# lh3/ropebwt2

Measured on AMD Instinct MI355X. Metric: Gsymbols/s inserted (wall-clock), bit-identical .fmd, higher is better.
Workload: dtype u8; 1 GPU; configs[1]: 100000000 x 101 bp synthetic reads (splitmix64 seed 42), -bsR -m4g, 1 x MI355X; step = one -m batch (40844297/40844297/18311406 reads); 20 steps = 7 job(s) of 3 batches, each job on an empty index (the last job stops after batch 2); reads_per_job=100000000, symbols=69532236588, symbols_per_gpu=69532236588, parallelism=1 GPU, driver=single engine, counts_ok=True

## Files before the change

include/rb2_hip.h:

```cpp
#ifndef RB2_HIP_H_
#define RB2_HIP_H_

#include <stdint.h>

#ifdef __cplusplus
extern "C" {
#endif

typedef struct rb2_hip_s rb2_hip_t;

#define RB2_SO_IO   0
#define RB2_SO_RLO  1
#define RB2_SO_RCLO 2

typedef void (*rb2_hip_fatal_cb)(void *user, const char *message);
void rb2_hip_set_fatal_handler(rb2_hip_fatal_cb cb, void *user);

int rb2_hip_device_count(void);

rb2_hip_t *rb2_hip_create(int device, int sorting_order);
void rb2_hip_destroy(rb2_hip_t *h);
int  rb2_hip_sorting_order(const rb2_hip_t *h);
void rb2_hip_reset(rb2_hip_t *h);

void rb2_hip_insert_multi(rb2_hip_t *h, int64_t len, const uint8_t *s);

void rb2_hip_set_lazy(rb2_hip_t *h, int on);
void rb2_hip_wait(rb2_hip_t *h);
int  rb2_hip_last_batch_counts(rb2_hip_t *h, int64_t d[36]);

void rb2_hip_prefetch(rb2_hip_t *h, const uint8_t *s, int64_t n_final, int64_t capacity);
int rb2_hip_host_register(void *p, int64_t nbytes);
int rb2_hip_host_unregister(void *p);

void rb2_hip_mem_info(int device, int64_t *free_bytes, int64_t *total_bytes);

void rb2_hip_insert_multi_dev(rb2_hip_t *h, int64_t len, const uint8_t *s_dev);

void rb2_hip_get_counts(rb2_hip_t *h, int64_t c[36]);

int64_t rb2_hip_rope_bytes(rb2_hip_t *h, int b);
int64_t rb2_hip_download_rope(rb2_hip_t *h, int b, uint8_t *dst);
typedef void (*rb2_hip_run_cb)(void *user, const uint8_t *runs, int64_t n_bytes);
int64_t rb2_hip_stream_rope(rb2_hip_t *h, int b, rb2_hip_run_cb cb, void *user);

void rb2_hip_load_ropes(rb2_hip_t *h, const uint8_t *const rle[6], const int64_t n_bytes[6]);

int64_t rb2_hip_load_fmd(rb2_hip_t *h, const void *fmd, int64_t n_bytes);
int64_t rb2_hip_load_fmd_file(rb2_hip_t *h, const char *path);

int64_t rb2_hip_save_fmd(rb2_hip_t *h, void *dst, int64_t cap);
int64_t rb2_hip_save_fmd_file(rb2_hip_t *h, const char *path);

int64_t rb2_hip_delete_strings(rb2_hip_t *h, int64_t n, const int64_t *ids);
void rb2_hip_delete_stats(rb2_hip_t *h, int64_t out[5]);

void rb2_hip_reserve(rb2_hip_t *h, int64_t batch_bytes, int64_t batch_strings, int64_t total_symbols);

void rb2_hip_rank1a(rb2_hip_t *h, int b, int64_t x, int64_t cx[6]);
void rb2_hip_rank_batch(rb2_hip_t *h, int b, int64_t n, const int64_t *x, int64_t *out);

void rb2_hip_backward_search(rb2_hip_t *h, int64_t n, const uint8_t *pat, const int64_t *off, int64_t *out);
void rb2_hip_backward_search_dev(rb2_hip_t *h, int64_t n, const uint8_t *pat, const int64_t *off, int64_t *out);
void rb2_hip_extend(rb2_hip_t *h, int64_t n, const int64_t *ik, int is_back, int64_t *ok);
int64_t rb2_hip_extract(rb2_hip_t *h, int64_t n, const int64_t *rows, int64_t max_len, uint8_t *out, int64_t *len);
int64_t rb2_hip_smem(rb2_hip_t *h, int64_t n, const uint8_t *qry, const int64_t *off, int64_t min_len, int64_t min_occ, int64_t max_mems,
                     int64_t *mem, int64_t *cnt);
void rb2_hip_smem_dev(rb2_hip_t *h, int64_t n, const uint8_t *qry, const int64_t *off, int64_t min_len, int64_t min_occ, int64_t max_mems,
                      int64_t *mem, int64_t *cnt);

int64_t rb2_hip_ssa_build(rb2_hip_t *h, int log2_step);
void    rb2_hip_ssa_drop(rb2_hip_t *h);
void    rb2_hip_ssa_info(rb2_hip_t *h, int64_t out[4]);
int64_t rb2_hip_locate(rb2_hip_t *h, int64_t n, const int64_t *iv, int64_t max_hits, int64_t *hit, int64_t *cnt);
void    rb2_hip_locate_dev(rb2_hip_t *h, int64_t n, const int64_t *iv, int64_t max_hits, int64_t *hit, int64_t *cnt);

int64_t rb2_hip_overlap(rb2_hip_t *h, int64_t n, const uint8_t *qry, const int64_t *off, int64_t min_ovlp, int64_t max_recs, int64_t *rec, int64_t *cnt);
void    rb2_hip_overlap_dev(rb2_hip_t *h, int64_t n, const uint8_t *qry, const int64_t *off, int64_t min_ovlp, int64_t max_recs, int64_t *rec, int64_t *cnt);
int64_t rb2_hip_string_ids(rb2_hip_t *h, int64_t n, const int64_t *zv, int64_t max_hits, int64_t *ids, int64_t *cnt);
void    rb2_hip_string_ids_dev(rb2_hip_t *h, int64_t n, const int64_t *zv, int64_t max_hits, int64_t *ids, int64_t *cnt);

int64_t rb2_hip_kmers(rb2_hip_t *h, int k, int64_t min_occ, int canonical, int64_t max_recs, int64_t *rec, int64_t hist_len, int64_t *hist, int64_t info[4]);

int64_t rb2_hip_approx(rb2_hip_t *h, int64_t n, const uint8_t *qry, const int64_t *off, int max_mm, int64_t min_occ, int64_t max_steps, int64_t max_recs, int64_t *rec, int64_t *cnt);
void    rb2_hip_approx_dev(rb2_hip_t *h, int64_t n, const uint8_t *qry, const int64_t *off, int max_mm, int64_t min_occ, int64_t max_steps, int64_t max_recs, int64_t *rec, int64_t *cnt);

int64_t rb2_hip_contained(rb2_hip_t *h, int64_t n, const int64_t *ids, int64_t *rec);
void    rb2_hip_contained_dev(rb2_hip_t *h, int64_t n, const int64_t *ids, int64_t *rec);

int64_t rb2_hip_irreducible(rb2_hip_t *h, int64_t n, const uint8_t *qry, const int64_t *off, int64_t min_ovlp, int64_t max_ext, int64_t max_steps, int64_t max_recs,
                            int64_t *rec, int64_t *cnt);
void    rb2_hip_irreducible_dev(rb2_hip_t *h, int64_t n, const uint8_t *qry, const int64_t *off, int64_t max_len, int64_t min_ovlp, int64_t max_ext, int64_t max_steps,
                                int64_t max_recs, int64_t *rec, int64_t *cnt);

int64_t rb2_hip_unitig_chains(rb2_hip_t *h, int64_t n_str, int64_t m, const int64_t *edges, int64_t *vtx, int64_t info[4]);
void    rb2_hip_unitig_chains_dev(rb2_hip_t *h, int64_t n_str, int64_t m, const int64_t *edges, int64_t *vtx, int64_t *info);
int64_t rb2_hip_unitig_text(rb2_hip_t *h, int64_t n_str, const int64_t *vtx, int canonical, int64_t min_reads, int64_t cap_u, int64_t cap_txt, int64_t *urec, uint8_t *txt,
                            int64_t info[4]);
int64_t rb2_hip_unitig_text_dev(rb2_hip_t *h, int64_t n_str, const int64_t *vtx, int canonical, int64_t min_reads, int64_t cap_u, int64_t cap_txt, int64_t *urec, uint8_t *txt,
                                int64_t info[4]);

uint64_t rb2_hip_rope_hash(rb2_hip_t *h, int b);

int64_t rb2_hip_unpack(rb2_hip_t *h, int64_t first, int64_t n, int reversed, int64_t cap, uint8_t *txt, int64_t *off);
int64_t rb2_hip_unpack_dev(rb2_hip_t *h, int64_t first, int64_t n, int reversed, int64_t cap, uint8_t *txt, int64_t *off);
int64_t rb2_hip_merge(rb2_hip_t *dst, rb2_hip_t *src, int64_t batch_bytes, int64_t info[4]);

int64_t rb2_hip_string_graph(rb2_hip_t *h, int64_t first, int64_t n, int64_t min_ovlp, int64_t max_ext, int64_t max_steps, int64_t max_recs, int64_t max_hits, int pairs,
                             int64_t cap, int64_t *edges, int64_t info[8]);
int64_t rb2_hip_string_graph_dev(rb2_hip_t *h, int64_t first, int64_t n, int64_t min_ovlp, int64_t max_ext, int64_t max_steps, int64_t max_recs, int64_t max_hits, int pairs,
                                 int64_t cap, int64_t *edges, int64_t info[8]);

int     rb2_hip_num_subropes(void);
void    rb2_hip_memcpy(rb2_hip_t *h, void *dst, const void *src, int64_t bytes, int kind);
void    rb2_hip_use_stream(rb2_hip_t *h, void *hip_stream);


typedef struct rb2_hip_multi_s rb2_hip_multi_t;
#define RB2_TRANSPORT_PEER 0
#define RB2_TRANSPORT_RCCL 1
#define RB2_MULTI_MAX_RANKS 64
rb2_hip_multi_t *rb2_hip_multi_create(int n, const int *devices, int sorting_order, int transport, const int *owner );
int rb2_hip_multi_transport(const rb2_hip_multi_t *m);
void rb2_hip_multi_unique_id(void *id128);
rb2_hip_multi_t *rb2_hip_multi_create_rank(int device, int rank, int nranks, const void *nccl_id, int sorting_order, const int *owner);
void rb2_hip_multi_destroy(rb2_hip_multi_t *m);
void rb2_hip_default_owners(int nranks, int owner[] );
int  rb2_hip_multi_nranks(const rb2_hip_multi_t *m);
int  rb2_hip_multi_nlocal(const rb2_hip_multi_t *m);
rb2_hip_t *rb2_hip_multi_engine(rb2_hip_multi_t *m, int local_rank);
void rb2_hip_multi_insert_multi(rb2_hip_multi_t *m, int64_t len, const uint8_t *s);
void rb2_hip_multi_insert_multi_dev(rb2_hip_multi_t *m, int64_t len, const uint8_t *const *s_dev);
void rb2_hip_multi_get_counts(rb2_hip_multi_t *m, int64_t c[36]);
int64_t rb2_hip_multi_rope_bytes(rb2_hip_multi_t *m, int b);
int64_t rb2_hip_multi_download_rope(rb2_hip_multi_t *m, int b, uint8_t *dst);
int64_t rb2_hip_multi_stream_rope(rb2_hip_multi_t *m, int b, rb2_hip_run_cb cb, void *user);
void rb2_hip_multi_load_ropes(rb2_hip_multi_t *m, const uint8_t *const rle[6], const int64_t n_bytes[6]);
int64_t rb2_hip_multi_load_fmd(rb2_hip_multi_t *m, const void *fmd, int64_t n_bytes);
void rb2_hip_multi_reserve(rb2_hip_multi_t *m, int64_t batch_bytes, int64_t batch_strings, int64_t total_symbols);
void rb2_hip_multi_reset(rb2_hip_multi_t *m);
void rb2_hip_multi_sync(rb2_hip_multi_t *m);
void rb2_hip_multi_rank1a(rb2_hip_multi_t *m, int b, int64_t x, int64_t cx[6]);
void rb2_hip_multi_stats(rb2_hip_multi_t *m, int64_t out[6]);
int64_t rb2_hip_multi_text_bytes(const rb2_hip_multi_t *m, int k);
uint64_t rb2_hip_multi_rope_hash(rb2_hip_multi_t *m, int b);
int rb2_hip_multi_plan_host(const int *owner , int nranks, const int64_t *g , int me, int64_t *sdest , int64_t (*pieces)[5] , int64_t *total);


void *rb2_hip_dev_alloc(rb2_hip_t *h, int64_t bytes);
void  rb2_hip_dev_free(rb2_hip_t *h, void *p);

void rb2_hip_synth_reads(rb2_hip_t *h, uint8_t *dst_dev, int64_t first_read, int64_t n_reads,
                         int read_len, uint64_t seed, int strand);
void rb2_hip_synth_reads_cov(rb2_hip_t *h, uint8_t *dst_dev, int64_t first_read, int64_t n_reads,
                             int read_len, uint64_t seed, int strand, int64_t genome_len);
void rb2_hip_synth_reads_skew(rb2_hip_t *h, uint8_t *dst_dev, int64_t first_read, int64_t n_reads,
                              int read_len, uint64_t seed, int strand, int64_t genome_len, int skew);

void rb2_hip_sync(rb2_hip_t *h);

void rb2_hip_sparse_stats(rb2_hip_t *h, int64_t out[4]);
void rb2_hip_layout_stats(rb2_hip_t *h, int64_t out[8]);
void rb2_hip_rewind_stats(rb2_hip_t *h, int64_t out[4]);
void rb2_hip_steady_stats(rb2_hip_t *h, int64_t out[4]);
void rb2_hip_lean_stats(rb2_hip_t *h, int64_t out[2]);
void rb2_hip_window_stats(rb2_hip_t *h, int64_t out[6]);

#define RB2_K_SYM      0
#define RB2_K_TSCAN    1
#define RB2_K_PREP     2
#define RB2_K_PART     3
#define RB2_K_MERGE    4
#define RB2_K_META     5
#define RB2_K_ADVANCE  6
#define RB2_K_INIT     7
#define RB2_K_RELAYOUT 8
#define RB2_K_SPLIT    9
#define RB2_K_COUNT    10
void rb2_hip_profile(rb2_hip_t *h, int enable);
void rb2_hip_profile_get(rb2_hip_t *h, int64_t launches[RB2_K_COUNT], double ms[RB2_K_COUNT],
                         int64_t units[RB2_K_COUNT], int reset);
const char *rb2_hip_kernel_name(int k);

void rb2_hip_layout(int *leaf_syms, int *tile_leaves, int *string_tile);

#ifdef __cplusplus
}
#endif
#endif
```

ropebwt2_amd/build.py:

```python
import os
import subprocess
import sys

PKG = os.path.dirname(os.path.abspath(__file__))
ROOT = os.path.dirname(PKG)
CSRC = os.path.join(PKG, "csrc")
LIBDIR = os.path.join(PKG, "lib")
BINDIR = os.path.join(PKG, "bin")
INC = os.path.join(ROOT, "include")


def lib_path(name):
    return os.path.join(LIBDIR, name)


def _newer(target, sources):
    if not os.path.exists(target):
        return False
    t = os.path.getmtime(target)
    return all(os.path.getmtime(s) <= t for s in sources)


def _run(cmd):
    r = subprocess.run(cmd, stdout=subprocess.PIPE, stderr=subprocess.STDOUT, text=True)
    if r.returncode != 0:
        sys.stderr.write(r.stdout)
        raise RuntimeError("build failed: " + " ".join(cmd))
    return r.stdout


def build_hip(force=False):
    os.makedirs(LIBDIR, exist_ok=True)
    out = lib_path("librb2hip.so")
    srcs = [os.path.join(CSRC, f) for f in ("rb2_engine.hip", "rb2_kernels.h", "rb2_merge.h", "rb2_device.h", "rb2_multi.h", "rb2_query.h", "rb2_unitig.h", "rb2_query_host.h", "rb2_query_plan.h", "rb2_kmer_plan.h", "rb2_fmd_load.h", "rb2_delete.h", "rb2_delete_plan.h", "rb2_fmd_save.h", "rb2_fmd_plan.h", "rb2_unpack.h", "rb2_merge_plan.h", "rb2_graph.h", "rb2_graph_plan.h")] + [os.path.join(INC, "rb2_hip.h")]
    if not force and _newer(out, srcs):
        return out
    hipcc = os.environ.get("HIPCC", "/opt/rocm/bin/hipcc")
    _run([hipcc, "--offload-arch=gfx950", "-O3", "-std=c++17", "-fPIC", "-shared", "-I" + INC, "-I" + CSRC,
          "-Wno-unused-value", "-o", out, srcs[0], "-ldl", "-lpthread"])
    return out


def build_host(force=False):
    host = os.path.join(CSRC, "host")
    if not os.path.isdir(host):
        return None
    os.makedirs(LIBDIR, exist_ok=True)
    os.makedirs(BINDIR, exist_ok=True)
    csrcs = sorted(os.path.join(host, f) for f in os.listdir(host) if f.endswith(".c") and f != "main.c")
    hdrs = [os.path.join(INC, f) for f in os.listdir(INC)] + [os.path.join(host, f) for f in os.listdir(host) if f.endswith(".h")]
    out = lib_path("libropebwt2.so")
    if force or not _newer(out, csrcs + hdrs + [lib_path("librb2hip.so")]):
        _run(["gcc", "-O2", "-g", "-std=gnu99", "-Wall", "-Werror=implicit-function-declaration", "-fPIC", "-shared", "-I" + INC, "-I" + host, "-o", out] + csrcs +
             ["-L" + LIBDIR, "-lrb2hip", "-Wl,-rpath,$ORIGIN", "-lpthread"])
    main_c = os.path.join(host, "main.c")
    exe = os.path.join(BINDIR, "ropebwt2")
    if os.path.exists(main_c) and (force or not _newer(exe, [main_c, out] + hdrs)):
        _run(["gcc", "-O2", "-g", "-std=gnu99", "-Wall", "-Werror=implicit-function-declaration", "-I" + INC, "-I" + host, "-o", exe, main_c,
              "-L" + LIBDIR, "-lropebwt2", "-lrb2hip", "-Wl,-rpath,$ORIGIN/../lib", "-lz", "-lpthread"])
    gen_c = os.path.join(ROOT, "tools", "synth_reads.c")
    gen = os.path.join(BINDIR, "synth_reads")
    if os.path.exists(gen_c) and (force or not _newer(gen, [gen_c])):
        _run(["gcc", "-O2", "-std=c99", "-Wall", "-o", gen, gen_c])
    return out


def build_all(force=False):
    build_hip(force)
    build_host(force)


if __name__ == "__main__":
    build_all(force="--force" in sys.argv)
    print("built:", sorted(os.listdir(LIBDIR)))
```

ropebwt2_amd/csrc/rb2_engine.hip:

```cpp
#include <hip/hip_runtime.h>
#include <cstdio>
#include <cstdlib>
#include <cstring>
#include <climits>
#include <vector>
#include <algorithm>
#include <chrono>
#include <mutex>
#include <thread>
#include <condition_variable>
#include "rb2_hip.h"
#include "rb2_kernels.h"
#include "rb2_query.h"
#include "rb2_unitig.h"
#include "rb2_unpack.h"
#include "rb2_graph.h"
#include "rb2_merge_plan.h"
#include "rb2_fmd_load.h"
#include "rb2_delete.h"
#include "rb2_fmd_save.h"
#include <cerrno>
#include <fcntl.h>
#include <unistd.h>

// ... 22 lines not shown
	if (g_fatal_cb) g_fatal_cb(g_fatal_user, msg);
	abort();
}
#define HIPCHK(expr) do { hipError_t e_ = (expr); if (e_ != hipSuccess) { \
	rb2_fatal("[rb2_hip] %s failed at %s:%d: %s\n", #expr, __FILE__, __LINE__, hipGetErrorString(e_)); } } while (0)

namespace {

static int g_vmm_ok = -1;
static size_t g_vmm_va = 0;
static bool vmm_enabled()
{
	if (g_vmm_ok < 0) {
		size_t fr = 0, tot = 0;
		g_vmm_ok = getenv("RB2_NO_VMM") ? 0 : 1;
		if (g_vmm_ok && hipMemGetInfo(&fr, &tot) == hipSuccess && tot > 0) g_vmm_va = (tot + (1ull << 30)) & ~((1ull << 30) - 1);
		else g_vmm_ok = 0;
	}
	return g_vmm_ok == 1;
}

static thread_local int64_t *t_grow_in_rounds = nullptr;
template <typename T> struct DevBuf {
	T *p = nullptr; size_t cap = 0;
	bool vm = false;
	size_t vm_div = 1;
	size_t vm_bytes = 0;
	bool vm_res = false;
	size_t vm_res_bytes = 0;
	size_t vm_piece = 0;
	std::vector<hipMemGenericAllocationHandle_t> vm_h; std::vector<size_t> vm_sz;
	size_t vm_range() const { return (g_vmm_va / vm_div + (4ull << 30)) & ~((2ull << 30) - 1); }
	bool vm_grow(size_t n)
	{
		const size_t CH = 64ull << 20;
		if (!vmm_enabled() || (p && !vm_res)) return false;
		int dev = 0;
		if (hipGetDevice(&dev) != hipSuccess) return false;
		hipMemAllocationProp prop = {};
		prop.type = hipMemAllocationTypePinned; prop.location.type = hipMemLocationTypeDevice; prop.location.id = dev;
		if (!p) {
			void *base = nullptr;
			const hipError_t er = hipMemAddressReserve(&base, vm_range(), CH, nullptr, 0);
			if (er != hipSuccess) {
				if (getenv("RB2_HIP_TRACE")) fprintf(stderr, "[rb2_hip] hipMemAddressReserve(%.1f GB) failed (%s): pools grow by hipMalloc + copy\n", vm_range() / 1e9, hipGetErrorString(er));
				(void)hipGetLastError(); g_vmm_ok = 0; return false;
			}
			p = (T*)base; vm_res = true; vm_res_bytes = vm_range();
		}
		if (!vm_piece) { vm_piece = CH; while (vm_piece < (2ull << 30) && vm_piece * 8 < n * sizeof(T)) vm_piece <<= 1; }
		const size_t want = (n * sizeof(T) + vm_piece - 1) / vm_piece * vm_piece;
		if (want > vm_res_bytes) {
			if (vm_bytes == 0) vm_release();
			return false;
		}
		hipMemAccessDesc acc = {};
		acc.location = prop.location; acc.flags = hipMemAccessFlagsProtReadWrite;
		while (vm_bytes < want) {
			const size_t add = vm_piece;
			hipMemGenericAllocationHandle_t h;
			bool ok = hipMemCreate(&h, add, &prop, 0) == hipSuccess;
			if (ok && (hipMemMap((char*)p + vm_bytes, add, 0, h, 0) != hipSuccess || hipMemSetAccess((char*)p + vm_bytes, add, &acc, 1) != hipSuccess)) {
				(void)hipMemUnmap((char*)p + vm_bytes, add); (void)hipMemRelease(h); ok = false;
			}
			if (!ok) {
				if (getenv("RB2_HIP_TRACE")) fprintf(stderr, "[rb2_hip] mapping %.2f GB behind %.2f GB failed (%s)\n", add / 1e9, vm_bytes / 1e9, hipGetErrorString(hipGetLastError()));
				(void)hipGetLastError();
				if (vm_bytes == 0) vm_release();
				return false;
			}
			vm_h.push_back(h); vm_sz.push_back(add);
			vm_bytes += add; cap = vm_bytes / sizeof(T);
		}
		return true;
	}
	void vm_release()
	{
		size_t off = 0;
		for (size_t i = 0; i < vm_h.size(); ++i) { (void)hipMemUnmap((char*)p + off, vm_sz[i]); (void)hipMemRelease(vm_h[i]); off += vm_sz[i]; }
		if (vm_res) (void)hipMemAddressFree(p, vm_res_bytes);
		vm_h.clear(); vm_sz.clear(); vm_bytes = 0; vm_res = false; vm_res_bytes = 0; p = nullptr; cap = 0;
	}
	void ensure(size_t n, bool keep = false, hipStream_t st = 0) {
		if (n <= cap) return;
		if (t_grow_in_rounds) ++*t_grow_in_rounds;
		if (vm && vm_grow(n)) return;
		size_t ncap = std::max(n, cap + cap / 2);
		T *q = nullptr;
		hipError_t e_ = hipMalloc((void**)&q, ncap * sizeof(T));
		if (e_ != hipSuccess && ncap > n) { ncap = n; (void)hipGetLastError(); e_ = hipMalloc((void**)&q, ncap * sizeof(T)); }
		if (e_ != hipSuccess) {
			size_t fr = 0, tot = 0;
			(void)hipMemGetInfo(&fr, &tot);
			rb2_fatal("[rb2_hip] out of device memory: a buffer of %.2f GB was needed (it held %.2f GB before), %.2f of %.2f GB are free; "
					"use smaller batches (-m) or shard the index over more GPUs\n", ncap * sizeof(T) / 1e9, cap * sizeof(T) / 1e9, fr / 1e9, tot / 1e9);
		}
		if (keep && p && cap) { HIPCHK(hipMemcpyAsync(q, p, cap * sizeof(T), hipMemcpyDeviceToDevice, st)); HIPCHK(hipStreamSynchronize(st)); }
		if (p) { if (vm_res) vm_release(); else HIPCHK(hipFree(p)); }
		p = q; cap = ncap;
	}
	void release() { if (p) { if (vm_res) vm_release(); else HIPCHK(hipFree(p)); } p = nullptr; cap = 0; }
};

struct Pool {
	DevBuf<uint8_t> data, xh; DevBuf<LeafMeta> meta, own; DevBuf<SbRec> sbrec; DevBuf<SbBase> sbbase;
	uint64_t cap_leaves = 0;
	void ensure(uint64_t leaves, bool keep, hipStream_t st) {
		if (leaves <= cap_leaves) return;
		data.vm = meta.vm = own.vm = sbrec.vm = true;
		meta.vm_div = own.vm_div = 16; sbrec.vm_div = 256;
		uint64_t nl = std::max<uint64_t>(leaves, cap_leaves + cap_leaves / 4);
		nl = (nl + SB - 1) / SB * SB;
		data.ensure(nl * LEAFB, keep, st); meta.ensure(nl, keep, st); own.ensure(nl, keep, st);
		sbrec.ensure(nl / SB + 1, keep, st); sbbase.ensure(nl / SB / SCHUNK + 2, keep, st); xh.ensure(nl / WPL + 1024, keep, st);
		cap_leaves = nl;
	}
	PoolView view() const { return PoolView{data.p, meta.p, sbrec.p, own.p, sbbase.p, xh.p}; }
	void release() { data.release(); meta.release(); own.release(); sbrec.release(); sbbase.release(); xh.release(); cap_leaves = 0; }
};

struct ProfRec { int k; hipEvent_t a, b; int64_t units; int round; };
constexpr uint64_t POS32_LIMIT = (1ull << 32) - (1ull << 24);

}

struct rb2_hip_s {
	int dev = 0, so = 0;
	hipStream_t st = 0;
	Pool pool[2];
	int side = 0;
	int pside = 0;
	bool sparse = false;
	double sp_lambda = 0.6;
	int sp_backoff = 0, sp_penalty = 0;
	int sp_head = 8;
	int sp_maxpen = 6;
	int leaf_pipe = 8192;
	Mailbox *mb_h = nullptr;
	Mailbox *mb_d = nullptr;
	uint64_t layout_epoch = 0;
	hipEvent_t ev_flag = nullptr;
	int dir_ride = 1;
	int ts_blocks = TSB;
	int lazy_verdict = 1;
	uint64_t spec_rounds = 0;
	int run_ahead = 3;
	int verdict_poll = 1;
	int steady_on = 1;
	int steady_ahead = 3;
	bool steady_launched = false;
	int64_t n_prep_skipped = 0, steady_seen = -1, steady_used = -1;
	int lean = 1;
	int64_t n_lean_rounds = 0;
	int64_t n_rewind = 0, n_rewound = 0, rewind_max = 0, n_rewind_even = 0;
	unsigned long long *pair_d = nullptr, *pair_h = nullptr;
	bool pair_valid = false;
	bool pending_end = false;
	double tl_base = 0, tl_last = 0;
	int64_t n_grow_in_rounds = 0;
	int timeline = 0;
	int lazy_insert = 1;
	int64_t n_relayout = 0, n_void = 0, n_sparse_rounds = 0;
	Ctl *ctl = nullptr;
	RopeDesc h_rope[NR];
	DevBuf<uint64_t> L[2], U[2], W[2], START, SIZE, INS_E, zblk;
	bool pos32 = false, want_pos32 = false;
	int pos_mode = getenv("RB2_POS") ? atoi(getenv("RB2_POS")) : 0;
	uint64_t pos_m0 = 0;
	DevBuf<uint16_t> RKREL;
	DevBuf<uint64_t> RKOLD;
	DevBuf<uint32_t> SPL;
	uint32_t split_epoch = 0;
	bool want_respread = false;
	int64_t n_respread = 0;
	DevBuf<uint64_t> qbuf;
	DevBuf<QTab> qtab;
	DevBuf<uint8_t> qbytes; DevBuf<int64_t> qin, qout;
	DevBuf<uint8_t> qscr;
	DevBuf<uint64_t> ssa_smp, ssa_len, ssa_head;
	bool ssa_valid = false; int ssa_s = 0; int64_t ssa_n = 0; uint64_t ssa_nstr = 0;
	uint64_t sp_nsb = 0;
	DevBuf<LeafDesc> LD;
	DevBuf<uint8_t> A[2], INS_A, sbuf;
	DevBuf<uint8_t> sbuf2; hipStream_t st_copy = nullptr; const uint8_t *pf_host = nullptr; size_t pf_done = 0; std::mutex pf_mu;
	bool pf_busy = false; std::condition_variable pf_cv;
	static constexpr int UP_T = 6, UP_NB = 2; static constexpr size_t UP_CH = 8u << 20;
	uint8_t *up_pin[UP_T][UP_NB] = {}; hipStream_t up_st[UP_T] = {}; hipEvent_t up_ev[UP_T][UP_NB] = {}; bool up_init = false;
	DevBuf<TileRec> trec; DevBuf<TileScan> tsc; DevBuf<TileFix> tfix; DevBuf<ChunkPart> cpart;
	DevBuf<SbTot> sbtot;
	uint64_t *d_tmp = nullptr;
	int prof = 0;
	std::vector<ProfRec> recs;
	std::vector<hipEvent_t> evpool;
	int64_t p_launch[RB2_K_COUNT]; double p_ms[RB2_K_COUNT]; int64_t p_units[RB2_K_COUNT];
	int debug = 0;
	int cur_round = -1;
	uint64_t *gcnt = nullptr;
	bool own_stream = true;
	int rank = 0, nranks = 1; int owner[NR] = {0};
	PushTab *push[2] = {nullptr, nullptr};
	int nactive = 1;
	DevBuf<uint8_t> xstage, xpack; DevBuf<uint16_t> xnb; DevBuf<uint64_t> xoff;
	uint8_t *xhost[2] = {nullptr, nullptr}; uint64_t *xtot[2] = {nullptr, nullptr}; hipEvent_t xev[2] = {nullptr, nullptr};
	int64_t fmds_size = -1;
	int compact_ok = 1;
	int compact_stats = 0;
	int64_t n_compact_rounds = 0;
	int64_t n_plain_handover = 0;
	bool pool_compact = false;
	bool plain_next = false;
	int ts_fold = SCHUNK;
	int ts_max = TS_MAX;
	int trace = 0;
	int64_t del_stats[5] = {0, 0, 0, 0, 0};
};

namespace {

hipEvent_t get_event(rb2_hip_t *h)
{
	if (!h->evpool.empty()) { hipEvent_t e = h->evpool.back(); h->evpool.pop_back(); return e; }
	hipEvent_t e; HIPCHK(hipEventCreate(&e)); return e;
}

struct Scope {
	rb2_hip_t *h; int k; ProfRec r; bool on;
	Scope(rb2_hip_t *h_, int k_, int64_t units) : h(h_), k(k_) {
		on = h->prof == 1 || (h->prof == 2 && k == RB2_K_MERGE);
		if (!on) return;
		r.k = k; r.units = units; r.round = h->cur_round; r.a = get_event(h); r.b = get_event(h);
		HIPCHK(hipEventRecord(r.a, h->st));
	}
	~Scope() {
		if (h->debug) { hipError_t e = hipStreamSynchronize(h->st); if (e != hipSuccess) { rb2_fatal("[rb2_hip] kernel group %s failed: %s\n", rb2_hip_kernel_name(k), hipGetErrorString(e)); } }
		if (!on) return;
		HIPCHK(hipEventRecord(r.b, h->st));
		h->recs.push_back(r);
	}
};

void drain_profile(rb2_hip_t *h)
{
	for (auto &r : h->recs) {
		float ms = 0;
		HIPCHK(hipEventElapsedTime(&ms, r.a, r.b));
		h->p_launch[r.k] += 1; h->p_ms[r.k] += ms; h->p_units[r.k] += r.units;
		if (h->trace && r.round >= 0 && (r.round < 20 || r.round % 10 == 0)) fprintf(stderr, "[rb2_hip] round %3d %-10s %8.3f ms\n", r.round, rb2_hip_kernel_name(r.k), ms);
		h->evpool.push_back(r.a); h->evpool.push_back(r.b);
	}
	h->recs.clear();
}

inline unsigned cdiv(uint64_t a, uint64_t b) { return (unsigned)((a + b - 1) / b); }
inline unsigned grid8(unsigned g) { return (g + 8u * XCD_RUN - 1u) & ~(8u * XCD_RUN - 1u); }

#define RB2_LAUNCH_STRIDE(h, KT, KF, ...) do { if ((h)->nranks > 1) hipLaunchKernelGGL(KT, __VA_ARGS__); else hipLaunchKernelGGL(KF, __VA_ARGS__); } while (0)
inline uint64_t rank_share(const rb2_hip_t *h, uint64_t whole)
{
	if (h->nranks <= 1) return whole;
	return std::min<uint64_t>(whole, 2 * whole / (uint64_t)std::max(1, h->nactive) + 64);
}

void build_directory(rb2_hip_t *h, int sd , int pool , uint64_t nsb_ub, bool sparse = false, bool leaves_done = false, uint64_t nsb_grid = 0)
{
	if (nsb_ub == 0) return;
	const hipStream_t st_ = h->st;
	if (nsb_grid == 0 || nsb_grid > nsb_ub) nsb_grid = nsb_ub;
	const unsigned nchunk = cdiv(nsb_ub, SCHUNK);
	h->sbtot.ensure(nsb_ub);
	PoolView pv = h->pool[pool].view();
	if (!leaves_done) RB2_LAUNCH_STRIDE(h, k_meta_sb<true>, k_meta_sb<false>, dim3(cdiv(nsb_grid, 8)), dim3(256), 0, st_, h->ctl, sd, pv, h->sbtot.p, (int)sparse);
	hipLaunchKernelGGL(k_sbscan3, dim3(nchunk), dim3(SCHUNK / SBT), 0, st_, (const Ctl*)h->ctl, (const SbTot*)h->sbtot.p, pv);
	hipLaunchKernelGGL(k_sbscan2, dim3(1), dim3(SB2T), 0, st_, (const Ctl*)h->ctl, pv.sbbase);
}

void fetch_ropes(rb2_hip_t *h)
{
	HIPCHK(hipMemcpyAsync(h->h_rope, &h->ctl->rope[h->side][0], sizeof(RopeDesc) * NR, hipMemcpyDeviceToHost, h->st));
	HIPCHK(hipStreamSynchronize(h->st));
}


struct BatchState {
	const uint8_t *s = nullptr; uint64_t len = 0, m = 0, max_len = 0, n_tot = 0, nsb_ub = 0;
	unsigned nst_ub = 0, nsc = 0;
	int cur = 0;
	bool known_ae = false;
	bool known_ae0 = false;
	bool known_steady = false;
	uint64_t counted = (uint64_t)-1;
	int lean = 0;
	uint64_t setup_round = (uint64_t)-1;
	bool setup_sparse = false; uint64_t setup_epoch = 0;
};
inline void mark_setup(const rb2_hip_t *h, BatchState &B, uint64_t r) { B.setup_round = r; B.setup_sparse = h->sparse; B.setup_epoch = h->layout_epoch; }
inline bool setup_done(const rb2_hip_t *h, const BatchState &B, uint64_t r, bool sparse) { return B.setup_round == r && B.setup_sparse == sparse && B.setup_epoch == h->layout_epoch; }

void ensure_strings(rb2_hip_t *h, uint64_t m)
{
	for (int i = 0; i < 2; ++i) { h->L[i].ensure(m); h->U[i].ensure(m); h->W[i].ensure(m); }
	h->SIZE.ensure(m); h->INS_E.ensure(m); h->RKREL.ensure(m); h->RKOLD.ensure(m); h->SPL.ensure(m + 64);
	h->A[0].ensure(m); h->A[1].ensure(m); h->INS_A.ensure(m); h->START.ensure(m + 1);
	const uint64_t nst = cdiv(m, STILE) + NR;
	h->trec.ensure(nst + 8 * XCD_RUN + 8); h->tsc.ensure(nst + 8 * XCD_RUN + 8); h->tfix.ensure(nst + 8 * XCD_RUN + 8); h->cpart.ensure(cdiv(nst, SCHUNK) + 1);
}

template <class P> StrArrays<P> str_arrays(rb2_hip_t *h, const BatchState &B)
{
	const int c = B.cur;
	return { (P*)h->L[c].p, (P*)h->U[c].p, h->W[c].p, h->A[c].p, (P*)h->L[c ^ 1].p, (P*)h->U[c ^ 1].p, h->W[c ^ 1].p, h->A[c ^ 1].p,
	         h->tfix.p, (P*)h->SIZE.p, (P*)h->INS_E.p, h->RKREL.p, (P*)h->RKOLD.p, h->INS_A.p };
}
template <class F> inline void with_pos(rb2_hip_t *h, const BatchState &B, F f) { if (h->pos32) f(str_arrays<uint32_t>(h, B)); else f(str_arrays<uint64_t>(h, B)); }

inline volatile unsigned long long *hmax_report(const rb2_hip_t *h) { return h->pos32 ? &h->mb_d->hmax : nullptr; }
inline volatile unsigned long long *steady_report(const rb2_hip_t *h) { return h->nranks == 1 ? &h->mb_d->steady : nullptr; }
inline uint32_t split_cap(const rb2_hip_t *h) { return (uint32_t)std::min<uint64_t>(h->SPL.cap, 0xffffffffu); }

static uint64_t max_batch_strings()
{
	const char *e = getenv("RB2_MAX_BATCH_STRINGS");
	uint64_t v = (1ull << 32) - 2 * STILE;
	if (e && atoll(e) > 0) v = std::min<uint64_t>(v, (uint64_t)atoll(e));
	return v;
}

static void index_rows_change(rb2_hip_t *h, bool drained = false)
{
	h->ssa_valid = false; h->ssa_s = 0; h->ssa_n = 0; h->ssa_nstr = 0;
	h->fmds_size = -1;
	if (!h->ssa_smp.p && !h->ssa_len.p && !h->ssa_head.p) return;
	if (!drained) HIPCHK(hipStreamSynchronize(h->st));
	h->ssa_smp.release(); h->ssa_len.release(); h->ssa_head.release();
}

bool batch_begin(rb2_hip_t *h, BatchState &B, int64_t len64, const uint8_t *s, bool may_split = false)
{
	const uint64_t len = (uint64_t)len64;
	hipStream_t st = h->st;
	const int is_srt = h->so != RB2_SO_IO;
	const unsigned nzb = cdiv(len, ZBLOCK);
	uint64_t m = 0;
	{
		Scope sc(h, RB2_K_INIT, 0);
		h->zblk.ensure(nzb + 2);
		uint64_t res[2] = {0, 0};
		HIPCHK(hipMemsetAsync(h->zblk.p + nzb + 1, 0, 8, st));
		hipLaunchKernelGGL(k_count_zeros, dim3(nzb), dim3(256), 0, st, s, len, h->zblk.p, h->zblk.p + nzb + 1);
		hipLaunchKernelGGL(k_zscan, dim3(1), dim3(SCHUNK), 0, st, h->zblk.p, nzb);
		HIPCHK(hipMemcpyAsync(res, h->zblk.p + nzb, 16, hipMemcpyDeviceToHost, st));
		HIPCHK(hipStreamSynchronize(st));
		m = res[0];
		if (res[1]) { rb2_fatal("[rb2_hip] the batch contains bytes that are not nt6 codes 0..5 ($ACGTN)\n"); }
		if (m >= max_batch_strings() && may_split) { B.m = m; return false; }
		if (m == 0 || m >= max_batch_strings()) { rb2_fatal("[rb2_hip] unsupported number of strings in one batch: %llu\n", (unsigned long long)m); }
		index_rows_change(h);
		h->START.ensure(m + 1);
		hipLaunchKernelGGL(k_write_starts, dim3(nzb), dim3(256), 0, st, s, len, h->zblk.p, h->START.p);
	}
	ensure_strings(h, m);
	B.nst_ub = cdiv(m, STILE) + NR;
	B.nsc = cdiv(B.nst_ub, SCHUNK);
	uint64_t n_tot = 0;
	for (int b = 0; b < NR; ++b) n_tot += h->h_rope[b].n;
	const uint64_t leaves_ub = (n_tot + len) / LEAF + NR * (SB + 1);
	if (!h->sparse) {
		h->pool[h->pside].ensure(leaves_ub, true, st);
		h->pool[h->pside ^ 1].ensure(leaves_ub, false, st);
	}
	if (!h->sparse) h->sbtot.ensure(leaves_ub / SB + 1);
	h->LD.ensure(std::max<uint64_t>(leaves_ub + NR + 16, m + 64 + (uint64_t)(NR + WLC + 1) * STILE / 2));
	B.s = s; B.len = len; B.m = m; B.n_tot = n_tot; B.nsb_ub = leaves_ub / SB + 1; B.cur = 0;
	{ uint64_t n0 = 0; for (int b = 0; b < NR; ++b) n0 += h->h_rope[b].cnt[0]; B.known_ae = B.known_ae0 = !is_srt || n0 == 0; }
	{
		uint64_t mx = 0;
		for (int b = 0; b < NR; ++b) mx = std::max<uint64_t>(mx, h->h_rope[b].n);
		h->pos_m0 = mx;
		h->pos32 = h->want_pos32 && h->pos_mode != 64 && mx + 2 * m < POS32_LIMIT;
		h->want_pos32 = false;
		h->mb_h->hmax = 0;
		h->mb_h->progress = 0;
		h->mb_h->steady = 0;
		h->steady_seen = h->steady_used = -1; h->steady_launched = false;
	}
	{
		Scope sc(h, RB2_K_INIT, 0);
		hipLaunchKernelGGL(k_batch_setup, dim3(1), dim3(1), 0, st, h->ctl, h->side, m, len, is_srt);
		with_pos(h, B, [&](const auto &S) { using P = std::remove_pointer_t<decltype(S.L)>;
		  hipLaunchKernelGGL(k_init_strings<P>, dim3(cdiv(m, 256)), dim3(256), 0, st, h->ctl, is_srt, s, h->START.p, S); });
	}
	HIPCHK(hipMemcpyAsync(&B.max_len, &h->ctl->max_len, 8, hipMemcpyDeviceToHost, st));
	HIPCHK(hipStreamSynchronize(st));
	return true;
}

void ne_snapshot(rb2_hip_t *h, uint64_t r)
{
	volatile uint32_t *slot = h->mb_h->ne[r % NE_RING];
	slot[0] = 0xffffffffu; slot[1] = 0xffffffffu;
	HIPCHK(hipMemcpyAsync((void*)slot, &h->ctl->ne[0], 8, hipMemcpyDeviceToHost, h->st));
}
bool ne_all_empty_from(rb2_hip_t *h, uint64_t r)
{
	for (uint64_t q = r; q-- > 0 && r - q < (uint64_t)NE_RING; ) {
		const volatile uint32_t *slot = h->mb_h->ne[q % NE_RING];
		const uint32_t v = slot[(q & 1) ^ 1];
		if (v == 0) return true;
		if (v != 0xffffffffu) return false;
	}
	return false;
}

uint32_t verdict_check(rb2_hip_t *h, bool drain);
uint32_t maybe_widen(rb2_hip_t *h, BatchState &B, uint64_t r)
{
	if (!h->pos32) return 0;
	const unsigned long long v = h->mb_h->hmax;
	uint64_t known = h->pos_m0, since = r + 1;
	if (v != 0) { known = v & ((1ull << 40) - 1); const uint64_t q = v >> 40; since = r >= q ? r - q : r + 1; }
	const char *e = getenv("RB2_POS_WIDEN_AT");
	if (known + (since + 1) * B.m < POS32_LIMIT && !(e && (uint64_t)atoll(e) == r)) return 0;
	if (const uint32_t v = verdict_check(h, true)) return v;
	hipStream_t st = h->st;
	const int cur = B.cur;
	for (DevBuf<uint64_t> *a : { &h->L[cur], &h->U[cur] }) {
		HIPCHK(hipMemcpyAsync(h->INS_E.p, a->p, B.m * 4, hipMemcpyDeviceToDevice, st));
		hipLaunchKernelGGL(k_widen, dim3(cdiv(B.m, 256)), dim3(256), 0, st, (const uint32_t*)h->INS_E.p, a->p, B.m);
	}
	h->pos32 = false;
	B.counted = (uint64_t)-1; B.lean = 0;
	if (h->trace) fprintf(stderr, "[rb2_hip] round %llu: positions widened to 64 bits (largest piece known: %llu symbols, %llu rounds ago)\n", (unsigned long long)r, (unsigned long long)known, (unsigned long long)since);
	return 0;
}

static inline void tl_slow(rb2_hip_t *h, const char *what)
{
	if (h->timeline < 2) return;
	const double now = std::chrono::duration<double, std::milli>(std::chrono::steady_clock::now().time_since_epoch()).count();
	if (h->tl_last != 0 && now - h->tl_last > 0.5) fprintf(stderr, "[rb2_hip] t = %8.3f ms  round %d: %.3f ms on the host up to and including %s\n", now - h->tl_base, h->cur_round, now - h->tl_last, what);
	h->tl_last = now;
}
inline bool lazy_round(const rb2_hip_t *h, bool spec) { return spec && h->lazy_verdict && h->nranks == 1; }
void require_verdicts_seen(const rb2_hip_t *h, uint64_t r, const char *what)
{ if (h->spec_rounds > 0) { rb2_fatal("[rb2_hip] internal: %s %llu queued behind %llu in-place rounds without their verdict\n", what, (unsigned long long)r, (unsigned long long)h->spec_rounds); } }
void round_counts(rb2_hip_t *h, BatchState &B, uint64_t r, bool spec = false, bool allow_lean = true)
{
	hipStream_t st = h->st;
	const int sd = h->side;
	const int64_t units = (int64_t)B.m;
	h->cur_round = (int)r;
	const TileRecs trs = { (uint32_t*)h->trec.p, (uint32_t)(h->trec.cap & ~(size_t)3) };
	tl_slow(h, "start of round_counts");
	B.lean = (allow_lean && !spec && h->nranks == 1 && !h->sparse && B.known_steady && h->steady_on) ? h->lean : 0;
	const bool one_launch_tail = B.nst_ub < (unsigned)h->ts_max;
	if (!spec) require_verdicts_seen(h, r, "counting phase without spec of round");
	SplitArgs sp; memset(&sp, 0, sizeof(sp));
	if (spec) {
	  sp.ctl = h->ctl; sp.pool = h->pool[h->pside].view(); sp.SPL = h->SPL.p; sp.spl_cap = split_cap(h); sp.epoch = h->split_epoch;
	  sp.mb = h->mb_d; sp.nsplitb = 64;
	  sp.round1 = (uint32_t)r;
	  sp.scan2 = (h->dir_ride && !one_launch_tail) ? sp.pool.sbbase : (SbBase*)nullptr;
	}
	SbBase *scan2_tail = (spec && h->dir_ride && one_launch_tail) ? h->pool[h->pside].view().sbbase : (SbBase*)nullptr;
	{ Scope sc(h, RB2_K_SYM, units);
	  with_pos(h, B, [&](const auto &S) { using P = std::remove_pointer_t<decltype(S.L)>;
	    if (spec) {
	      hipLaunchKernelGGL((k_sym<false, P, true>), dim3((unsigned)rank_share(h, B.nst_ub) + sp.nsplitb + (sp.scan2 ? 1u : 0u)), dim3(256), 0, st, h->ctl, sd, (int)(r & 1), S, trs, sp);
	    } else
	    if (h->nranks > 1) hipLaunchKernelGGL((k_sym<true, P>), dim3(grid8((unsigned)rank_share(h, B.nst_ub))), dim3(256), 0, st, h->ctl, sd, (int)(r & 1), S, trs, sp);
	    else if (B.lean) hipLaunchKernelGGL((k_sym<false, P, false, true>), dim3(grid8(cdiv(B.nst_ub, (unsigned)SYM_PAIR))), dim3(256), 0, st, h->ctl, sd, (int)(r & 1), S, trs, sp);
	    else hipLaunchKernelGGL((k_sym<false, P>), dim3(grid8(cdiv(B.nst_ub, (unsigned)SYM_PAIR))), dim3(256), 0, st, h->ctl, sd, (int)(r & 1), S, trs, sp); }); }
	tl_slow(h, "k_sym");
	if (spec && !lazy_round(h, spec)) HIPCHK(hipEventRecord(h->ev_flag, st));
	if (one_launch_tail) {
	  Scope sc(h, RB2_K_TSCAN, units);
	  const int do_setup = h->nranks == 1;
	  const unsigned grid = (unsigned)std::max(1, std::min<int>(TSB, h->ts_blocks)) + (scan2_tail ? 7u : 0u);
	  hipLaunchKernelGGL((h->sparse ? k_tscan_setup<true> : k_tscan_setup<false>), dim3(grid), dim3(SCHUNK), 0, st, h->ctl, sd, (int)(r & 1), trs, h->tfix.p, h->gcnt, do_setup, (int)spec, (uint32_t)r, hmax_report(h), scan2_tail, steady_report(h));
	  if (do_setup) mark_setup(h, B, r);
	} else
	{ Scope sc(h, RB2_K_TSCAN, units);
	  hipLaunchKernelGGL(k_tscan1, dim3(B.nsc), dim3(SCHUNK), 0, st, h->ctl, sd, trs, h->cpart.p);
	  if (B.nsc <= (unsigned)h->ts_fold) hipLaunchKernelGGL(k_tscan3<true>, dim3(B.nsc), dim3(SCHUNK), 0, st, h->ctl, sd, trs, h->cpart.p, h->tsc.p);
	  else {
	    hipLaunchKernelGGL(k_tscan2, dim3(1), dim3(SCHUNK), 0, st, h->ctl, sd, h->cpart.p);
	    hipLaunchKernelGGL(k_tscan3<false>, dim3(B.nsc), dim3(SCHUNK), 0, st, h->ctl, sd, trs, h->cpart.p, h->tsc.p);
	  }
	  const int do_setup = h->nranks == 1;
	  hipLaunchKernelGGL(k_tfix, dim3(std::max<unsigned>(1u, cdiv(B.nst_ub, 256))), dim3(256), 0, st, h->ctl, sd, (int)(r & 1), trs, h->tsc.p, h->tfix.p, h->gcnt, do_setup, (int)h->sparse, (uint32_t)r, hmax_report(h), (int)spec, steady_report(h));
	  if (do_setup) mark_setup(h, B, r); }
	tl_slow(h, "tile scans");
}

template <bool SPARSE, class P> void launch_prep(rb2_hip_t *h, const BatchState &B, uint64_t r, const PoolView &oldp, const StrArrays<P> &S)
{
	if (!SPARSE && B.known_steady && h->steady_on && h->nranks == 1) { ++h->n_prep_skipped; h->steady_launched = true; return; }
	Scope sc(h, RB2_K_PREP, (int64_t)B.m);
	const int sd = h->side, par = (int)(r & 1), is_comp = h->so == RB2_SO_RCLO;
	const unsigned tg = grid8((unsigned)rank_share(h, B.nst_ub));
	if (!B.known_ae) RB2_LAUNCH_STRIDE(h, (k_prep<false, SPARSE, true, P>), (k_prep<false, SPARSE, false, P>), dim3(tg), dim3(256), 0, h->st, h->ctl, sd, par, is_comp, oldp, S);
	RB2_LAUNCH_STRIDE(h, (k_prep<true, SPARSE, true, P>), (k_prep<true, SPARSE, false, P>), dim3(h->nranks > 1 ? tg : grid8(cdiv(tg, PREP_PT))), dim3(256), 0, h->st, h->ctl, sd, par, is_comp, oldp, S);
}

template <bool SPARSE, class P> void launch_advance(rb2_hip_t *h, const BatchState &B, uint64_t r, const PoolView &newp, const StrArrays<P> &S, ShardRec *send, ScanRide sr)
{
	Scope sc(h, RB2_K_ADVANCE, (int64_t)B.m);
	const int sd = h->side, is_comp = h->so == RB2_SO_RCLO;
	const unsigned tg = grid8((unsigned)rank_share(h, B.nst_ub));
	const PushTab *push = h->push[B.cur ^ 1];
	if (!B.known_ae) RB2_LAUNCH_STRIDE(h, (k_advance<false, SPARSE, true, P>), (k_advance<false, SPARSE, false, P>), dim3(tg), dim3(256), 0, h->st, h->ctl, sd, is_comp, (uint32_t)r, B.s, newp, S, send, push, ScanRide{ nullptr, 0u });
	RB2_LAUNCH_STRIDE(h, (k_advance<true, SPARSE, true, P>), (k_advance<true, SPARSE, false, P>), dim3(tg + sr.nscan), dim3(256), 0, h->st, h->ctl, sd, is_comp, (uint32_t)r, B.s, newp, S, send, push, sr);
}

void round_merge(rb2_hip_t *h, BatchState &B, uint64_t r, ShardRec *send, bool compact_out = false)
{
	hipStream_t st = h->st;
	const int sd = h->side;
	const int64_t units = (int64_t)B.m;
	PoolView oldp = h->pool[h->pside].view(), newp = h->pool[h->pside ^ 1].view();
	const uint64_t n_new_ub = B.n_tot + std::min<uint64_t>(B.len, (r + 1) * B.m);
	const unsigned nlf = cdiv(n_new_ub, WIN) + NR;
	const unsigned wg = cdiv(B.n_tot + rank_share(h, std::min<uint64_t>(B.len, (r + 1) * B.m)), WIN) + NR;
	if ((uint64_t)nlf * 64 >= (1ull << 32)) { rb2_fatal("[rb2_hip] the index is too large for one k_merge launch (%llu symbols: a launch is capped at 2^32 threads)\n", (unsigned long long)n_new_ub); }
	if (!setup_done(h, B, r, false))
	{ Scope sc(h, RB2_K_TSCAN, 0);
	  hipLaunchKernelGGL(k_setup<false>, dim3(1), dim3(64), 0, st, h->ctl, sd, h->gcnt, (int)(r & 1), (uint32_t)r, hmax_report(h), (int)(h->push[0] != nullptr), steady_report(h)); }
	const bool lean = B.lean != 0;
	if (lean && (h->nranks != 1 || h->sparse || !B.known_steady)) { rb2_fatal("[rb2_hip] internal: round %llu was counted lean and is not merged as a steady dense round\n", (unsigned long long)r); }
	if (lean) ++h->n_lean_rounds;
	with_pos(h, B, [&](const auto &S) { using P = std::remove_pointer_t<decltype(S.L)>;
	launch_prep<false>(h, B, r, oldp, S);
	tl_slow(h, "k_prep");
	{ Scope sc(h, RB2_K_PART, units);
	  const uint8_t *old_xh = h->pool_compact ? (const uint8_t*)oldp.xh : (const uint8_t*)nullptr;
	  if (lean) hipLaunchKernelGGL((k_part<false, P, true>), dim3(cdiv(wg + NR, 255)), dim3(256), 0, st, h->ctl, sd, (const P*)S.L, h->LD.p, old_xh);
	  else RB2_LAUNCH_STRIDE(h, (k_part<true, P>), (k_part<false, P>), dim3(cdiv(wg + NR, 255)), dim3(256), 0, st, h->ctl, sd, S.INS_E, h->LD.p, old_xh); }
	tl_slow(h, "k_part");
	{ Scope sc(h, RB2_K_MERGE, units);
	  if (lean) hipLaunchKernelGGL((k_merge<false, P, true>), dim3(grid8(cdiv(wg, MMW))), dim3(64 * MMW), 0, st, h->ctl, h->LD.p, oldp, newp, (const P*)S.L, (const uint8_t*)S.A, S.RKREL, (int)compact_out | (h->compact_stats ? 2 : 0), (int)(r & 1));
	  else RB2_LAUNCH_STRIDE(h, (k_merge<true, P>), (k_merge<false, P>), dim3(grid8(cdiv(wg, MMW))), dim3(64 * MMW), 0, st, h->ctl, h->LD.p, oldp, newp, S.INS_E, S.INS_A, S.RKREL, (int)compact_out | (h->compact_stats ? 2 : 0), (int)(r & 1)); }
	tl_slow(h, "k_merge");
	{ Scope sc(h, RB2_K_META, units);
	  build_directory(h, sd ^ 1, h->pside ^ 1, std::min<uint64_t>(B.nsb_ub, n_new_ub / (LEAF * SB) + NR + 1), false, false, (uint64_t)wg * WPL / SB + NR + 1); }
	tl_slow(h, "directory");
	launch_advance<false>(h, B, r, newp, S, send, ScanRide{ nullptr, 0u });
	});
	tl_slow(h, "k_advance");
	if (!B.known_ae && !send && h->nranks == 1) ne_snapshot(h, r);
	HIPCHK(hipGetLastError());
	tl_slow(h, "ne snapshot");
	h->side ^= 1; h->pside ^= 1; B.cur ^= 1;
	B.lean = 0;
	h->pool_compact = compact_out;
	if (compact_out) ++h->n_compact_rounds;
}

uint64_t slots_for(uint64_t n, bool sparse)
{
	if (!sparse) return n / LEAF + NR * (SB + 1);
	return (n / ((uint64_t)SP_FILL * SP_USED) + NR + 1) * SB;
}

void require_plain(rb2_hip_t *h, const char *who)
{
	if (!h->sparse && h->pool_compact) { rb2_fatal("[rb2_hip] internal: %s would read a pool that holds compact windows\n", who); }
}

void relayout(rb2_hip_t *h, bool to_sparse, uint64_t n_ub, uint64_t n_grow)
{
	hipStream_t st = h->st;
	require_plain(h, "a re-layout");
	struct NoWatch { int64_t *keep = t_grow_in_rounds; NoWatch() { t_grow_in_rounds = nullptr; } ~NoWatch() { t_grow_in_rounds = keep; } } nw;
	const auto t_host0 = std::chrono::steady_clock::now();
	const uint64_t cap_before[2] = { h->pool[0].cap_leaves, h->pool[1].cap_leaves };
	const uint32_t F = to_sparse ? SP_FILL : LEAF, K = to_sparse ? SP_USED : SB;
	const uint64_t slots = slots_for(n_ub, to_sparse), cap = to_sparse ? slots : slots_for(std::max(n_ub, n_grow), false);
	if (h->pool[h->pside ^ 1].cap_leaves < cap) {
		HIPCHK(hipStreamSynchronize(st));
		const auto tg0 = std::chrono::steady_clock::now();
		h->pool[h->pside ^ 1].ensure(cap, false, st);
		if (h->trace) fprintf(stderr, "[rb2_hip] pool grown to %.1f M leaf slots in %.3f s\n", h->pool[h->pside ^ 1].cap_leaves / 1e6, std::chrono::duration<double>(std::chrono::steady_clock::now() - tg0).count());
	}
	{
		Scope sc(h, RB2_K_RELAYOUT, 0);
		hipLaunchKernelGGL(k_relayout_setup, dim3(1), dim3(64), 0, st, h->ctl, h->side, F, K);
		hipLaunchKernelGGL(k_relayout, dim3(std::min<uint64_t>(cdiv(slots, MW), 1u << 20)), dim3(256), 0, st, (const Ctl*)h->ctl, h->side, h->pool[h->pside].view(), h->pool[h->pside ^ 1].view(), F, K, (int)h->sparse);
		build_directory(h, h->side, h->pside ^ 1, slots / SB + 1, to_sparse);
		HIPCHK(hipGetLastError());
	}
	h->pside ^= 1; h->sparse = to_sparse; ++h->n_relayout; ++h->layout_epoch; h->pool_compact = false;
	if (to_sparse) h->sp_nsb = slots / SB + 1;
	if (!to_sparse && h->pool[h->pside ^ 1].cap_leaves < cap) {
		HIPCHK(hipStreamSynchronize(st));
		h->pool[h->pside ^ 1].ensure(cap, false, st);
	}
	if (h->trace) {
		HIPCHK(hipStreamSynchronize(st));
		fprintf(stderr, "[rb2_hip] re-layout to %s: %.1f G symbols, %.3f s on the host clock, pools %.1f / %.1f -> %.1f / %.1f M leaf slots\n", to_sparse ? "sparse" : "dense", n_ub / 1e9,
				std::chrono::duration<double>(std::chrono::steady_clock::now() - t_host0).count(), cap_before[0] / 1e6, cap_before[1] / 1e6, h->pool[0].cap_leaves / 1e6, h->pool[1].cap_leaves / 1e6);
	}
}

void wait_progress(rb2_hip_t *h, uint64_t r)
{
	const uint32_t want = (uint32_t)r - (uint32_t)h->run_ahead;
	const auto t_spin = std::chrono::steady_clock::now();
	for (uint32_t spins = 0; (int32_t)(h->mb_h->progress - want) < 0 && !h->mb_h->void_round; ++spins) {
		if ((spins & 1023u) == 1023u) {
			if (hipStreamQuery(h->st) == hipSuccess) break;
			if (std::chrono::steady_clock::now() - t_spin > std::chrono::seconds(2)) { HIPCHK(hipStreamSynchronize(h->st)); break; }
		}
#if defined(__x86_64__)
#if defined(__x86_64__) || defined(__i386__)
		__builtin_ia32_pause();
#endif
#else
		std::this_thread::yield();
#endif
	}
}

constexpr uint64_t STEADY_BOUND_ROUNDS = 48;
void steady_poll(rb2_hip_t *h, BatchState &B, uint64_t r, bool bound)
{
	if (B.known_steady) return;
	auto reported = [&](unsigned long long v) -> int64_t { return v ? (int64_t)(v >> 1) - 1 : -1; };
	unsigned long long v = h->mb_h->steady;
	if (bound && h->steady_ahead > 0 && r < STEADY_BOUND_ROUNDS && !(v & 1ull) && (int64_t)r - reported(v) > (int64_t)h->steady_ahead) {
		const auto t_spin = std::chrono::steady_clock::now();
		for (uint32_t spins = 0; !((v = h->mb_h->steady) & 1ull) && (int64_t)r - reported(v) > (int64_t)h->steady_ahead && !h->mb_h->void_round; ++spins) {
			if ((spins & 1023u) == 1023u) {
				if (hipStreamQuery(h->st) == hipSuccess) break;
				if (std::chrono::steady_clock::now() - t_spin > std::chrono::seconds(2)) { HIPCHK(hipStreamSynchronize(h->st)); break; }
			}
#if defined(__x86_64__) || defined(__i386__)
			__builtin_ia32_pause();
#else
			std::this_thread::yield();
#endif
		}
		v = h->mb_h->steady;
	}
	if (!(v & 1ull)) return;
	B.known_steady = true; B.known_ae = true;
	h->steady_seen = reported(v);
	if (h->steady_on) h->steady_used = (int64_t)r;
}

int64_t take_back(rb2_hip_t *h, BatchState &B, uint64_t r_void, uint64_t r)
{
	if (r_void >= r || r - r_void > std::max<uint64_t>(h->spec_rounds, 1)) { rb2_fatal("[rb2_hip] internal: void round %llu reported while queueing round %llu (%llu in flight)\n", (unsigned long long)r_void, (unsigned long long)r, (unsigned long long)h->spec_rounds); }
	const int64_t depth = (int64_t)(r - r_void);
	if (depth & 1) { h->side ^= 1; B.cur ^= 1; }
	HIPCHK(hipMemsetAsync(&h->ctl->overflow, 0, 4, h->st));
	h->spec_rounds = 0; h->mb_h->void_round = 0;
	h->mb_h->progress = (uint32_t)r_void;
	B.counted = (uint64_t)-1; B.setup_round = (uint64_t)-1; B.lean = 0;
	return depth;
}

bool round_merge_sparse(rb2_hip_t *h, BatchState &B, uint64_t r, ShardRec *send = nullptr, bool spec = true)
{
	hipStream_t st = h->st;
	const int sd = h->side;
	const int64_t units = (int64_t)B.m;
	PoolView pv = h->pool[h->pside].view();
	const unsigned tg = grid8((unsigned)rank_share(h, B.nst_ub));
	if (++h->split_epoch == 0) ++h->split_epoch;
	if (!setup_done(h, B, r, true))
	{ Scope sc(h, RB2_K_TSCAN, 0);
	  require_verdicts_seen(h, r, "k_setup of in-place round");
	  hipLaunchKernelGGL(k_setup<true>, dim3(1), dim3(64), 0, st, h->ctl, sd, h->gcnt, (int)(r & 1), (uint32_t)r, hmax_report(h), (int)(h->push[0] != nullptr), steady_report(h)); }
	const bool lazy = lazy_round(h, spec);
	if (!lazy) { h->mb_h->void_round = 0; h->mb_h->respread = 0; }
	else if (h->spec_rounds > (uint64_t)h->run_ahead) wait_progress(h, r);
	const bool ride = h->dir_ride != 0;
	with_pos(h, B, [&](const auto &S) { using P = std::remove_pointer_t<decltype(S.L)>;
	launch_prep<true>(h, B, r, pv, S);
	{ Scope sc(h, RB2_K_PART, units);
	  RB2_LAUNCH_STRIDE(h, (k_part_sparse<true, P>), (k_part_sparse<false, P>), dim3(tg), dim3(256), 0, st, h->ctl, sd, pv, S.INS_E, S.INS_A, S.tf, (SpOrd*)h->LD.p, h->SPL.p, split_cap(h), S.RKOLD, (uint32_t)r); }
	{ Scope sc(h, RB2_K_MERGE, units);
	  const unsigned quads = cdiv(rank_share(h, B.m), MW * LROWS * LQ);
	  hipLaunchKernelGGL(k_merge_leaf<P>, dim3(std::max<unsigned>(WLC / MW, (h->leaf_pipe > 0 ? std::min<unsigned>(quads, (unsigned)h->leaf_pipe) : quads) / (WLC / MW) * (WLC / MW))), dim3(256), 0, st, (const Ctl*)h->ctl, (const SpOrd*)h->LD.p, pv, S.INS_E, S.INS_A, S.RKREL, h->sbtot.p); }
	if (!ride)
	{ Scope sc(h, RB2_K_META, units);
	  build_directory(h, sd ^ 1, h->pside, h->sp_nsb, true, true); }
	launch_advance<true>(h, B, r, pv, S, send, ScanRide{ (const SbTot*)h->sbtot.p, ride ? cdiv(h->sp_nsb, SCHUNK) : 0u });
	});
	const bool sp = spec && r + 1 <= B.max_len;
	if (!sp)
	{ Scope sc(h, RB2_K_SPLIT, 0);
	  hipLaunchKernelGGL(k_split, dim3(256 + (ride ? 1 : 0)), dim3(256), 0, st, h->ctl, pv, (const uint32_t*)h->SPL.p, split_cap(h), h->split_epoch, h->mb_d,
	                     ride ? pv.sbbase : (SbBase*)nullptr, (uint32_t)r + 1u); }
	if (!B.known_ae && !send && h->nranks == 1) ne_snapshot(h, r);
	HIPCHK(hipGetLastError());
	if (!sp && !lazy) HIPCHK(hipEventRecord(h->ev_flag, st));
	h->side ^= 1; B.cur ^= 1;
	if (sp) round_counts(h, B, r + 1, true);
	if (lazy) {
		B.counted = sp ? r + 1 : (uint64_t)-1;
		++h->n_sparse_rounds; ++h->spec_rounds;
		return true;
	}
	HIPCHK(hipEventSynchronize(h->ev_flag));
	if (const uint32_t v = h->mb_h->void_round) { take_back(h, B, v - 1, r + 1); return false; }
	if (h->mb_h->respread) h->want_respread = true;
	B.counted = sp ? r + 1 : (uint64_t)-1;
	++h->n_sparse_rounds;
	return true;
}

uint32_t verdict_check(rb2_hip_t *h, bool drain)
{
	if (!h->spec_rounds) return 0;
	if (drain) HIPCHK(hipStreamSynchronize(h->st));
	const uint32_t v = h->mb_h->void_round;
	if (h->mb_h->respread) { h->want_respread = true; if (drain) h->mb_h->respread = 0; }
	if (drain && !v) h->spec_rounds = 0;
	if (!drain && !h->verdict_poll) return 0;
	return v;
}

void batch_end(rb2_hip_t *h)
{
	h->cur_round = -1;
	HIPCHK(hipGetLastError());
	fetch_ropes(h);
	if (h->steady_launched) {
		uint32_t bad = 0;
		HIPCHK(hipMemcpyAsync(&bad, &h->ctl->steady_bad, 4, hipMemcpyDeviceToHost, h->st));
		HIPCHK(hipStreamSynchronize(h->st));
		h->steady_launched = false;
		if (bad) { rb2_fatal("[rb2_hip] internal: round %u is not a round of one-member groups behind a round that was\n", bad - 1u); }
	}
	drain_profile(h);
}

bool choose_layout(rb2_hip_t *h, BatchState &B, uint64_t r, uint64_t m_eff)
{
	const uint64_t n_ub = B.n_tot + std::min<uint64_t>(B.len, r * B.m);
	const double lambda = (double)m_eff / ((double)n_ub / LEAF + 1.0);
	bool want = h->sp_lambda > 0 && lambda < h->sp_lambda && h->sp_backoff == 0 && B.m < (1ull << 27);
	if (h->sparse && !want && lambda < 2 * h->sp_lambda && h->sp_backoff == 0) want = true;
	if (h->sp_backoff > 0) --h->sp_backoff;
	h->plain_next = false;
	if (want && !h->sparse && h->pool_compact) { want = false; h->plain_next = true; ++h->n_plain_handover; }
	if (want && !h->sparse) {
		const uint64_t need = slots_for(n_ub, true);
		const int grow = (need > h->pool[0].cap_leaves) + (need > h->pool[1].cap_leaves);
		size_t fr = 0, tot = 0;
		double leaves_more = 0;
		for (int k = 0; k < 2; ++k)
			if (need > h->pool[k].cap_leaves) leaves_more += h->pool[k].data.vm_res ? 1.25 * (double)need - (double)h->pool[k].cap_leaves : (double)need * 1.25;
		const double bytes = leaves_more * (LEAFB + 2 * sizeof(LeafMeta) + 2.0) * 1.02 + (256u << 20);
		if (grow && hipMemGetInfo(&fr, &tot) == hipSuccess && bytes > (double)fr) {
			want = false; h->sp_backoff = 1 << 30;
			if (h->trace) fprintf(stderr, "[rb2_hip] not enough free device memory for the sparse layout (%.1f GB needed, %.1f GB free): staying dense\n", bytes / 1e9, fr / 1e9);
		}
	}
	if (want != h->sparse || (h->sparse && h->want_respread)) {
		if (verdict_check(h, true)) return false;
	}
	if (want != h->sparse) { relayout(h, want, n_ub, B.n_tot + B.len); h->want_respread = false; }
	else if (h->sparse && h->want_respread) {
		if (h->trace) fprintf(stderr, "[rb2_hip] round %llu: re-spread (a superblock has no free slot left)\n", (unsigned long long)r);
		relayout(h, true, n_ub, B.n_tot + B.len);
		h->want_respread = false; ++h->n_respread;
	}
	return true;
}

void void_to_dense(rb2_hip_t *h, BatchState &B, uint64_t r)
{
	++h->n_void;
	if (h->trace) fprintf(stderr, "[rb2_hip] void round %llu (penalty %d)\n", (unsigned long long)r, h->sp_penalty);
	const uint64_t n_ub = B.n_tot + std::min<uint64_t>(B.len, r * B.m);
	relayout(h, false, n_ub, B.n_tot + B.len);
	h->sp_penalty = std::min(h->sp_penalty + 1, h->sp_maxpen);
	h->sp_backoff = 1 << h->sp_penalty;
}

void round_merge_any(rb2_hip_t *h, BatchState &B, uint64_t r, ShardRec *send, bool spec)
{
	if (h->sparse) {
		if (B.lean) round_counts(h, B, r, false, false);
		if (round_merge_sparse(h, B, r, send, spec)) { if (h->sp_penalty > 0 && (h->n_sparse_rounds & 63) == 0) --h->sp_penalty; return; }
		void_to_dense(h, B, r);
		if (spec) round_counts(h, B, r);
	}
	round_merge(h, B, r, send, h->compact_ok && (B.known_ae || h->nranks == 1) && r < B.max_len && !h->plain_next);
}

void batch_trace(rb2_hip_t *h)
{
	if (h->trace) fprintf(stderr, "[rb2_hip] batch done: layout %s, relayouts %lld (of them re-spreads %lld), void sparse rounds %lld, sparse rounds %lld\n", h->sparse ? "sparse" : "dense",
			(long long)h->n_relayout, (long long)h->n_respread, (long long)h->n_void, (long long)h->n_sparse_rounds);
}

void finish_pending(rb2_hip_t *h)
{
	if (!h || !h->pending_end) return;
	h->pending_end = false;
	HIPCHK(hipSetDevice(h->dev));
	batch_end(h);
	batch_trace(h);
}

static int64_t split_point(rb2_hip_t *h, const uint8_t *s, int64_t len)
{
	const int64_t W = 1 << 20;
	std::vector<uint8_t> win((size_t)W);
	for (int64_t a = len / 2; a < len - 1; a += W) {
		const int64_t n = std::min(W, len - 1 - a);
		HIPCHK(hipMemcpyAsync(win.data(), s + a, (size_t)n, hipMemcpyDeviceToHost, h->st)); HIPCHK(hipStreamSynchronize(h->st));
		const void *z = memchr(win.data(), 0, (size_t)n);
		if (z) return a + ((const uint8_t*)z - win.data()) + 1;
	}
	for (int64_t b = len / 2; b > 0; b -= W) {
		const int64_t a = std::max<int64_t>(0, b - W), n = b - a;
		HIPCHK(hipMemcpyAsync(win.data(), s + a, (size_t)n, hipMemcpyDeviceToHost, h->st)); HIPCHK(hipStreamSynchronize(h->st));
		for (int64_t i = n - 1; i >= 0; --i) if (win[(size_t)i] == 0) return a + i + 1;
	}
	rb2_fatal("[rb2_hip] insert_multi: cannot cut a batch of one string\n");
}

void insert_dev(rb2_hip_t *h, int64_t len64, const uint8_t *s, bool lazy = false)
{
	if (h->nranks > 1) { rb2_fatal("[rb2_hip] this handle is one rank of a rope-sharded index: insert through its rb2_hip_multi_t\n"); }
	BatchState B;
	const bool will_lazy = lazy && h->lazy_insert && !h->prof && !h->debug;
	h->want_pos32 = true;
	if (!batch_begin(h, B, len64, s, true)) {
		const int64_t p = split_point(h, s, len64);
		if (h->trace) fprintf(stderr, "[rb2_hip] batch of %llu strings cut at byte %lld of %lld\n", (unsigned long long)B.m, (long long)p, (long long)len64);
		insert_dev(h, p, s, false);
		DevBuf<uint8_t> half;
		half.ensure((size_t)(len64 - p) + 64);
		HIPCHK(hipMemcpyAsync(half.p, s + p, (size_t)(len64 - p), hipMemcpyDeviceToDevice, h->st));
		insert_dev(h, len64 - p, half.p, false);
		HIPCHK(hipStreamSynchronize(h->st));
		half.release();
		return;
	}
	if (h->sparse && h->sp_backoff < h->sp_head) h->sp_backoff = h->sp_head;
	struct GrowWatch { GrowWatch(int64_t *c) { t_grow_in_rounds = c; } ~GrowWatch() { t_grow_in_rounds = nullptr; } } gw(&h->n_grow_in_rounds);
	for (uint64_t r = 0; ; ) {
		uint32_t rv = verdict_check(h, r > B.max_len);
		if (!rv && r > B.max_len) break;
		if (!rv) {
			if (h->timeline > 1 && (r < 4 || r % 10 == 0)) fprintf(stderr, "[rb2_hip] t = %8.3f ms  queueing round %llu\n", std::chrono::duration<double, std::milli>(std::chrono::steady_clock::now().time_since_epoch()).count() - h->tl_base, (unsigned long long)r);
			if (!B.known_ae && r > 0 && ne_all_empty_from(h, r)) B.known_ae = true;
			steady_poll(h, B, r, !will_lazy);
			if (!(rv = maybe_widen(h, B, r)) && !(rv = verdict_check(h, false)) && !choose_layout(h, B, r, B.m)) rv = verdict_check(h, true);
		}
		if (rv) {
			rv = verdict_check(h, true);
			const uint64_t r_void = rv - 1;
			const int64_t depth = take_back(h, B, r_void, r);
			h->n_sparse_rounds -= depth;
			++h->n_rewind; h->n_rewound += depth; h->rewind_max = std::max(h->rewind_max, depth); if (!(depth & 1)) ++h->n_rewind_even;
			B.known_ae = B.known_ae0;
			memset((void*)h->mb_h->ne, 0xff, sizeof(h->mb_h->ne));
			B.known_steady = false; h->mb_h->steady = 0; B.lean = 0;
			r = r_void;
			void_to_dense(h, B, r);
			round_counts(h, B, r);
			round_merge_any(h, B, r, nullptr, true);
			++r;
			continue;
		}
		if (B.counted != r) round_counts(h, B, r);
		round_merge_any(h, B, r, nullptr, true);
		++r;
	}
	if (will_lazy) { h->cur_round = -1; HIPCHK(hipGetLastError()); h->pending_end = true; return; }
	batch_end(h);
	batch_trace(h);
}

void check_last_byte(rb2_hip_t *h, int64_t len, const uint8_t *s_dev)
{
	uint8_t last = 1;
	HIPCHK(hipMemcpyAsync(&last, s_dev + len - 1, 1, hipMemcpyDeviceToHost, h->st));
	HIPCHK(hipStreamSynchronize(h->st));
	if (last != 0) { rb2_fatal("[rb2_hip] insert_multi: buffer must be non-empty and end with a sentinel\n"); }
}

}


extern "C" {

void rb2_hip_set_fatal_handler(rb2_hip_fatal_cb cb, void *user) { g_fatal_cb = cb; g_fatal_user = user; }

int rb2_hip_device_count(void)
{
	int n = 0;
	if (hipGetDeviceCount(&n) != hipSuccess) return 0;
	return n;
}

rb2_hip_t *rb2_hip_create(int device, int sorting_order)
{
	int n = rb2_hip_device_count();
	if (n <= 0 || device < 0 || device >= n) {
		rb2_fatal("[rb2_hip] no usable HIP device (requested %d, visible %d); this engine has no CPU fallback\n", device, n);
	}
	if (sorting_order < 0 || sorting_order > 2) { rb2_fatal("[rb2_hip] bad sorting order %d\n", sorting_order); }
	HIPCHK(hipSetDevice(device));
	rb2_hip_t *h = new rb2_hip_s();
	h->dev = device; h->so = sorting_order;
	h->debug = getenv("RB2_HIP_DEBUG") ? atoi(getenv("RB2_HIP_DEBUG")) : 0;
	h->trace = getenv("RB2_HIP_TRACE") ? atoi(getenv("RB2_HIP_TRACE")) : 0;
	if (getenv("RB2_SPARSE_LAMBDA")) h->sp_lambda = atof(getenv("RB2_SPARSE_LAMBDA"));
	if (getenv("RB2_SPARSE_HEAD")) h->sp_head = atoi(getenv("RB2_SPARSE_HEAD"));
	if (getenv("RB2_LEAF_PIPE")) h->leaf_pipe = atoi(getenv("RB2_LEAF_PIPE"));
	if (getenv("RB2_COMPACT")) h->compact_ok = atoi(getenv("RB2_COMPACT"));
	if (getenv("RB2_COMPACT_STATS")) h->compact_stats = atoi(getenv("RB2_COMPACT_STATS"));
	if (getenv("RB2_TS_MAX")) h->ts_max = std::max(0, std::min((int)TS_MAX, atoi(getenv("RB2_TS_MAX"))));
	if (getenv("RB2_TS_FOLD")) h->ts_fold = std::max(0, std::min((int)SCHUNK, atoi(getenv("RB2_TS_FOLD"))));
	if (getenv("RB2_HIP_LAZY_INSERT")) h->lazy_insert = atoi(getenv("RB2_HIP_LAZY_INSERT"));
	if (getenv("RB2_HIP_TIMELINE")) h->timeline = atoi(getenv("RB2_HIP_TIMELINE"));
	if (getenv("RB2_SPARSE_MAXPEN")) h->sp_maxpen = atoi(getenv("RB2_SPARSE_MAXPEN"));
	if (h->trace) h->prof = 1;
	HIPCHK(hipStreamCreateWithFlags(&h->st, hipStreamNonBlocking));
	HIPCHK(hipMalloc((void**)&h->ctl, sizeof(Ctl)));
	HIPCHK(hipMalloc((void**)&h->d_tmp, 256));
	HIPCHK(hipMalloc((void**)&h->gcnt, GCN * 8));
	HIPCHK(hipHostMalloc((void**)&h->mb_h, sizeof(Mailbox), hipHostMallocDefault));
	memset(h->mb_h, 0, sizeof(Mailbox));
	HIPCHK(hipHostGetDevicePointer((void**)&h->mb_d, h->mb_h, 0));
	HIPCHK(hipEventCreateWithFlags(&h->ev_flag, hipEventDisableTiming));
	if (getenv("RB2_DIR_RIDE")) h->dir_ride = atoi(getenv("RB2_DIR_RIDE"));
	if (getenv("RB2_TS_BLOCKS")) h->ts_blocks = atoi(getenv("RB2_TS_BLOCKS"));
	if (getenv("RB2_LAZY_VERDICT")) h->lazy_verdict = atoi(getenv("RB2_LAZY_VERDICT"));
	if (getenv("RB2_RUN_AHEAD")) h->run_ahead = std::max(1, atoi(getenv("RB2_RUN_AHEAD")));
	if (getenv("RB2_VERDICT_POLL")) h->verdict_poll = atoi(getenv("RB2_VERDICT_POLL"));
	if (getenv("RB2_STEADY")) h->steady_on = atoi(getenv("RB2_STEADY")) != 0;
	if (getenv("RB2_STEADY_LEAN")) h->lean = std::min(1, std::max(0, atoi(getenv("RB2_STEADY_LEAN"))));
	if (!h->steady_on) h->lean = 0;
	if (getenv("RB2_STEADY_AHEAD")) h->steady_ahead = std::max(0, atoi(getenv("RB2_STEADY_AHEAD")));
	{ Ctl *hc = (Ctl*)calloc(1, sizeof(Ctl)); for (int b = 0; b < NR; ++b) hc->own[b] = 1; HIPCHK(hipMemcpy(h->ctl, hc, sizeof(Ctl), hipMemcpyHostToDevice)); free(hc); }
	HIPCHK(hipMemsetAsync(h->d_tmp, 0, 256, h->st));
	memset(h->h_rope, 0, sizeof(h->h_rope));
	memset(h->p_launch, 0, sizeof(h->p_launch)); memset(h->p_ms, 0, sizeof(h->p_ms)); memset(h->p_units, 0, sizeof(h->p_units));
	h->pool[0].ensure(SB * 8, false, h->st); h->pool[1].ensure(SB * 8, false, h->st);
	HIPCHK(hipStreamSynchronize(h->st));
	return h;
}

void rb2_hip_destroy(rb2_hip_t *h)
{ finish_pending(h);
	if (!h) return;
	HIPCHK(hipSetDevice(h->dev));
	if (h->own_stream) HIPCHK(hipStreamSynchronize(h->st)); else HIPCHK(hipDeviceSynchronize());
	index_rows_change(h, true);
	for (int i = 0; i < 2; ++i) { h->pool[i].release(); h->L[i].release(); h->U[i].release(); h->W[i].release(); }
	h->START.release(); h->SIZE.release(); h->INS_E.release(); h->RKREL.release(); h->RKOLD.release(); h->SPL.release(); h->qbuf.release(); h->zblk.release(); h->qtab.release(); h->qbytes.release(); h->qin.release(); h->qout.release(); h->qscr.release();
	h->LD.release(); h->A[0].release(); h->A[1].release(); h->INS_A.release(); h->sbuf.release(); h->sbuf2.release();
	if (h->st_copy) HIPCHK(hipStreamDestroy(h->st_copy));
	h->trec.release(); h->tsc.release(); h->tfix.release(); h->cpart.release(); h->sbtot.release();
	for (auto e : h->evpool) hipEventDestroy(e);
	HIPCHK(hipHostFree(h->mb_h)); HIPCHK(hipEventDestroy(h->ev_flag));

	if (h->pair_d) { HIPCHK(hipFree(h->pair_d)); HIPCHK(hipHostFree(h->pair_h)); }
	HIPCHK(hipFree(h->ctl)); HIPCHK(hipFree(h->d_tmp)); HIPCHK(hipFree(h->gcnt)); h->xstage.release(); h->xnb.release(); h->xpack.release(); h->xoff.release();
	for (int i = 0; i < 2; ++i) if (h->xhost[i]) { HIPCHK(hipHostFree(h->xhost[i])); HIPCHK(hipHostFree(h->xtot[i])); HIPCHK(hipEventDestroy(h->xev[i])); }
	if (h->own_stream) HIPCHK(hipStreamDestroy(h->st));
	delete h;
}

int rb2_hip_sorting_order(const rb2_hip_t *h) { return h->so; }

void rb2_hip_reset(rb2_hip_t *h)
{ finish_pending(h);
	HIPCHK(hipSetDevice(h->dev));
	index_rows_change(h);
	memset(h->h_rope, 0, sizeof(h->h_rope));
	h->sparse = false; h->sp_backoff = h->sp_penalty = 0;
	HIPCHK(hipMemsetAsync(&h->ctl->rope[0][0], 0, sizeof(RopeDesc) * 2 * NR, h->st));
	HIPCHK(hipMemsetAsync(&h->ctl->nsb_total, 0, 8, h->st));
}

void rb2_hip_insert_multi_dev(rb2_hip_t *h, int64_t len, const uint8_t *s_dev)
{ finish_pending(h); h->pair_valid = false;
	HIPCHK(hipSetDevice(h->dev));
	if (len <= 0) { rb2_fatal("[rb2_hip] insert_multi: len must be > 0\n"); }
	check_last_byte(h, len, s_dev);
	if (((uintptr_t)s_dev & 15) != 0) {
		h->sbuf.ensure((size_t)len + 64);
		HIPCHK(hipMemcpyAsync(h->sbuf.p, s_dev, (size_t)len, hipMemcpyDeviceToDevice, h->st));
		s_dev = h->sbuf.p;
	}
	insert_dev(h, len, s_dev);
}

void rb2_hip_prefetch(rb2_hip_t *h, const uint8_t *s, int64_t n_final, int64_t capacity)
{
	std::unique_lock<std::mutex> lk(h->pf_mu);
	HIPCHK(hipSetDevice(h->dev));
	h->pf_cv.wait(lk, [h] { return !h->pf_busy; });
	if (!h->st_copy) HIPCHK(hipStreamCreateWithFlags(&h->st_copy, hipStreamNonBlocking));
	if (s == nullptr) {
		HIPCHK(hipStreamSynchronize(h->st_copy));
		h->pf_host = nullptr; h->pf_done = 0;
		return;
	}
	if (h->pf_host != s) { h->pf_host = s; h->pf_done = 0; }
	if (n_final <= (int64_t)h->pf_done) return;
	const size_t need = (size_t)std::max(n_final, capacity) + 64;
	const size_t from = need > h->sbuf2.cap ? 0 : h->pf_done;
	h->pf_busy = true;
	lk.unlock();
	if (need > h->sbuf2.cap) { HIPCHK(hipStreamSynchronize(h->st_copy)); h->sbuf2.ensure(need); }
	HIPCHK(hipMemcpyAsync(h->sbuf2.p + from, s + from, (size_t)n_final - from, hipMemcpyHostToDevice, h->st_copy));
	lk.lock();
	h->pf_done = (size_t)n_final;
	h->pf_busy = false;
	h->pf_cv.notify_all();
}

int rb2_hip_host_register(void *p, int64_t nbytes)
{
	if (!p || nbytes <= 0) return -1;
	if (hipHostRegister(p, (size_t)nbytes, hipHostRegisterDefault) != hipSuccess) { (void)hipGetLastError(); return -1; }
	return 0;
}
int rb2_hip_host_unregister(void *p)
{
	if (hipHostUnregister(p) != hipSuccess) { (void)hipGetLastError(); return -1; }
	return 0;
}

void rb2_hip_mem_info(int device, int64_t *free_bytes, int64_t *total_bytes)
{
	size_t fr = 0, tot = 0;
	if (rb2_hip_device_count() <= device || hipSetDevice(device) != hipSuccess || hipMemGetInfo(&fr, &tot) != hipSuccess) { fr = tot = 0; (void)hipGetLastError(); }
	if (free_bytes) *free_bytes = (int64_t)fr;
	if (total_bytes) *total_bytes = (int64_t)tot;
}

void rb2_hip_insert_multi(rb2_hip_t *h, int64_t len, const uint8_t *s)
{
	HIPCHK(hipSetDevice(h->dev));
	if (len <= 0 || s[len - 1] != 0) { rb2_fatal("[rb2_hip] insert_multi: buffer must be non-empty and end with a sentinel\n"); }
	static const double tl0 = std::chrono::duration<double, std::milli>(std::chrono::steady_clock::now().time_since_epoch()).count();
	h->tl_base = tl0;
	auto tl = [&](const char *what) { if (h->timeline) fprintf(stderr, "[rb2_hip] t = %8.3f ms  %s\n", std::chrono::duration<double, std::milli>(std::chrono::steady_clock::now().time_since_epoch()).count() - tl0, what); };
	tl("insert_multi: enter");
	{
		std::unique_lock<std::mutex> lk(h->pf_mu);
		if (!h->st_copy) HIPCHK(hipStreamCreateWithFlags(&h->st_copy, hipStreamNonBlocking));
		h->pf_cv.wait(lk, [h] { return !h->pf_busy; });
		size_t have = 0;
		if (h->pf_host == s && h->pf_done > 0 && (int64_t)h->pf_done <= len && h->sbuf2.cap >= (size_t)len + 64) have = h->pf_done;
		h->pf_host = nullptr; h->pf_done = 0;
		h->pf_busy = true;
		lk.unlock();
		if (h->sbuf2.cap < (size_t)len + 64) { HIPCHK(hipStreamSynchronize(h->st_copy)); h->sbuf2.ensure((size_t)len + 64); have = 0; }
		if ((size_t)len > have) HIPCHK(hipMemcpyAsync(h->sbuf2.p + have, s + have, (size_t)len - have, hipMemcpyHostToDevice, h->st_copy));
		if (!h->pair_d) { HIPCHK(hipMalloc((void**)&h->pair_d, 36 * 8)); HIPCHK(hipHostMalloc((void**)&h->pair_h, 36 * 8, hipHostMallocDefault)); }
		HIPCHK(hipMemsetAsync(h->pair_d, 0, 36 * 8, h->st_copy));
		hipLaunchKernelGGL(k_pair_hist, dim3((unsigned)std::min<uint64_t>(((uint64_t)len + 4095) / 4096, 8192)), dim3(256), 0, h->st_copy, (const uint8_t*)h->sbuf2.p, (uint64_t)len, h->pair_d);
		HIPCHK(hipMemcpyAsync(h->pair_h, h->pair_d, 36 * 8, hipMemcpyDeviceToHost, h->st_copy));
		tl("upload queued");
		HIPCHK(hipStreamSynchronize(h->st_copy));
		h->pair_valid = true;
		tl("upload done");
		finish_pending(h);
		lk.lock();
		std::swap(h->sbuf, h->sbuf2);
		h->pf_busy = false;
		h->pf_cv.notify_all();
	}
	tl("previous batch done");
	insert_dev(h, len, h->sbuf.p, true);
	tl("rounds queued");
}

int rb2_hip_last_batch_counts(rb2_hip_t *h, int64_t d[36])
{
	if (!h->pair_valid) return 0;
	for (int i = 0; i < 36; ++i) d[i] = (int64_t)h->pair_h[i];
	return 1;
}

void rb2_hip_set_lazy(rb2_hip_t *h, int on) { finish_pending(h); h->lazy_insert = on; }
void rb2_hip_wait(rb2_hip_t *h) { finish_pending(h); }

void rb2_hip_get_counts(rb2_hip_t *h, int64_t c[36])
{ finish_pending(h);
	for (int i = 0; i < 36; ++i) c[i] = 0;
	for (int r = 0; r < NR; ++r) for (int a = 0; a < 6; ++a) c[rope_sym(r) * 6 + a] += (int64_t)h->h_rope[r].cnt[a];
// ... 631 lines not shown
}

static void fmds_begin(rb2_hip_t *h)
{
	finish_pending(h);
	HIPCHK(hipSetDevice(h->dev));
	if (h->nranks > 1) { rb2_fatal("[rb2_hip] save_fmd: this handle holds only its own sub-ropes of a sharded index; an .fmd needs the whole index on one engine\n"); }
	ensure_dense(h);
	require_plain(h, "save_fmd");
}

int64_t rb2_hip_save_fmd(rb2_hip_t *h, void *dst, int64_t cap)
{
	fmds_begin(h);
	if (h->fmds_size < 0) h->fmds_size = fmds_encode(h, nullptr);
	const int64_t size = h->fmds_size;
	if (!dst || cap < size) return size;
	FmdsOut o = {(uint8_t*)dst, -1, false};
	const int64_t got = fmds_encode(h, &o);
	if (got != size) { rb2_fatal("[rb2_hip] save_fmd: internal: the image has %lld bytes, the sizing pass said %lld\n", (long long)got, (long long)size); }
	return size;
}

int64_t rb2_hip_save_fmd_file(rb2_hip_t *h, const char *path)
{
	fmds_begin(h);
	const int fd = path ? open(path, O_WRONLY | O_CREAT | O_TRUNC, 0666) : -1;
	if (fd < 0) return -1;
	FmdsOut o = {nullptr, fd, false};
	const int64_t size = fmds_encode(h, &o);
	if (close(fd) != 0) o.err = true;
	if (o.err) return -1;
	h->fmds_size = size;
	return size;
}

static uint64_t piece_hash(rb2_hip_t *h, int r)
{
	HIPCHK(hipSetDevice(h->dev));
	ensure_dense(h);
	if (h->h_rope[r].n == 0) return 0;
	h->qbuf.ensure(8);
	HIPCHK(hipMemsetAsync(h->qbuf.p, 0, 8, h->st));
	require_plain(h, "a checksum");
	hipLaunchKernelGGL(k_piece_hash, dim3(2048), dim3(256), 0, h->st, (const Ctl*)h->ctl, h->side, h->pool[h->pside].view(), r, (unsigned long long*)h->qbuf.p);
	HIPCHK(hipGetLastError());
	uint64_t v = 0;
	HIPCHK(hipMemcpyAsync(&v, h->qbuf.p, 8, hipMemcpyDeviceToHost, h->st));
	HIPCHK(hipStreamSynchronize(h->st));
	return v;
}
static uint64_t hash_mix(uint64_t acc, uint64_t piece, uint64_t n)
{
	acc = (acc ^ piece) * 0x9E3779B97F4A7C15ull; acc ^= acc >> 29;
	return (acc ^ n) * 0xBF58476D1CE4E5B9ull;
}
uint64_t rb2_hip_rope_hash(rb2_hip_t *h, int b)
{ finish_pending(h);
	uint64_t acc = 0;
	if (h->nranks > 1) { rb2_fatal("[rb2_hip] rope_hash: this handle holds only its own sub-ropes of a sharded index (use rb2_hip_multi_rope_hash)\n"); }
	for (int r = 0; r < NR; ++r) if (rope_sym(r) == b) acc = hash_mix(acc, piece_hash(h, r), h->h_rope[r].n);
	return acc;
}

static void rank_piece(rb2_hip_t *h, int r, int64_t p, int64_t out[6])
{
	HIPCHK(hipSetDevice(h->dev));
	h->qbuf.ensure(8);
	require_plain(h, "a rank query");
	hipLaunchKernelGGL(k_rank_piece, dim3(1), dim3(64), 0, h->st, (const Ctl*)h->ctl, h->side, h->pool[h->pside].view(), r, (uint64_t)p, h->qbuf.p, (int)h->sparse);
	HIPCHK(hipGetLastError());
	HIPCHK(hipMemcpyAsync(out, h->qbuf.p, 48, hipMemcpyDeviceToHost, h->st));
	HIPCHK(hipStreamSynchronize(h->st));
}

void *rb2_hip_dev_alloc(rb2_hip_t *h, int64_t bytes)
{
	HIPCHK(hipSetDevice(h->dev));
	void *p = nullptr;
	HIPCHK(hipMalloc(&p, (size_t)bytes));
	return p;
}

void rb2_hip_dev_free(rb2_hip_t *h, void *p) { finish_pending(h); HIPCHK(hipSetDevice(h->dev)); HIPCHK(hipFree(p)); }

void rb2_hip_synth_reads_skew(rb2_hip_t *h, uint8_t *dst_dev, int64_t first_read, int64_t n_reads, int read_len, uint64_t seed, int strand, int64_t genome_len, int skew)
{ finish_pending(h);
	HIPCHK(hipSetDevice(h->dev));
	const uint64_t total = (uint64_t)n_reads * (read_len + 1) * (strand ? 2 : 1);
	if (total == 0) return;
	if ((uintptr_t)dst_dev & 15) { rb2_fatal("[rb2_hip] synth_reads: destination must be 16-byte aligned\n"); }
	if (genome_len != 0 && genome_len < read_len) { rb2_fatal("[rb2_hip] synth_reads: genome shorter than a read\n"); }
	hipLaunchKernelGGL(k_synth, dim3(cdiv(total, 256 * 16)), dim3(256), 0, h->st, dst_dev, (uint64_t)first_read, (uint64_t)n_reads, (uint32_t)read_len, seed, strand, (uint64_t)genome_len, skew);
	HIPCHK(hipGetLastError());
}

void rb2_hip_synth_reads_cov(rb2_hip_t *h, uint8_t *dst_dev, int64_t first_read, int64_t n_reads, int read_len, uint64_t seed, int strand, int64_t genome_len)
{
	rb2_hip_synth_reads_skew(h, dst_dev, first_read, n_reads, read_len, seed, strand, genome_len, 0);
}

void rb2_hip_synth_reads(rb2_hip_t *h, uint8_t *dst_dev, int64_t first_read, int64_t n_reads, int read_len, uint64_t seed, int strand)
{
	rb2_hip_synth_reads_cov(h, dst_dev, first_read, n_reads, read_len, seed, strand, 0);
}

void rb2_hip_reserve(rb2_hip_t *h, int64_t batch_bytes, int64_t batch_strings, int64_t total_symbols)
{ finish_pending(h);
	HIPCHK(hipSetDevice(h->dev));
	if (batch_bytes > 0) h->zblk.ensure(cdiv((uint64_t)batch_bytes, ZBLOCK) + 2);
	if (batch_strings > 0) ensure_strings(h, (uint64_t)batch_strings);
	if (total_symbols > 0) {
		const uint64_t leaves = (uint64_t)total_symbols / LEAF + NR * (SB + 1);
		size_t fr = 0, tot = 0;
		if (hipMemGetInfo(&fr, &tot) == hipSuccess && 2.0 * leaves * (LEAFB + 2.0 * sizeof(LeafMeta) + 2.0) > 0.6 * (double)fr) return;
		h->pool[h->pside].ensure(leaves, true, h->st);
		h->pool[h->pside ^ 1].ensure(leaves, false, h->st);
		h->LD.ensure(leaves + NR + 16);
		if (!h->sparse) h->sbtot.ensure(leaves / SB + 1);
	}
}

void rb2_hip_sparse_stats(rb2_hip_t *h, int64_t out[4])
{ finish_pending(h);
	out[0] = h->n_relayout; out[1] = h->n_void; out[2] = h->n_sparse_rounds; out[3] = h->sparse ? 1 : 0;
}

void rb2_hip_layout_stats(rb2_hip_t *h, int64_t out[8])
{ finish_pending(h);
	uint64_t ns = 0;
	HIPCHK(hipSetDevice(h->dev));
	HIPCHK(hipMemcpyAsync(&ns, &h->ctl->nsplit_total, 8, hipMemcpyDeviceToHost, h->st));
	HIPCHK(hipStreamSynchronize(h->st));
	out[0] = h->n_relayout; out[1] = h->n_void; out[2] = h->n_sparse_rounds; out[3] = h->sparse ? 1 : 0;
	out[4] = h->n_respread; out[5] = (int64_t)ns; out[6] = h->n_grow_in_rounds; out[7] = h->n_plain_handover;
}

void rb2_hip_steady_stats(rb2_hip_t *h, int64_t out[4])
{ finish_pending(h);
	out[0] = 0;
	out[1] = h->n_prep_skipped; out[2] = h->steady_seen; out[3] = h->steady_used;
}

void rb2_hip_rewind_stats(rb2_hip_t *h, int64_t out[4])
{ finish_pending(h);
	out[0] = h->n_rewind; out[1] = h->n_rewound; out[2] = h->rewind_max; out[3] = h->n_rewind_even;
}

void rb2_hip_lean_stats(rb2_hip_t *h, int64_t out[2])
{ finish_pending(h);
	out[0] = h->n_lean_rounds; out[1] = h->lean;
}

void rb2_hip_window_stats(rb2_hip_t *h, int64_t out[6])
{ finish_pending(h);
	unsigned long long w[4] = {0, 0, 0, 0};
	HIPCHK(hipSetDevice(h->dev));
	HIPCHK(hipMemcpyAsync(w, &h->ctl->wfmt[0], sizeof(w), hipMemcpyDeviceToHost, h->st));
	HIPCHK(hipStreamSynchronize(h->st));
	for (int i = 0; i < 4; ++i) out[i] = (int64_t)w[i];
	out[4] = h->n_compact_rounds; out[5] = h->compact_stats ? 1 : 0;
}

void rb2_hip_sync(rb2_hip_t *h) { finish_pending(h); HIPCHK(hipSetDevice(h->dev)); HIPCHK(hipStreamSynchronize(h->st)); }

void rb2_hip_profile(rb2_hip_t *h, int enable) { finish_pending(h); h->prof = enable; }

void rb2_hip_profile_get(rb2_hip_t *h, int64_t launches[RB2_K_COUNT], double ms[RB2_K_COUNT], int64_t units[RB2_K_COUNT], int reset)
{ finish_pending(h);
	for (int k = 0; k < RB2_K_COUNT; ++k) { launches[k] = h->p_launch[k]; ms[k] = h->p_ms[k]; units[k] = h->p_units[k]; }
	if (reset) { memset(h->p_launch, 0, sizeof(h->p_launch)); memset(h->p_ms, 0, sizeof(h->p_ms)); memset(h->p_units, 0, sizeof(h->p_units)); }
}

const char *rb2_hip_kernel_name(int k)
{
	static const char *nm[RB2_K_COUNT] = {"k_sym", "k_tscan", "k_prep", "k_part", "k_merge", "k_meta", "k_advance", "k_init", "k_relayout", "k_split"};
	return (k >= 0 && k < RB2_K_COUNT) ? nm[k] : "?";
}

void rb2_hip_layout(int *leaf_syms, int *tile_leaves, int *string_tile)
{
	if (leaf_syms) *leaf_syms = LEAF;
	if (tile_leaves) *tile_leaves = WPL;
	if (string_tile) *string_tile = STILE;
}

}

#include "rb2_multi.h"
```

ropebwt2_amd/csrc/rb2_kernels.h:

```cpp
#pragma once
#include "rb2_device.h"

namespace rb2 {


__device__ __forceinline__ uint32_t zero_bytes(uint32_t x)
{
	const uint32_t t = ((x & 0x7f7f7f7fu) + 0x7f7f7f7fu) | x;
	return __popc(~t & 0x80808080u);
}

__device__ __forceinline__ void load64(const uint8_t *s, uint64_t len, uint64_t base, uint32_t w[16])
{
	if (base + 64 <= len) {
		const uint4 *p = (const uint4*)(s + base);
#pragma unroll
		for (int i = 0; i < 4; ++i) { uint4 v = p[i]; w[4*i] = v.x; w[4*i+1] = v.y; w[4*i+2] = v.z; w[4*i+3] = v.w; }
	} else {
#pragma unroll
		for (int i = 0; i < 16; ++i) {
			uint32_t x = 0;
			for (int k = 0; k < 4; ++k) {
				const uint64_t p = base + 4*i + k;
				x |= (uint32_t)(p < len ? s[p] : 0xffu) << (8*k);
			}
			w[i] = x;
		}
	}
}

__global__ __launch_bounds__(256) void k_count_zeros(const uint8_t *s, uint64_t len, uint64_t *blk, uint64_t *bad_out)
{
	__shared__ uint32_t s_w[4];
	uint32_t w[16], c = 0, bad = 0;
	const uint64_t base = (uint64_t)blockIdx.x * ZBLOCK + threadIdx.x * 64;
	load64(s, len, base, w);
#pragma unroll
	for (int i = 0; i < 16; ++i) c += zero_bytes(w[i]);
	if (base + 64 <= len) {
#pragma unroll
		for (int i = 0; i < 16; ++i) bad |= (w[i] & 0xf8f8f8f8u) | ((w[i] >> 1) & (w[i] >> 2) & 0x01010101u);
	} else for (uint64_t p = base; p < len; ++p) bad |= s[p] > 5;
	uint32_t tot;
	block_excl_add<uint32_t>(c, s_w, &tot);
	if (threadIdx.x == 0) blk[blockIdx.x] = tot;
	if (bad) *bad_out = 1;
}

__global__ __launch_bounds__(256) void k_pair_hist(const uint8_t *s , uint64_t len, unsigned long long *out)
{
	__shared__ uint32_t h[36];
	if (threadIdx.x < 36) h[threadIdx.x] = 0;
	__syncthreads();
	uint32_t loc[36];
#pragma unroll
	for (int i = 0; i < 36; ++i) loc[i] = 0;
	const uint64_t K = 0x0101010101010101ull, L7 = 0x7f7f7f7f7f7f7f7full;
	auto eq = [&](uint64_t x, uint32_t v) -> uint64_t { const uint64_t t = x ^ (K * v); return ~(((t & L7) + L7) | t | L7); };
	for (uint64_t p = ((uint64_t)blockIdx.x * 256 + threadIdx.x) * 16; p < len; p += (uint64_t)gridDim.x * 256 * 16) {
		uint64_t w[2];
		if (p + 16 <= len) { const uint4 v = *(const uint4*)(s + p); w[0] = v.x | (uint64_t)v.y << 32; w[1] = v.z | (uint64_t)v.w << 32; }
		else { w[0] = w[1] = 0x0707070707070707ull; for (uint64_t q = p; q < len; ++q) { uint64_t &d = w[(q - p) >> 3]; const int sh = 8 * (int)((q - p) & 7); d = (d & ~(0xffull << sh)) | (uint64_t)s[q] << sh; } }
		uint64_t prev = p ? s[p - 1] : 0ull;
#pragma unroll
		for (int k = 0; k < 2; ++k) {
			const uint64_t cur = w[k], pw = cur << 8 | prev;
			prev = cur >> 56;
			uint64_t mp[6], mc[6];
#pragma unroll
			for (int v = 0; v < 6; ++v) { mp[v] = eq(pw, v); mc[v] = eq(cur, v); }
#pragma unroll
			for (int a = 0; a < 6; ++a)
#pragma unroll
				for (int b = 0; b < 6; ++b) loc[a * 6 + b] += (uint32_t)__popcll(mp[a] & mc[b]);
		}
	}
#pragma unroll
	for (int i = 0; i < 36; ++i) {
		uint32_t v = loc[i];
		for (int o = 32; o > 0; o >>= 1) v += __shfl_xor((int)v, o);
		if (lane_id() == 0 && v) atomicAdd(&h[i], v);
	}
	__syncthreads();
	if (threadIdx.x < 36 && h[threadIdx.x]) atomicAdd(&out[threadIdx.x], (unsigned long long)h[threadIdx.x]);
}

__global__ __launch_bounds__(SCHUNK) void k_zscan(uint64_t *blk, uint32_t n)
{
	__shared__ uint64_t s_w[16];
	uint64_t run = 0;
	for (uint32_t i0 = 0; i0 < n; i0 += SCHUNK) {
		const uint32_t i = i0 + threadIdx.x;
		const uint64_t v = i < n ? blk[i] : 0ull;
		uint64_t tot;
		const uint64_t ex = block_excl_add<uint64_t>(v, s_w, &tot);
		if (i < n) blk[i] = run + ex;
		run += tot;
	}
	if (threadIdx.x == 0) blk[n] = run;
}

__global__ __launch_bounds__(256) void k_write_starts(const uint8_t *s, uint64_t len, const uint64_t *blkoff, uint64_t *START)
{
	__shared__ uint32_t s_w[4];
	uint32_t w[16], c = 0;
	const uint64_t base = (uint64_t)blockIdx.x * ZBLOCK + threadIdx.x * 64;
	load64(s, len, base, w);
	if (blockIdx.x == 0 && threadIdx.x == 0) START[0] = 0;
#pragma unroll
	for (int i = 0; i < 16; ++i) c += zero_bytes(w[i]);
	uint64_t id = blkoff[blockIdx.x] + block_excl_add<uint32_t>(c, s_w, (uint32_t*)0);
	if (c == 0) return;
#pragma unroll
	for (int i = 0; i < 16; ++i) {
		if (zero_bytes(w[i]) == 0) continue;
		for (int k = 0; k < 4; ++k)
			if (((w[i] >> (8*k)) & 0xff) == 0) START[++id] = base + 4*i + k + 1;
	}
}

constexpr int CUR_SYMS = 9;
constexpr int CUR_BITS = 3 * CUR_SYMS;
constexpr uint64_t CUR_MASK = (1ull << CUR_BITS) - 1ull;
__device__ __forceinline__ uint32_t tri4(uint32_t x)
{
	x = (x & 0x07070707u) + 0x01010101u;
	x = (x | x >> 5) & 0x003f003fu;
	return (x | x >> 10) & 0xfffu;
}
__device__ __forceinline__ uint32_t pack9(const uint8_t *s, uint64_t len, uint64_t p)
{
	if (p + 16 <= len) {
		const uint32_t *q = (const uint32_t*)(s + (p & ~3ull));
		const uint32_t sh = (uint32_t)(p & 3) * 8;
		const uint32_t d0 = q[0], d1 = q[1], d2 = q[2], d3 = q[3];
		const uint32_t w0 = __builtin_amdgcn_alignbit(d1, d0, sh), w1 = __builtin_amdgcn_alignbit(d2, d1, sh), w2 = __builtin_amdgcn_alignbit(d3, d2, sh);
		return tri4(w0) | tri4(w1) << 12 | (tri4(w2) & 0x7u) << 24;
	}
	uint32_t w = 0;
	for (int i = 0; i < CUR_SYMS; ++i) {
		const uint64_t q = p + i;
		w |= (uint32_t)((q < len ? (s[q] & 7) : 0) + 1) << (3 * i);
	}
	return w;
}
__device__ __forceinline__ uint32_t pack9_words(uint32_t d0, uint32_t d1, uint32_t d2, uint32_t d3, uint32_t sh )
{
	const uint32_t w0 = __builtin_amdgcn_alignbit(d1, d0, sh), w1 = __builtin_amdgcn_alignbit(d2, d1, sh), w2 = __builtin_amdgcn_alignbit(d3, d2, sh);
	return tri4(w0) | tri4(w1) << 12 | (tri4(w2) & 0x7u) << 24;
}
__device__ __forceinline__ uint64_t cur_make(uint64_t next_pos, uint32_t syms) { return next_pos << CUR_BITS | syms; }
__device__ __forceinline__ uint64_t cur_pos(uint64_t w) { return w >> CUR_BITS; }
__device__ __forceinline__ bool cur_empty(uint64_t w) { return (w & 7) == 0; }
__device__ __forceinline__ int cur_sym(uint64_t w) { return (int)(w & 7) - 1; }
__device__ __forceinline__ uint64_t cur_next(uint64_t w) { return (w & ~CUR_MASK) | ((w & CUR_MASK) >> 3); }
__device__ __forceinline__ uint64_t cur_refill(const uint8_t *s, uint64_t len, uint64_t w) { const uint64_t p = cur_pos(w); return cur_make(p + CUR_SYMS, pack9(s, len, p)); }
// ... 152 lines not shown
		const uint4 okv = *(const uint4*)s_ok[q];
		allsingle[q] = (okv.x & okv.y & okv.z & okv.w) != 0;
		fused[q] = ae && allsingle[q];
		if (!fused[q] && have[q] && threadIdx.x == 0 && !(SPLIT && ctl->overflow)) ((Ctl*)ctl)->unfused[par] = 1;
		if (!LEAN && fused[q]) {
			P *Eb = INS_E + t[q].base; uint8_t *Ib = INS_A + t[q].base;
			const P slot0 = (P)(t[q].lt * STILE);
#pragma unroll
			for (int h = 0; h < 2; ++h) {
				const uint32_t x = (uint32_t)(h * 256) + threadIdx.x;
				if (x >= nval[q]) continue;
				Eb[x] = (P)(uv[q][h] - (slot0 + (P)x));
				Ib[x] = (uint8_t)av[q][h];
			}
		}
	}
	if (threadIdx.x < 6 * NT) {
		const int q = NT > 1 ? (int)(threadIdx.x >= 6) : 0, s = (int)threadIdx.x - 6 * q;
		const bool q1 = NT > 1 && q;
		const bool hv = q1 ? have[NT - 1] : true, as = q1 ? allsingle[NT - 1] : allsingle[0], fu = q1 ? fused[NT - 1] : fused[0];
		const uint32_t nv = q1 ? nval[NT - 1] : nval[0], mytile = tile + (uint32_t)q;
		uint32_t run = 0, fhpre = 0, lhpre = 0; int fh = -1, lh = -1;
		if (as) {
#pragma unroll
			for (int c = 0; c < 8; ++c) run += __popcll(s_bal[q][c][s]);
			if (nv) { fh = 0; lh = (int)nv - 1; lhpre = run - (uint32_t)((s_bal[q][lh >> 6][s] >> (lh & 63)) & 1ull); }
		} else
		for (int c = 0; c < 8; ++c) {
			const uint64_t hm = s_head[q][c], bm = s_bal[q][c][s];
			if (hm) {
				const int f = __builtin_ctzll(hm), l = 63 - __builtin_clzll(hm);
				if (fh < 0) { fh = c * 64 + f; fhpre = run + __popcll(bm & lt_mask(f)); }
				lh = c * 64 + l; lhpre = run + __popcll(bm & lt_mask(l));
			}
			run += __popcll(bm);
		}
		if (hv) {
			trec.hist(s, mytile) = run; trec.fhpre(s, mytile) = fhpre; trec.lhpre(s, mytile) = lhpre;
			if (s == 0) { trec.fh(mytile) = fh; trec.lh(mytile) = lh | (fu ? TILE_DONE : 0) | (as ? TILE_SINGLE : 0); }
		}
	}
	if (!STRIDE) return;
	}
}


__global__ __launch_bounds__(SCHUNK) void k_tscan1(const Ctl *ctl, int side, const TileRecs trec, ChunkPart *part)
{
	__shared__ uint32_t s_w[16]; __shared__ int s_wi[16];
	const uint32_t nt = ctl->seg[side].tile0[NR];
	const uint32_t t = blockIdx.x * SCHUNK + threadIdx.x;
	if (blockIdx.x * SCHUNK >= nt) return;
	const bool ok = t < nt;
	uint32_t tot;
	ChunkPart p;
	for (int s = 0; s < 6; ++s) { block_excl_add<uint32_t>(ok ? trec.hist(s, t) : 0u, s_w, &tot); p.sum[s] = tot; }
	const bool hh = ok && trec.fh(t) >= 0;
	int v = hh ? (int)t : -1;
	v = wave_incl_max(v);
	if (lane_id() == 63) s_wi[wave_id()] = v;
	__syncthreads();
	int mx = -1; for (int i = 0; i < SCHUNK / 64; ++i) mx = max(mx, s_wi[i]);
	__syncthreads();
	v = hh ? (int)t : INT_MAX;
	v = wave_incl_min_down(v);
	if (lane_id() == 0) s_wi[wave_id()] = v;
	__syncthreads();
	int mn = INT_MAX; for (int i = 0; i < SCHUNK / 64; ++i) mn = min(mn, s_wi[i]);
	p.mx = mx; p.mn = mn;
	if (threadIdx.x == 0) part[blockIdx.x] = p;
}

__device__ __forceinline__ int block_all_max(int v, int *s_w)
{
#pragma unroll
	for (int d = 32; d >= 1; d >>= 1) v = max(v, __shfl_xor(v, d));
	if (lane_id() == 0) s_w[wave_id()] = v;
	__syncthreads();
	int m = s_w[0];
	for (int i = 1; i < (int)(blockDim.x >> 6); ++i) m = max(m, s_w[i]);
	__syncthreads();
	return m;
}

__global__ __launch_bounds__(SCHUNK) void k_tscan2(const Ctl *ctl, int side, ChunkPart *part)
{
	__shared__ uint32_t s_w[16]; __shared__ int s_wi[16];
	const uint32_t nt = ctl->seg[side].tile0[NR];
	const uint32_t nc = (nt + SCHUNK - 1) / SCHUNK;
	uint32_t run[6] = {0, 0, 0, 0, 0, 0};
	int run_mx = -1;
	for (uint32_t i0 = 0; i0 < nc; i0 += SCHUNK) {
		const uint32_t i = i0 + threadIdx.x;
		const bool ok = i < nc;
		ChunkPart p;
		if (ok) p = part[i];
		else { for (int s = 0; s < 6; ++s) p.sum[s] = 0; p.mx = -1; p.mn = INT_MAX; }
		uint32_t o[6];
		for (int s = 0; s < 6; ++s) { uint32_t tot; o[s] = run[s] + block_excl_add<uint32_t>(p.sum[s], s_w, &tot); run[s] += tot; }
		const int omx = max(run_mx, block_excl_max(p.mx, s_wi, -1));
		run_mx = max(run_mx, block_all_max(p.mx, s_wi));
		if (ok) { for (int s = 0; s < 6; ++s) part[i].sum[s] = o[s]; part[i].mx = omx; }
	}
	int run_mn = INT_MAX;
	for (uint32_t k = (nc + SCHUNK - 1) / SCHUNK; k-- > 0; ) {
		const uint32_t i = k * SCHUNK + threadIdx.x;
		const bool ok = i < nc;
		const int mn = ok ? part[i].mn : INT_MAX;
		const int omn = min(run_mn, block_excl_min_down(mn, s_wi, INT_MAX));
		run_mn = min(run_mn, -block_all_max(mn == INT_MAX ? INT_MIN + 1 : -mn, s_wi));
		if (ok) part[i].mn = omn;
	}
}

template <bool FOLD> __global__ __launch_bounds__(SCHUNK) void k_tscan3(const Ctl *ctl, int side, const TileRecs trec, const ChunkPart *part, TileScan *tsc)
{
	__shared__ uint32_t s_w[16]; __shared__ int s_wi[16];
	const uint32_t nt = ctl->seg[side].tile0[NR];
	const uint32_t t = blockIdx.x * SCHUNK + threadIdx.x;
	if (blockIdx.x * SCHUNK >= nt) return;
	const bool ok = t < nt;
	ChunkPart cp;
	if (FOLD) {
		const uint32_t nc = (nt + SCHUNK - 1) / SCHUNK, i = threadIdx.x;
		ChunkPart p;
		for (int s = 0; s < 6; ++s) p.sum[s] = 0;
		p.mx = -1; p.mn = INT_MAX;
		if (i < nc) p = part[i];
		for (int s = 0; s < 6; ++s) { uint32_t tot; block_excl_add<uint32_t>(i < blockIdx.x ? p.sum[s] : 0u, s_w, &tot); cp.sum[s] = tot; }
		cp.mx = block_all_max(i < blockIdx.x ? p.mx : -1, s_wi);
		const int nmn = block_all_max((i > blockIdx.x && p.mn != INT_MAX) ? -p.mn : INT_MIN + 1, s_wi);
		cp.mn = nmn == INT_MIN + 1 ? INT_MAX : -nmn;
	} else cp = part[blockIdx.x];
	TileScan o;
	uint32_t h[6];
	for (int s = 0; s < 6; ++s) {
		h[s] = ok ? trec.hist(s, t) : 0u;
		o.pre[s] = cp.sum[s] + block_excl_add<uint32_t>(h[s], s_w, (uint32_t*)0);
	}
	const bool hh = ok && trec.fh(t) >= 0;
	o.lht = max(cp.mx, block_excl_max(hh ? (int)t : -1, s_wi, -1));
	o.nht = min(cp.mn, block_excl_min_down(hh ? (int)t : INT_MAX, s_wi, INT_MAX));
	if (ok) tsc[t] = o;
	if (ok && t == nt - 1) {
		TileScan e;
		for (int s = 0; s < 6; ++s) e.pre[s] = o.pre[s] + h[s];
		e.lht = -1; e.nht = INT_MAX;
		tsc[nt] = e;
	}
}


template <bool SPARSE> __device__ __forceinline__ void setup_body(Ctl *ctl, int side, const uint64_t *gcnt, int par, uint32_t round, volatile unsigned long long *hmax, volatile unsigned long long *steady, bool keep_ne = false);
__global__ __launch_bounds__(256) void k_tfix(Ctl *ctl, int side, int par, const TileRecs trec, const TileScan *tsc, TileFix *tf, uint64_t *gcnt, int do_setup, int sparse,
		uint32_t round, volatile unsigned long long *hmax, int spec, volatile unsigned long long *steady)
{
	__shared__ uint32_t s_t0[NR + 1];
	__shared__ uint64_t s_g[NR * 6];
	if (spec && ctl->overflow) return;
	const SegDesc &sg = ctl->seg[side];
	if (threadIdx.x <= NR) s_t0[threadIdx.x] = sg.tile0[threadIdx.x];
	__syncthreads();
	if (blockIdx.x == 0) {
		const int i = threadIdx.x;
		if (i < NR * 6) { const int b = i / 6, a = i % 6; const uint64_t v = s_t0[NR] ? (uint64_t)(tsc[s_t0[b + 1]].pre[a] - tsc[s_t0[b]].pre[a]) : 0ull; gcnt[i] = v; s_g[i] = v; }
		if (i == NR * 6) gcnt[NR * 6] = ctl->ne[par];
		if (do_setup) {
			__syncthreads();
			if (i < 64) { if (sparse) setup_body<true>(ctl, side, s_g, par, round, hmax, steady); else setup_body<false>(ctl, side, s_g, par, round, hmax, steady); }
		}
	}
	const uint32_t tile = blockIdx.x * 256 + threadIdx.x;
	if (tile >= s_t0[NR]) return;
	int b = 0;
	while (tile >= s_t0[b+1]) ++b;
	const uint32_t t0 = s_t0[b], t1 = s_t0[b+1];
	const TileScan me = tsc[tile], first = tsc[t0];
	const int lt = me.lht, nt = me.nht;
	TileFix f;
	TileScan sl, sn;
	const bool hl = lt >= (int)t0, hn = nt < (int)t1;
	if (hl) sl = tsc[lt];
	if (hn) sn = tsc[nt]; else sn = tsc[t1];
	for (int s = 0; s < 6; ++s) {
		f.tpre[s] = me.pre[s] - first.pre[s];
		f.popen[s] = hl ? sl.pre[s] - first.pre[s] + trec.lhpre(s, (uint32_t)lt) : 0u;
		f.pnext[s] = sn.pre[s] - first.pre[s] + (hn ? trec.fhpre(s, (uint32_t)nt) : 0u);
	}
	f.fopen = hl ? (uint32_t)((lt - t0) * STILE + (trec.lh((uint32_t)lt) & (TILE_DONE - 1))) : 0u;
	const int32_t mylh = trec.lh(tile);
	f.b = (uint32_t)b; f.lt = tile - t0; f.nexthead = ((tile + 1 >= t1 || trec.fh(tile + 1) == 0) ? 1u : 0u) | ((mylh >= 0 && (mylh & TILE_DONE)) ? 2u : 0u) | ((mylh >= 0 && (mylh & TILE_SINGLE)) ? 4u : 0u);
	f.segstart = sg.start[b]; f.segend = sg.start[b] + sg.cnt[b];
	tf[tile] = f;
}

template <bool SPARSE> __device__ __forceinline__ void setup_body(Ctl *ctl, int side, const uint64_t *gcnt , int par, uint32_t round, volatile unsigned long long *hmax, volatile unsigned long long *steady, bool keep_ne)
{
	const int r = lane_id();
	if (r == 0) { if (!keep_ne) ctl->ne[par ^ 1] = 0; ctl->overflow = 0; ctl->sbfull = 0; ctl->nsplit2[round & 1u] = 0; }
	if (r == 0) {
		const uint32_t uf = ctl->unfused[par];
		ctl->unfused[par ^ 1] = 0;
		if (steady) {
			*steady = ((unsigned long long)round + 1ull) << 1 | (uf ? 0ull : 1ull);
			if (uf && ctl->was_fused) ctl->steady_bad = round + 1u;
			if (!uf) ctl->was_fused = 1;
		}
	}
	if (r < WLC) ctl->wcnt[r * WLS] = 0;
	if (r == 0) ctl->wstride = max(1u, (ctl->seg[side].tile0[NR] + WLC - 1) / WLC) * STILE;
	const bool ok = r < NR;
	const int rr = ok ? r : 0;
	const SegDesc &sg = ctl->seg[side];
	SegDesc &ng = ctl->seg[side ^ 1];
	const RopeDesc o = ctl->rope[side][rr];
	RopeDesc n;
	n.n = ok ? o.n + sg.cnt[rr] : 0;
	if (hmax) {
		unsigned long long mx = n.n;
#pragma unroll
		for (int dd = 32; dd >= 1; dd >>= 1) { const unsigned long long t = __shfl_xor(mx, dd); mx = t > mx ? t : mx; }
		if (r == 0) *hmax = (unsigned long long)round << 40 | (mx < (1ull << 40) ? mx : (1ull << 40) - 1ull);
	}
	const int first = rope_of(rope_sym(rr), 0);
	for (int a = 0; a < 6; ++a) {
		const uint64_t c = ok ? gcnt[rr * 6 + a] : 0ull;
		n.cnt[a] = ok ? o.cnt[a] + c : 0ull;
		const uint64_t inc = dpp_incl_add64(n.cnt[a]);
		const uint64_t ex = inc - n.cnt[a];
		const uint64_t exf = __shfl(ex, first);
		if (ok) { ctl->count[r][a] = c; ctl->ac[r][a] = ex - exf; }
	}
	if (SPARSE) {
		n.nleaves = o.nleaves; n.leaf0 = o.leaf0; n.sb0 = o.sb0;
		if (ok) ctl->rope[side ^ 1][r] = n;
	} else {
		n.nleaves = (n.n + LEAF - 1) / LEAF;
		const uint64_t padded = (n.nleaves + SB - 1) / SB * SB, nwin = (n.nleaves + WPL - 1) / WPL;
		const uint64_t pinc = dpp_incl_add64(padded), winc = dpp_incl_add64(nwin);
		n.leaf0 = pinc - padded; n.sb0 = n.leaf0 / SB;
		if (ok) { ctl->rope[side ^ 1][r] = n; ctl->wf0[r] = winc - nwin; }
		if (r == 63) { ctl->wf0[NR] = winc; ctl->wf0[NR + 1] = winc; ctl->nsb_total = pinc / SB; }
	}
	uint64_t c2 = 0;
	if (ok && r != 0 && ctl->own[r]) {
		const int a = rope_sym(r), b = rope_prev(r);
		if (b == 0) c2 = gcnt[a];
		else for (int x = 0; x < 6; ++x) c2 += gcnt[rope_of(b, x) * 6 + a];
	}
	const uint64_t cinc = dpp_incl_add64(c2), st = cinc - c2;
	const uint32_t nt = (uint32_t)((c2 + STILE - 1) / STILE);
	const uint32_t tinc = dpp_incl_add(nt);
	if (ok) { ng.start[r] = st; ng.cnt[r] = c2; ng.tile0[r] = tinc - nt; }
	if (r == 63) { ng.tile0[NR] = tinc; ng.tile0[NR + 1] = tinc; }
	for (int a = 1; a < 6; ++a) {
		const int r2 = rope_of(a, rope_sym(rr));
		const uint64_t st2 = __shfl(st, r2);
		uint64_t before = 0;
		if (rope_sym(rr) != 0) for (int x = 0; x < rope_prev(rr); ++x) before += gcnt[rope_of(rope_sym(rr), x) * 6 + a];
		if (ok) ctl->dest[r][a] = st2 + before;
	}
	if (ok) ctl->dest[r][0] = 0;
}
template <bool SPARSE> __global__ __launch_bounds__(64) void k_setup(Ctl *ctl, int side, const uint64_t *gcnt, int par, uint32_t round, volatile unsigned long long *hmax, int keep_ne, volatile unsigned long long *steady)
{
	if (blockIdx.x) return;
	setup_body<SPARSE>(ctl, side, gcnt, par, round, hmax, steady, keep_ne != 0);
}

constexpr int TS_MAX = 4 * SCHUNK;
constexpr int TFW = 26;
static_assert(sizeof(TileFix) == TFW * 4, "TileFix is written out as 26 dwords");
constexpr int TSB = 4;
template <bool SPARSE> __global__ __launch_bounds__(SCHUNK) void k_tscan_setup(Ctl *ctl, int side, int par, const TileRecs trec, TileFix *tf, uint64_t *gcnt, int do_setup, int spec,
		uint32_t round, volatile unsigned long long *hmax, SbBase *scan2, volatile unsigned long long *steady)
{
	__shared__ uint32_t s_pre[6][TS_MAX + 4];
	__shared__ uint32_t s_out[SCHUNK / 64][32 * TFW];
	__shared__ unsigned long long s_head[TS_MAX / 64];
	__shared__ uint32_t s_p[6][16];
	__shared__ uint32_t s_t0[NR + 1];
	__shared__ uint64_t s_g[NR * 6];
	if (scan2 && blockIdx.x + 7 >= gridDim.x) { sbscan2_col<SCHUNK, 5>(ctl, scan2, (uint64_t*)s_out, (int)(blockIdx.x + 7 - gridDim.x)); return; }
	if (spec && ctl->overflow) return;
	const SegDesc &sg = ctl->seg[side];
	const int ln = lane_id(), wv = __builtin_amdgcn_readfirstlane(threadIdx.x >> 6);
	if (threadIdx.x <= NR) s_t0[threadIdx.x] = sg.tile0[threadIdx.x];
	if (threadIdx.x < TS_MAX / 64) s_head[threadIdx.x] = 0;
	const uint32_t nt_g = sg.tile0[NR];
	const uint32_t t_first = threadIdx.x * 4;
	uint32_t hs[4][6], tot[6] = {0, 0, 0, 0, 0, 0}, hb = 0;
	{
		const bool any = t_first < nt_g;
#pragma unroll
		for (int s = 0; s < 6; ++s) {
			uint4 v = make_uint4(0, 0, 0, 0);
			if (any) v = *(const uint4*)&trec.hist(s, t_first);
			hs[0][s] = v.x; hs[1][s] = v.y; hs[2][s] = v.z; hs[3][s] = v.w;
		}
		int4 f = make_int4(-1, -1, -1, -1);
		if (any) f = *(const int4*)&trec.fh(t_first);
		const int fv[4] = { f.x, f.y, f.z, f.w };
#pragma unroll
		for (int k = 0; k < 4; ++k) {
			const bool ok = t_first + k < nt_g;
			if (!ok) { for (int s = 0; s < 6; ++s) hs[k][s] = 0; }
			if (ok && fv[k] >= 0) hb |= 1u << k;
		}
	}
#pragma unroll
	for (int k = 0; k < 4; ++k)
#pragma unroll
		for (int s = 0; s < 6; ++s) { const uint32_t v = hs[k][s]; hs[k][s] = tot[s]; tot[s] += v; }
	uint32_t inc[6];
#pragma unroll
	for (int s = 0; s < 6; ++s) { inc[s] = dpp_incl_add(tot[s]); if (ln == 63) s_p[s][wv] = inc[s]; }
	__syncthreads();
	if (hb) atomicOr(&s_head[t_first >> 6], (unsigned long long)hb << (t_first & 63));
#pragma unroll
	for (int s = 0; s < 6; ++s) {
		const uint32_t p = ln < 16 ? s_p[s][ln] : 0u;
		const uint32_t pin = dpp_incl_add(p);
		const uint32_t off = wv ? (uint32_t)__builtin_amdgcn_readlane((int)pin, wv - 1) : 0u;
		const uint32_t base = off + inc[s] - tot[s];
#pragma unroll
		for (int k = 0; k < 4; ++k) if (t_first + k <= nt_g) s_pre[s][t_first + k] = base + hs[k][s];
	}
	__syncthreads();
	const uint32_t nt = s_t0[NR];
	const bool lead = blockIdx.x == 0;
	if (threadIdx.x < NR * 6) {
		const int b = threadIdx.x / 6, a = threadIdx.x % 6;
		const uint64_t v = nt ? (uint64_t)(s_pre[a][s_t0[b + 1]] - s_pre[a][s_t0[b]]) : 0ull;
		s_g[threadIdx.x] = v; if (lead) gcnt[threadIdx.x] = v;
	}
	if (lead && threadIdx.x == NR * 6) gcnt[NR * 6] = ctl->ne[par];
	__syncthreads();
	constexpr int NWV = SCHUNK / 64;
	const int tw0 = (do_setup ? NWV - 1 : NWV);
	if (lead && do_setup && wv == NWV - 1) { setup_body<SPARSE>(ctl, side, s_g, par, round, hmax, steady); return; }
	const uint32_t nscanb = gridDim.x - (scan2 ? 7u : 0u);
	const uint32_t wid = lead ? (uint32_t)wv : (uint32_t)tw0 + (blockIdx.x - 1u) * NWV + (uint32_t)wv, tw = (uint32_t)tw0 + (nscanb - 1u) * NWV;
	uint32_t *so = s_out[wv];
	for (uint32_t tb = wid * 64; tb < nt; tb += tw * 64) {
		const uint32_t tile = tb + (uint32_t)ln;
		const bool live = tile < nt;
		uint32_t f[TFW];
#pragma unroll
		for (int i = 0; i < TFW; ++i) f[i] = 0;
		if (live) {
			int b = 0;
			while (tile >= s_t0[b + 1]) ++b;
			const uint32_t t0 = s_t0[b], t1 = s_t0[b + 1];
			int lt = -1, nx = INT_MAX;
			{
				int w = (int)(tile >> 6);
				unsigned long long m = s_head[w] & lt_mask((int)(tile & 63));
				while (m == 0 && w > 0) m = s_head[--w];
				if (m) lt = w * 64 + 63 - __builtin_clzll(m);
				w = (int)(tile >> 6);
				const int wl = (int)((nt - 1) >> 6);
				m = (tile & 63) == 63 ? 0ull : s_head[w] & (~0ull << ((tile & 63) + 1));
				while (m == 0 && w < wl) m = s_head[++w];
				if (m) nx = w * 64 + __builtin_ctzll(m);
			}
			const bool hl = lt >= (int)t0, hn = nx < (int)t1;
			const uint32_t pn = hn ? (uint32_t)nx : t1;
#pragma unroll
			for (int s = 0; s < 6; ++s) {
				const uint32_t first = s_pre[s][t0];
				f[s] = s_pre[s][tile] - first;
				f[6 + s] = hl ? s_pre[s][lt] - first + trec.lhpre(s, (uint32_t)lt) : 0u;
				f[12 + s] = s_pre[s][pn] - first + (hn ? trec.fhpre(s, (uint32_t)nx) : 0u);
			}
			f[18] = hl ? (uint32_t)((lt - (int)t0) * STILE + (trec.lh((uint32_t)lt) & (TILE_DONE - 1))) : 0u;
			const int32_t mylh = trec.lh(tile);
			f[19] = (uint32_t)b; f[20] = tile - t0; f[21] = ((tile + 1 >= t1 || trec.fh(tile + 1) == 0) ? 1u : 0u) | ((mylh >= 0 && (mylh & TILE_DONE)) ? 2u : 0u) | ((mylh >= 0 && (mylh & TILE_SINGLE)) ? 4u : 0u);
			const uint64_t ss = sg.start[b], se = ss + sg.cnt[b];
			f[22] = (uint32_t)ss; f[23] = (uint32_t)(ss >> 32); f[24] = (uint32_t)se; f[25] = (uint32_t)(se >> 32);
		}
#pragma unroll
		for (int half = 0; half < 2; ++half) {
			if ((ln >> 5) == half) {
#pragma unroll
				for (int i = 0; i < TFW; ++i) so[(ln & 31) * TFW + i] = f[i];
			}
			__builtin_amdgcn_fence(__ATOMIC_SEQ_CST, "wavefront"); __builtin_amdgcn_wave_barrier();
			const uint32_t r0 = tb + 32u * half;
			const uint32_t nrec = r0 < nt ? min(32u, nt - r0) : 0u;
			uint32_t *dst = (uint32_t*)(tf + r0);
#pragma unroll
			for (int i = 0; i < 32 * TFW / 64; ++i) { const uint32_t d = (uint32_t)(i * 64 + ln); if (d < nrec * TFW) dst[d] = so[d]; }
			__builtin_amdgcn_fence(__ATOMIC_SEQ_CST, "wavefront"); __builtin_amdgcn_wave_barrier();
		}
	}
// ... 71 lines not shown
		if (hm) hpos = c * 64 + 63 - __builtin_clzll(hm);
		else for (int cc = c - 1; cc >= 0; --cc) if (G.head[cc]) { hpos = cc * 64 + 63 - __builtin_clzll(G.head[cc]); break; }
		uint64_t nm = G.head[c] & ~le;
		if (nm) npos = c * 64 + __builtin_ctzll(nm);
		else for (int cc = c + 1; cc < 8; ++cc) if (G.head[cc]) { npos = cc * 64 + __builtin_ctzll(G.head[cc]); break; }
	}
	m.pa = G.fix.tpre[a] + before(x, a);
	if (hpos == x && npos == x + 1) {
		m.pga = m.pa; m.F = (uint32_t)t.lt * STILE + (uint32_t)x; m.slot = m.F; m.lead = x;
		return m;
	}
	m.pga = hpos >= 0 ? G.fix.tpre[a] + before(hpos, a) : G.fix.popen[a];
	m.F = hpos >= 0 ? (uint32_t)t.lt * STILE + (uint32_t)hpos : G.fix.fopen;
	uint32_t bef = 0;
	const int oa = orda[a];
	for (int s = 0; s < 6; ++s) {
		if (orda[s] >= oa) continue;
		const uint32_t pg = hpos >= 0 ? G.fix.tpre[s] + before(hpos, s) : G.fix.popen[s];
		const uint32_t pn = npos >= 0 ? G.fix.tpre[s] + before(npos, s) : G.fix.pnext[s];
		bef += pn - pg;
	}
	m.slot = m.F + bef + (m.pa - m.pga);
	m.lead = hpos >= 0 ? hpos : 0;
	return m;
}

template <bool AE, bool SPARSE, typename P> __device__ __forceinline__ bool prep_tile(const uint32_t tile, const Ctl *ctl, int side, int par, int is_comp, const PoolView &oldp, const StrArrays<P> &S)
{
	const P *L = S.L, *U = S.U; uint8_t *A = S.A; const TileFix *tf = S.tf; P *INS_E = S.INS_E; uint8_t *INS_A = S.INS_A; P *SIZE = S.SIZE;
	__shared__ GroupLds G;
	const TileFix &tfx = tf[tile];
	const SegDesc &sg = ctl->seg[side];
	if ((ctl->ne[par] == 0) != AE) return false;
	if (SPARSE && ctl->overflow) return false;
	if (tile >= sg.tile0[NR]) return false;
	if (AE && (tfx.nexthead & 2u)) return true;
	TileCtx t;
	tile_ctx_fix(tfx, t);
	int sym2[2], flag2[2];
	P l2[2], u2[2];
	uint32_t araw[2];
	const uint32_t fixw = tilefix_word(tf, tile);
	const uint32_t nval = (uint32_t)min((uint64_t)STILE, t.segend - t.base);
#pragma unroll
	for (int h = 0; h < 2; ++h) {
		const uint32_t x = (uint32_t)(h * 256) + threadIdx.x;
		l2[h] = u2[h] = 0; araw[h] = 7;
		if (x < nval) { l2[h] = (L + t.base)[x]; u2[h] = AE ? l2[h] : (U + t.base)[x]; araw[h] = (A + t.base)[x]; }
	}
	group_setup(G, t, araw, fixw, sym2, flag2);
	const RopeDesc &rp = ctl->rope[side][t.b];
	const int orda[6] = { sym_ord(0, is_comp), sym_ord(1, is_comp), sym_ord(2, is_comp), sym_ord(3, is_comp), sym_ord(4, is_comp), sym_ord(5, is_comp) };
	if (AE) {
#pragma unroll
		for (int h = 0; h < 2; ++h) {
			const int x = h * 256 + threadIdx.x;
			if ((uint32_t)x >= nval) continue;
			const int a = sym2[h];
			const Member m = group_member(G, t, x, a, orda);
			(INS_E + t.segstart)[m.slot] = (P)(l2[h] - (P)m.F);
			(INS_A + t.segstart)[m.slot] = (uint8_t)a;
		}
		return true;
	}
	__shared__ P s_d[AE ? 1 : STILE][6];
	__shared__ uint16_t s_qs[AE ? 1 : STILE], s_qw[AE ? 1 : STILE];
	__shared__ uint32_t s_ns, s_nw;
	if (threadIdx.x == 0) { s_ns = 0; s_nw = 0; }
	__syncthreads();
	Member mm[2];
	P l0[2], u0[2];
#pragma unroll
	for (int h = 0; h < 2; ++h) {
		const int x = h * 256 + threadIdx.x;
		l0[h] = u0[h] = 0; mm[h].lead = -1;
		if ((uint32_t)x >= nval) continue;
		mm[h] = group_member(G, t, x, sym2[h], orda);
		l0[h] = (P)(l2[h] - (P)mm[h].F); u0[h] = (P)(u2[h] - (P)mm[h].F);
		if (mm[h].lead == x && u0[h] != l0[h]) {
			const bool small = u0[h] - l0[h] <= 3 * GSYM && (SPARSE || ((u0[h] - 1) >> LEAF_SH) == (l0[h] >> LEAF_SH));
			s_d[x][0] = l0[h]; s_d[x][1] = u0[h];
			if (small) s_qs[atomicAdd(&s_ns, 1u)] = (uint16_t)x; else s_qw[atomicAdd(&s_nw, 1u)] = (uint16_t)x;
		}
	}
	__syncthreads();
	for (uint32_t i = threadIdx.x; i < s_ns; i += 256) {
		const int x = s_qs[i];
		P d[6];
		range_counts<SPARSE, P>(oldp, rp, s_d[x][0], s_d[x][1], d);
		for (int s = 0; s < 6; ++s) s_d[x][s] = d[s];
	}
	for (uint32_t q = wave_id(); q < s_nw; q += 4) {
		const int x = s_qw[q];
		P d[6];
		wave_range_counts<SPARSE, P>(oldp, rp, s_d[x][0], s_d[x][1], d);
		__builtin_amdgcn_wave_barrier();
		if (lane_id() == 0) for (int s = 0; s < 6; ++s) s_d[x][s] = d[s];
	}
	__syncthreads();
#pragma unroll
	for (int h = 0; h < 2; ++h) {
		const int x = h * 256 + threadIdx.x;
		if ((uint32_t)x >= nval) continue;
		const int a = sym2[h];
		P e = l0[h];
		if (u0[h] != l0[h]) {
			const int oa = orda[a];
			P size = 0;
			for (int s = 0; s < 6; ++s) {
				const P d = s_d[mm[h].lead][s];
				if (orda[s] < oa) e += d;
				if (s == a) size = d;
			}
			(SIZE + t.base)[x] = (P)size;
			(A + t.base)[x] = (uint8_t)(a | 0x40 | (G.head[x >> 6] >> (x & 63) & 1 ? 0x80 : 0));
		}
		(INS_E + t.segstart)[mm[h].slot] = (P)e;
		(INS_A + t.segstart)[mm[h].slot] = (uint8_t)a;
	}
	return true;
}

constexpr int PREP_PT = 8;

template <bool AE, bool SPARSE = false, bool STRIDE = false, typename P = uint64_t> __global__ __launch_bounds__(256) void k_prep(const Ctl *ctl, int side, int par, int is_comp, PoolView oldp, StrArrays<P> S)
{
	if (AE && !STRIDE) {
		const uint32_t t0 = xcd_item() * PREP_PT, nt = ctl->seg[side].tile0[NR];
		if (ctl->ne[par] != 0) return;
		if (SPARSE && ctl->overflow) return;
		const uint32_t ln = (uint32_t)lane_id();
		const bool mine = ln < (uint32_t)PREP_PT && t0 + ln < nt;
		uint32_t nh = 2u;
		if (mine) nh = S.tf[t0 + ln].nexthead;
		uint64_t todo = __ballot(mine && !(nh & 2u));
		while (todo) {
			const uint32_t k = (uint32_t)__builtin_ctzll(todo);
			todo &= todo - 1;
			prep_tile<AE, SPARSE, P>(t0 + k, ctl, side, par, is_comp, oldp, S);
			if (todo) __syncthreads();
		}
		return;
	}
	for (uint32_t tile = STRIDE ? blockIdx.x : xcd_item(); ; ) {
		if (!prep_tile<AE, SPARSE, P>(tile, ctl, side, par, is_comp, oldp, S)) return;
		if (!STRIDE) return;
		tile += gridDim.x;
		if (tile >= ctl->seg[side].tile0[NR]) return;
		__syncthreads();
	}
}


template <bool STRIDE, typename P = uint64_t, bool LEAN = false> __global__ __launch_bounds__(256) void k_part(const Ctl *ctl, int side, const P *INS_E, LeafDesc *LD, const uint8_t *old_xh)
{
	__shared__ uint64_t s_wf0[NR + 1];
	__shared__ uint32_t s_q[256];
	if (threadIdx.x <= NR) s_wf0[threadIdx.x] = ctl->wf0[threadIdx.x];
	__syncthreads();
	for (uint64_t blk = blockIdx.x; blk * 255 < s_wf0[NR] + NR; blk += gridDim.x) {
	if (STRIDE && blk != blockIdx.x) __syncthreads();
	const uint64_t gid = blk * 255 + threadIdx.x;
	const bool ok = gid < s_wf0[NR] + NR;
	int b = 0; uint64_t j = 0; uint32_t q = 0;
	if (ok) {
		while (gid >= s_wf0[b+1] + b + 1) ++b;
		j = gid - s_wf0[b] - b;
		const SegDesc &sg = ctl->seg[side];
		const P *E = INS_E + sg.start[b];
		const uint64_t o = j * WIN;
		uint64_t lo = 0, hi = sg.cnt[b];
		while (lo < hi) {
			const uint64_t mid = (lo + hi) >> 1;
			if ((LEAN ? (uint64_t)E[mid] : E[mid] + mid) >= o) hi = mid; else lo = mid + 1;
		}
		q = (uint32_t)lo;
	}
	s_q[threadIdx.x] = q;
	__syncthreads();
	if (!ok || threadIdx.x == 255 || j >= s_wf0[b+1] - s_wf0[b]) { if (!STRIDE) return; continue; }
	const RopeDesc &orp = ctl->rope[side][b], &nrp = ctl->rope[side ^ 1][b];
	const uint32_t q1 = s_q[threadIdx.x + 1];
	const uint64_t o0 = j * WIN, i0 = o0 - q;
	LeafDesc d;
	d.i0 = i0;
	d.ins0 = ctl->seg[side].start[b] + q;
	d.gl = nrp.leaf0 + j * WPL;
	d.oleaf0 = (uint32_t)orp.leaf0;
	const uint64_t ow = i0 >> 12, onw = (orp.nleaves + WPL - 1) / WPL;
	static_assert(WPL * LEAF == 4096, "a window is 4096 symbols");
	const uint8_t *xw = old_xh ? old_xh + orp.leaf0 / WPL : nullptr;
	const uint32_t h0 = ow < onw ? (xw ? (uint32_t)xw[ow] & 3u : 0u) : 1u;
	const uint32_t h1 = ow + 1 < onw ? (xw ? (uint32_t)xw[ow + 1] & 3u : 0u) : 1u;
	d.ni = (uint16_t)((uint32_t)(q1 - q) | h0 << 14);
	d.nvalid = (uint16_t)((uint32_t)min((uint64_t)WIN, nrp.n - o0) | h1 << 14);
	LD[s_wf0[b] + j] = d;
	if (!STRIDE) return;
	}
}


template <typename P> __device__ __forceinline__ bool part_sparse_tile(const uint32_t tile, Ctl *ctl, int side, const PoolView &oldp, const P *__restrict__ INS_E, const uint8_t *__restrict__ INS_A, const TileFix *tf, SpOrd *LD, uint32_t *SPL, uint32_t spl_cap, P *RKOLD, uint32_t round)
{
	const TileFix &tfx = tf[tile];
	if (tile >= ctl->seg[side].tile0[NR]) return false;
	TileCtx t;
	tile_ctx_fix(tfx, t);
	const RopeDesc &rp = ctl->rope[side][t.b];
	const P *E = INS_E;
	__shared__ uint32_t s_w[4], s_base;
	const uint64_t nsb = (rp.nleaves + SB - 1) / SB;
	const uint64_t base = nsb ? sb_pos(oldp, rp.sb0) : 0;
	__shared__ P s_cb[6];
	if (threadIdx.x < 6) s_cb[threadIdx.x] = nsb ? (P)sb_cum(oldp, rp.sb0, (int)threadIdx.x) : (P)0;
	bool ok[2];
	uint64_t p[2], pprev[2], sbi[2], sbs[2];
	uint32_t aq[2];
#pragma unroll
	for (int h = 0; h < 2; ++h) {
		const uint64_t g = t.base + h * 256 + threadIdx.x;
		ok[h] = g < t.segend;
		p[h] = ok[h] ? (uint64_t)E[g] : 0;
		aq[h] = ok[h] ? (uint32_t)INS_A[g] & 7u : 0u;
		if (aq[h] > 5u) aq[h] = 0;
		pprev[h] = (ok[h] && g > t.segstart) ? (uint64_t)E[g - 1] : ~0ull;
	}
	bool slow[2];
	uint64_t cum[2];
#pragma unroll
	for (int h = 0; h < 2; ++h) { slow[h] = false; sbs[h] = 0; cum[h] = 0; sbi[h] = 0; }
	{
		uint4 hi[2]; uint32_t cg[2]; uint64_t bp[2], bc[2];
		uint64_t gq[2], c0p[2], c1p[2];
#pragma unroll
		for (int h = 0; h < 2; ++h) {
			uint64_t g = (rp.n && nsb) ? (uint64_t)((double)p[h] / (double)rp.n * (double)nsb) : 0;
			if (nsb && g >= nsb) g = nsb - 1;
			gq[h] = g;
			const bool on = ok[h] && nsb;
			const uint64_t c = on ? (rp.sb0 + g) >> SCHUNK_SH : 0;
			c0p[h] = oldp.sbbase[c].pos; c1p[h] = oldp.sbbase[c + 1].pos;
		}
#pragma unroll
		for (int h = 0; h < 2; ++h) {
			uint64_t g = gq[h];
			const bool on = ok[h] && nsb;
			if (on) {
				const uint64_t c = (rp.sb0 + g) >> SCHUNK_SH, pa = base + p[h];
				const uint64_t s_lo = max(c << SCHUNK_SH, rp.sb0), s_hi = min((c + 1) << SCHUNK_SH, rp.sb0 + nsb);
				const uint64_t p_lo = (c << SCHUNK_SH) >= rp.sb0 ? c0p[h] : base, p_hi = ((c + 1) << SCHUNK_SH) <= rp.sb0 + nsb ? c1p[h] : base + rp.n;
				if (pa >= p_lo && pa < p_hi && p_hi > p_lo) {
					uint64_t g2 = s_lo + (uint64_t)((double)(pa - p_lo) / (double)(p_hi - p_lo) * (double)(s_hi - s_lo));
					if (g2 >= s_hi) g2 = s_hi - 1;
					g = g2 - rp.sb0;
				}
			}
			sbi[h] = g;
			const SbRec *rec = oldp.sbrec + (on ? rp.sb0 + g : 0);
			const SbBase *bb = oldp.sbbase + (on ? (rp.sb0 + g) >> SCHUNK_SH : 0);
			hi[h] = *(const uint4*)&rec->cum[4];
			cg[h] = rec->cum[aq[h] & 3u];
			bp[h] = bb->pos; bc[h] = bb->cum[aq[h]];
		}
		uint64_t g2[2]; bool again[2];
#pragma unroll
		for (int h = 0; h < 2; ++h) {
			const bool on = ok[h] && nsb;
			const uint64_t P0 = bp[h] + hi[h].z - base;
			const bool in = P0 <= p[h] && (p[h] < P0 + hi[h].w || sbi[h] + 1 >= nsb);
			again[h] = on && !in;
			g2[h] = p[h] < P0 ? sbi[h] - 1 : sbi[h] + 1;
			sbs[h] = P0;
			cum[h] = bc[h] + (aq[h] < 4u ? cg[h] : (aq[h] == 4u ? hi[h].x : hi[h].y));
		}
		if (again[0] || again[1]) {
#pragma unroll
			for (int h = 0; h < 2; ++h) {
				const SbRec *rec = oldp.sbrec + (again[h] ? rp.sb0 + g2[h] : 0);
				const SbBase *bb = oldp.sbbase + (again[h] ? (rp.sb0 + g2[h]) >> SCHUNK_SH : 0);
				if (again[h]) { hi[h] = *(const uint4*)&rec->cum[4]; cg[h] = rec->cum[aq[h] & 3u]; bp[h] = bb->pos; bc[h] = bb->cum[aq[h]]; }
			}
#pragma unroll
			for (int h = 0; h < 2; ++h) if (again[h]) {
				const uint64_t P0 = bp[h] + hi[h].z - base;
				const bool in = P0 <= p[h] && (p[h] < P0 + hi[h].w || g2[h] + 1 >= nsb);
				slow[h] = !in;
				sbi[h] = g2[h]; sbs[h] = P0;
				cum[h] = bc[h] + (aq[h] < 4u ? cg[h] : (aq[h] == 4u ? hi[h].x : hi[h].y));
			}
		}
	}
	Loc lc[2];
	uint4 fr[2][3], cr[2][3];
#pragma unroll
	for (int h = 0; h < 2; ++h) {
		const bool ld = ok[h] && nsb && !slow[h];
		const uint4 *q = (const uint4*)dir_row(oldp, ld ? rp.sb0 + sbi[h] : 0, 0), *qc = (const uint4*)dir_row(oldp, ld ? rp.sb0 + sbi[h] : 0, 1 + (int)aq[h]);
#pragma unroll
		for (int i = 0; i < 3; ++i) { fr[h][i] = q[i]; cr[h][i] = qc[i]; }
	}
	static_assert(SP_USED == 24, "three 16-byte pieces of a directory row are the slots a re-layout fills");
	P rko[2] = { 0, 0 };
#pragma unroll
	for (int h = 0; h < 2; ++h) {
		lc[h].gl = rp.leaf0; lc[h].s = 0; lc[h].n = 0; lc[h].p2 = 0;
		if (!ok[h] || !nsb) continue;
		if (slow[h]) {
			lc[h] = locate(oldp, rp, p[h]);
			rko[h] = (P)(sb_cum(oldp, lc[h].gl / SB, (int)aq[h]) + dir_prefix(oldp, lc[h].gl / SB, 1 + (int)aq[h], (uint32_t)(lc[h].gl % SB)));
			continue;
		}
		const uint32_t rel = (uint32_t)(p[h] - sbs[h]);
		uint32_t run = 0, klo = 0, pre = 0, nk = 0;
		auto scan8 = [&](const uint4 &v, int i) {
			const uint32_t w[4] = { v.x, v.y, v.z, v.w };
#pragma unroll
			for (int j = 0; j < 8; ++j) {
				const uint32_t e = (j & 1) ? w[j >> 1] >> 16 : w[j >> 1] & 0xffffu, n = e & FILL_MASK;
				if (n > 0 && run <= rel) { klo = (uint32_t)(8 * i + j); pre = run; nk = e; }
				run += n;
			}
		};
#pragma unroll
		for (int i = 0; i < 3; ++i) scan8(fr[h][i], i);
		uint32_t acc = 0;
		auto add8 = [&](const uint4 &v, int i) {
			const uint32_t w[4] = { v.x, v.y, v.z, v.w };
#pragma unroll
			for (int j = 0; j < 4; ++j) {
				const uint32_t s0 = (uint32_t)(8 * i + 2 * j);
				acc += w[j] & (klo > s0 + 1 ? 0xffffffffu : (klo == s0 + 1 ? 0xffffu : 0u));
			}
		};
		if (run <= rel) {
			scan8(((const uint4*)dir_row(oldp, rp.sb0 + sbi[h], 0))[3], 3);
			if (klo > 24u) add8(((const uint4*)dir_row(oldp, rp.sb0 + sbi[h], 1 + (int)aq[h]))[3], 3);
		}
#pragma unroll
		for (int i = 0; i < 3; ++i) add8(cr[h][i], i);
		lc[h].gl = (rp.sb0 + sbi[h]) * SB + klo; lc[h].s = sbs[h] + pre; lc[h].n = nk & FILL_MASK; lc[h].p2 = nk >> 15;
		rko[h] = (P)(cum[h] + (acc & 0xffffu) + (acc >> 16));
	}
	bool head[2];
#pragma unroll
	for (int h = 0; h < 2; ++h) head[h] = ok[h] && (pprev[h] == ~0ull || pprev[h] < lc[h].s);
	uint32_t tot;
	const uint32_t mine = (uint32_t)head[0] + (uint32_t)head[1];
	uint32_t off = block_excl_add<uint32_t>(mine, s_w, &tot);
	if (threadIdx.x == 0) { const uint32_t ws = ctl->wstride, c = tile / (ws / STILE); s_base = c * ws + (tot ? atomicAdd(&ctl->wcnt[c * WLS], tot) : 0u); }
	__syncthreads();
	off += s_base;
// ... 855 lines not shown
```

ropebwt2_amd/hipbwt.py:

```python
import ctypes as C
import os

import numpy as np

from .build import lib_path

K_NAMES = ["k_sym", "k_tscan", "k_prep", "k_part", "k_merge", "k_meta", "k_advance", "k_init", "k_relayout", "k_split"]
_lib = None


def load_hip_lib():
    global _lib
    if _lib is not None:
        return _lib
    path = os.environ.get("RB2_HIP_LIB") or lib_path("librb2hip.so")
    if not os.path.exists(path):
        raise RuntimeError("%s missing: run `python -m ropebwt2_amd.build` (hipcc, gfx950) first" % path)
    L = C.CDLL(path)
    vp, i64, i32, u64 = C.c_void_p, C.c_int64, C.c_int, C.c_uint64
    sig = {
        "rb2_hip_device_count": (i32, []),
        "rb2_hip_set_fatal_handler": (None, [vp, vp]),
        "rb2_hip_create": (vp, [i32, i32]),
        "rb2_hip_destroy": (None, [vp]),
        "rb2_hip_sorting_order": (i32, [vp]),
        "rb2_hip_reset": (None, [vp]),
        "rb2_hip_insert_multi": (None, [vp, i64, vp]),
        "rb2_hip_insert_multi_dev": (None, [vp, i64, vp]),
        "rb2_hip_prefetch": (None, [vp, vp, i64, i64]),
        "rb2_hip_set_lazy": (None, [vp, C.c_int]),
        "rb2_hip_wait": (None, [vp]),
        "rb2_hip_last_batch_counts": (C.c_int, [vp, vp]),
        "rb2_hip_mem_info": (None, [i32, vp, vp]),
        "rb2_hip_get_counts": (None, [vp, vp]),
        "rb2_hip_rope_bytes": (i64, [vp, i32]),
        "rb2_hip_download_rope": (i64, [vp, i32, vp]),
        "rb2_hip_stream_rope": (i64, [vp, i32, vp, vp]),
        "rb2_hip_load_ropes": (None, [vp, vp, vp]),
        "rb2_hip_load_fmd": (i64, [vp, vp, i64]),
        "rb2_hip_load_fmd_file": (i64, [vp, C.c_char_p]),
        "rb2_hip_save_fmd": (i64, [vp, vp, i64]),
        "rb2_hip_save_fmd_file": (i64, [vp, C.c_char_p]),
        "rb2_hip_delete_strings": (i64, [vp, i64, vp]),
        "rb2_hip_delete_stats": (None, [vp, vp]),
        "rb2_hip_rank1a": (None, [vp, i32, i64, vp]),
        "rb2_hip_rank_batch": (None, [vp, i32, i64, vp, vp]),
        "rb2_hip_backward_search": (None, [vp, i64, vp, vp, vp]),
        "rb2_hip_backward_search_dev": (None, [vp, i64, vp, vp, vp]),
        "rb2_hip_extend": (None, [vp, i64, vp, i32, vp]),
        "rb2_hip_extract": (i64, [vp, i64, vp, i64, vp, vp]),
        "rb2_hip_smem": (i64, [vp, i64, vp, vp, i64, i64, i64, vp, vp]),
        "rb2_hip_smem_dev": (None, [vp, i64, vp, vp, i64, i64, i64, vp, vp]),
        "rb2_hip_ssa_build": (i64, [vp, i32]),
        "rb2_hip_ssa_drop": (None, [vp]),
        "rb2_hip_ssa_info": (None, [vp, vp]),
        "rb2_hip_locate": (i64, [vp, i64, vp, i64, vp, vp]),
        "rb2_hip_locate_dev": (None, [vp, i64, vp, i64, vp, vp]),
        "rb2_hip_overlap": (i64, [vp, i64, vp, vp, i64, i64, vp, vp]),
        "rb2_hip_overlap_dev": (None, [vp, i64, vp, vp, i64, i64, vp, vp]),
        "rb2_hip_string_ids": (i64, [vp, i64, vp, i64, vp, vp]),
        "rb2_hip_string_ids_dev": (None, [vp, i64, vp, i64, vp, vp]),
        "rb2_hip_kmers": (i64, [vp, i32, i64, i32, i64, vp, i64, vp, vp]),
        "rb2_hip_approx": (i64, [vp, i64, vp, vp, i32, i64, i64, i64, vp, vp]),
        "rb2_hip_approx_dev": (None, [vp, i64, vp, vp, i32, i64, i64, i64, vp, vp]),
        "rb2_hip_contained": (i64, [vp, i64, vp, vp]),
        "rb2_hip_contained_dev": (None, [vp, i64, vp, vp]),
        "rb2_hip_irreducible": (i64, [vp, i64, vp, vp, i64, i64, i64, i64, vp, vp]),
        "rb2_hip_irreducible_dev": (None, [vp, i64, vp, vp, i64, i64, i64, i64, i64, vp, vp]),
        "rb2_hip_unitig_chains": (i64, [vp, i64, i64, vp, vp, vp]),
        "rb2_hip_unitig_chains_dev": (None, [vp, i64, i64, vp, vp, vp]),
        "rb2_hip_unitig_text": (i64, [vp, i64, vp, i32, i64, i64, i64, vp, vp, vp]),
        "rb2_hip_unitig_text_dev": (i64, [vp, i64, vp, i32, i64, i64, i64, vp, vp, vp]),
        "rb2_hip_unpack": (i64, [vp, i64, i64, i32, i64, vp, vp]),
        "rb2_hip_unpack_dev": (i64, [vp, i64, i64, i32, i64, vp, vp]),
        "rb2_hip_merge": (i64, [vp, vp, i64, vp]),
        "rb2_hip_string_graph": (i64, [vp, i64, i64, i64, i64, i64, i64, i64, i32, i64, vp, vp]),
        "rb2_hip_string_graph_dev": (i64, [vp, i64, i64, i64, i64, i64, i64, i64, i32, i64, vp, vp]),
        "rb2_hip_reserve": (None, [vp, i64, i64, i64]),
        "rb2_hip_num_subropes": (i32, []),
        "rb2_hip_memcpy": (None, [vp, vp, vp, i64, i32]),
        "rb2_hip_use_stream": (None, [vp, vp]),
        "rb2_hip_dev_alloc": (vp, [vp, i64]),
        "rb2_hip_dev_free": (None, [vp, vp]),
        "rb2_hip_synth_reads": (None, [vp, vp, i64, i64, i32, u64, i32]),
        "rb2_hip_synth_reads_cov": (None, [vp, vp, i64, i64, i32, u64, i32, i64]),
        "rb2_hip_synth_reads_skew": (None, [vp, vp, i64, i64, i32, u64, i32, i64, i32]),
        "rb2_hip_sync": (None, [vp]),
        "rb2_hip_sparse_stats": (None, [vp, vp]),
        "rb2_hip_layout_stats": (None, [vp, vp]),
        "rb2_hip_rewind_stats": (None, [vp, vp]),
        "rb2_hip_steady_stats": (None, [vp, vp]),
        "rb2_hip_lean_stats": (None, [vp, vp]),
        "rb2_hip_window_stats": (None, [vp, vp]),
        "rb2_hip_host_register": (C.c_int, [vp, C.c_int64]),
        "rb2_hip_host_unregister": (C.c_int, [vp]),
        "rb2_hip_profile": (None, [vp, i32]),
        "rb2_hip_profile_get": (None, [vp, vp, vp, vp, i32]),
        "rb2_hip_kernel_name": (C.c_char_p, [i32]),
        "rb2_hip_layout": (None, [vp, vp, vp]),
        "rb2_hip_multi_create": (vp, [i32, vp, i32, i32, vp]),
        "rb2_hip_multi_unique_id": (None, [vp]),
        "rb2_hip_multi_create_rank": (vp, [i32, i32, i32, vp, i32, vp]),
        "rb2_hip_multi_destroy": (None, [vp]),
        "rb2_hip_default_owners": (None, [i32, vp]),
        "rb2_hip_multi_nranks": (i32, [vp]),
        "rb2_hip_multi_transport": (i32, [vp]),
        "rb2_hip_multi_nlocal": (i32, [vp]),
        "rb2_hip_multi_engine": (vp, [vp, i32]),
        "rb2_hip_multi_insert_multi": (None, [vp, i64, vp]),
        "rb2_hip_multi_insert_multi_dev": (None, [vp, i64, vp]),
        "rb2_hip_multi_get_counts": (None, [vp, vp]),
        "rb2_hip_multi_rope_bytes": (i64, [vp, i32]),
        "rb2_hip_multi_download_rope": (i64, [vp, i32, vp]),
        "rb2_hip_multi_stream_rope": (i64, [vp, i32, vp, vp]),
        "rb2_hip_multi_load_ropes": (None, [vp, vp, vp]),
        "rb2_hip_multi_load_fmd": (i64, [vp, vp, i64]),
        "rb2_hip_multi_reserve": (None, [vp, i64, i64, i64]),
        "rb2_hip_multi_reset": (None, [vp]),
        "rb2_hip_multi_sync": (None, [vp]),
        "rb2_hip_multi_rank1a": (None, [vp, i32, i64, vp]),
        "rb2_hip_multi_stats": (None, [vp, vp]),
        "rb2_hip_multi_text_bytes": (i64, [vp, C.c_int]),
        "rb2_hip_multi_rope_hash": (u64, [vp, i32]),
        "rb2_hip_multi_plan_host": (i32, [vp, i32, vp, i32, vp, vp, vp]),
        "rb2_hip_rope_hash": (u64, [vp, i32]),
    }
    for name, (res, args) in sig.items():
        try:
            f = getattr(L, name)
        except AttributeError:
            if os.environ.get("RB2_HIP_LIB"):
                continue
            raise
        f.restype = res
        f.argtypes = args
    _lib = L
    return L


ABI_SYMBOLS = [
    "rb2_hip_device_count", "rb2_hip_set_fatal_handler", "rb2_hip_create", "rb2_hip_destroy", "rb2_hip_sorting_order", "rb2_hip_reset",
    "rb2_hip_insert_multi", "rb2_hip_insert_multi_dev", "rb2_hip_set_lazy", "rb2_hip_wait", "rb2_hip_last_batch_counts", "rb2_hip_prefetch", "rb2_hip_mem_info", "rb2_hip_get_counts", "rb2_hip_rope_bytes",
    "rb2_hip_download_rope", "rb2_hip_stream_rope", "rb2_hip_load_ropes", "rb2_hip_load_fmd", "rb2_hip_load_fmd_file", "rb2_hip_save_fmd", "rb2_hip_save_fmd_file", "rb2_hip_delete_strings", "rb2_hip_delete_stats", "rb2_hip_rank1a", "rb2_hip_rank_batch", "rb2_hip_reserve",
    "rb2_hip_backward_search", "rb2_hip_backward_search_dev", "rb2_hip_extend", "rb2_hip_extract", "rb2_hip_smem", "rb2_hip_smem_dev", "rb2_hip_dev_alloc",
    "rb2_hip_ssa_build", "rb2_hip_ssa_drop", "rb2_hip_ssa_info", "rb2_hip_locate", "rb2_hip_locate_dev",
    "rb2_hip_overlap", "rb2_hip_overlap_dev", "rb2_hip_string_ids", "rb2_hip_string_ids_dev", "rb2_hip_kmers",
    "rb2_hip_approx", "rb2_hip_approx_dev", "rb2_hip_contained", "rb2_hip_contained_dev",
    "rb2_hip_irreducible", "rb2_hip_irreducible_dev",
    "rb2_hip_unitig_chains", "rb2_hip_unitig_chains_dev", "rb2_hip_unitig_text", "rb2_hip_unitig_text_dev",
    "rb2_hip_unpack", "rb2_hip_unpack_dev", "rb2_hip_merge",
    "rb2_hip_string_graph", "rb2_hip_string_graph_dev",
    "rb2_hip_num_subropes", "rb2_hip_memcpy", "rb2_hip_use_stream",
    "rb2_hip_dev_free", "rb2_hip_synth_reads", "rb2_hip_synth_reads_cov", "rb2_hip_synth_reads_skew", "rb2_hip_sync", "rb2_hip_sparse_stats", "rb2_hip_layout_stats", "rb2_hip_rewind_stats", "rb2_hip_steady_stats", "rb2_hip_lean_stats", "rb2_hip_window_stats", "rb2_hip_host_register", "rb2_hip_host_unregister", "rb2_hip_profile",
    "rb2_hip_profile_get", "rb2_hip_kernel_name", "rb2_hip_layout",
    "rb2_hip_multi_create", "rb2_hip_multi_unique_id", "rb2_hip_multi_create_rank", "rb2_hip_multi_destroy", "rb2_hip_default_owners",
    "rb2_hip_multi_nranks", "rb2_hip_multi_transport", "rb2_hip_multi_nlocal", "rb2_hip_multi_engine", "rb2_hip_multi_insert_multi", "rb2_hip_multi_insert_multi_dev",
    "rb2_hip_multi_get_counts", "rb2_hip_multi_rope_bytes", "rb2_hip_multi_download_rope", "rb2_hip_multi_stream_rope",
    "rb2_hip_multi_load_ropes", "rb2_hip_multi_load_fmd", "rb2_hip_multi_reserve", "rb2_hip_multi_rope_hash", "rb2_hip_rope_hash", "rb2_hip_multi_plan_host", "rb2_hip_multi_reset", "rb2_hip_multi_sync", "rb2_hip_multi_rank1a", "rb2_hip_multi_stats", "rb2_hip_multi_text_bytes",
]


_NT6 = np.full(256, 255, dtype=np.uint8)
for _i, _ch in enumerate("$ACGTN"):
    _NT6[ord(_ch)] = _NT6[ord(_ch.lower())] = _i


def encode_pattern(p):
    if isinstance(p, str):
        p = p.encode("ascii")
    if isinstance(p, (bytes, bytearray)):
        a = _NT6[np.frombuffer(bytes(p), dtype=np.uint8)]
        if (a == 255).any():
            raise ValueError("pattern %r: only the letters $ACGTN are allowed" % (p,))
        return a
    return np.asarray(p, dtype=np.uint8).reshape(-1)


def pack_patterns(patterns):
    enc = [encode_pattern(p) for p in patterns]
    off = np.zeros(len(enc) + 1, np.int64)
    if enc:
        off[1:] = np.cumsum([len(e) for e in enc])
    pat = np.concatenate(enc) if enc and off[-1] else np.zeros(1, np.uint8)
    return np.ascontiguousarray(pat, dtype=np.uint8), off


def pack_kmer(seq):
    a = encode_pattern(seq).astype(np.uint64)
    if not 1 <= len(a) <= 32 or (a < 1).any() or (a > 4).any():
        raise ValueError("k-mer %r: 1 .. 32 symbols out of ACGT" % (seq,))
    return np.uint64(((a - np.uint64(1)) << (np.uint64(2) * np.arange(len(a) - 1, -1, -1, dtype=np.uint64))).sum())


def unpack_kmers(codes, k):
    codes = np.asarray(codes, dtype=np.uint64).reshape(-1)
    sh = np.uint64(2) * np.arange(k - 1, -1, -1, dtype=np.uint64)
    return ((codes[:, None] >> sh[None, :]) & np.uint64(3)).astype(np.uint8) + np.uint8(1)


def pack_subs(subs):
    subs = sorted(((int(p), int(c)) for p, c in subs), reverse=True)
    if len(subs) > 4 or any(not (0 <= p < 8192 and 1 <= c <= 4) for p, c in subs) or len({p for p, _ in subs}) != len(subs):
        raise ValueError("substitutions %r: at most four (pos, sym) with distinct pos < 8192 and sym in 1..4" % (subs,))
    return sum((p << 3 | c) << (16 * k) for k, (p, c) in enumerate(subs))


def unpack_subs(subs):
    subs = int(subs) & 0xFFFFFFFFFFFFFFFF
    out = []
    while subs & 0xFFFF:
        out.append(((subs & 0xFFFF) >> 3, subs & 7))
        subs >>= 16
    return out


class StepBudgetExceeded(RuntimeError):
    def __init__(self, queries, results, who="approx", lower="max_mm"):
        RuntimeError.__init__(self, "%s: %d queries ran out of steps (the first: %s); raise max_steps or lower %s" % (who, len(queries), queries[:5], lower))
        self.queries, self.results = queries, results


def expand_runs(rle):
    rle = np.asarray(rle, dtype=np.uint8)
    return np.repeat(rle & 7, rle >> 3)


def encode_runs(symbols):
    symbols = np.asarray(symbols, dtype=np.uint8)
    out = bytearray()
    if len(symbols) == 0:
        return np.zeros(0, np.uint8)
    edges = np.flatnonzero(np.diff(symbols)) + 1
    starts = np.concatenate([[0], edges])
    lens = np.diff(np.concatenate([starts, [len(symbols)]]))
    for c, l in zip(symbols[starts].tolist(), lens.tolist()):
        if l < 16:
            out.append(l << 3 | c)
        else:
            n = 2 if l < 256 else 4 if l < (1 << 19) else 8
            tail = []
            for _ in range(n - 1):
                tail.append(0x80 | (l & 0x3f))
                l >>= 6
            out.append({2: 0xC0, 4: 0xE0, 8: 0xF0}[n] | l << 3 | c)
            out.extend(reversed(tail))
    return np.frombuffer(bytes(out), dtype=np.uint8)


def _fmd_image(src):
    if isinstance(src, (str, os.PathLike)):
        return np.fromfile(os.fspath(src), dtype=np.uint8)
    if isinstance(src, (bytes, bytearray, memoryview)):
        return np.frombuffer(src, dtype=np.uint8)
    return np.ascontiguousarray(src, dtype=np.uint8).reshape(-1)


def _stored(cnt, cap, what):
    if (cnt < 0).any():
        raise ValueError("%s: %s" % (what, np.flatnonzero(cnt < 0)[:5].tolist()))
    return np.minimum(cnt, cap)


class HipBwt:

    def __init__(self, sorting_order=0, device=0):
        self.L = load_hip_lib()
        if self.L.rb2_hip_device_count() <= 0:
            raise RuntimeError("no HIP device visible: the gfx950 engine has no CPU fallback")
        self.h = self.L.rb2_hip_create(device, sorting_order)
        self.so = sorting_order

    def close(self):
        if getattr(self, "h", None):
            self.L.rb2_hip_destroy(self.h)
            self.h = None

    def __del__(self):
        try:
            self.close()
        except Exception:
            pass

    def reset(self):
        self.L.rb2_hip_reset(self.h)

    def insert_multi(self, buf):
        buf = np.ascontiguousarray(buf, dtype=np.uint8)
        self.L.rb2_hip_insert_multi(self.h, len(buf), buf.ctypes.data)

    def insert_multi_dev(self, dev_ptr, nbytes):
        self.L.rb2_hip_insert_multi_dev(self.h, nbytes, dev_ptr)

    def set_lazy(self, on):
        self.L.rb2_hip_set_lazy(self.h, int(on))

    def wait(self):
        self.L.rb2_hip_wait(self.h)

    def last_batch_counts(self):
        d = np.zeros(36, np.int64)
        return d.reshape(6, 6) if self.L.rb2_hip_last_batch_counts(self.h, d.ctypes.data) else None

    def prefetch(self, buf, n_final, capacity=0):
        self.L.rb2_hip_prefetch(self.h, buf.ctypes.data, n_final, capacity or len(buf))

    def counts(self):
# ... 327 lines not shown

    def unitig_text_dev(self, n_str, vtx_dev, urec_dev, txt_dev, canonical=False, min_reads=1, cap_u=0, cap_txt=0):
        info = np.zeros(4, np.int64)
        stored = self.L.rb2_hip_unitig_text_dev(self.h, n_str, vtx_dev, int(bool(canonical)), int(min_reads), int(cap_u), int(cap_txt), urec_dev or None, txt_dev or None,
                                                info.ctypes.data)
        return int(stored), info

    def unitigs(self, min_ovlp, canonical=True, min_reads=1, **kw):
        vtx, _ = self.unitig_chains(self.edges(min_ovlp=min_ovlp, pairs=True, **kw))
        urec, txt = self.unitig_text(vtx, canonical, min_reads)
        order = np.lexsort((vtx[:, 1], vtx[:, 0]))
        first = np.searchsorted(vtx[order, 0], urec[:, 0])
        return [(txt[o:o + l].copy(), order[f:f + k].copy(), bool(fl & 1)) for (hd, k, o, l, fl), f in zip(urec.tolist(), first.tolist())]

    def _graph_args(self, who, first, n, max_ext, pairs):
        total = self._n_strings()
        if pairs and (self.so != 0 or total % 2):
            raise ValueError("%s(pairs=True): the index must be in input order and hold an even number of strings" % who)
        if n is None:
            n = total - first
        if max_ext is None:
            off = np.zeros(total + 1, np.int64)
            self.L.rb2_hip_unpack(self.h, 0, total, 0, 0, None, off.ctypes.data)
            max_ext = min(max(int(np.diff(off).max()) - 1 if total else 1, 1), 8192)
        return int(first), int(n), int(max_ext)

    def string_graph_dev(self, first, n, edges_dev, cap, min_ovlp=1, max_ext=8192, max_steps=1 << 16, max_recs=16, max_hits=8, pairs=False):
        info = np.zeros(8, np.int64)
        m = self.L.rb2_hip_string_graph_dev(self.h, first, n, min_ovlp, max_ext, max_steps, max_recs, max_hits, int(bool(pairs)), int(cap), edges_dev or None, info.ctypes.data)
        return int(m), info

    def string_graph_raw(self, first, n, cap, min_ovlp=1, max_ext=8192, max_steps=1 << 16, max_recs=16, max_hits=8, pairs=False, fill=0):
        edges = np.full((max(int(cap), 0), 4), fill, np.int64)
        info = np.zeros(8, np.int64)
        m = self.L.rb2_hip_string_graph(self.h, first, n, min_ovlp, max_ext, max_steps, max_recs, max_hits, int(bool(pairs)), int(cap), edges.ctypes.data if len(edges) else None,
                                        info.ctypes.data)
        return int(m), edges, info

    def string_graph(self, first=0, n=None, min_ovlp=1, max_ext=None, max_steps=1 << 16, max_recs=16, max_hits=8, pairs=False):
        first, n, max_ext = self._graph_args("string_graph", first, n, max_ext, pairs)
        kw = dict(min_ovlp=min_ovlp, max_ext=max_ext, max_steps=max_steps, max_recs=max_recs, max_hits=max_hits, pairs=pairs)
        m, edges, info = self.string_graph_raw(first, n, 2 * n + 16, **kw)
        if m > len(edges):
            m, edges, info = self.string_graph_raw(first, n, m, **kw)
        return edges[:m].copy(), info

    def assemble(self, min_ovlp, canonical=True, min_reads=1, **kw):
        _, n, max_ext = self._graph_args("assemble", 0, None, kw.pop("max_ext", None), True)
        kw.update(min_ovlp=min_ovlp, max_ext=max_ext, pairs=True)
        ptrs = []

        def alloc(nbytes):
            ptrs.append(self.dev_alloc(max(int(nbytes), 8)))
            return ptrs[-1]

        def fetch(dev, shape, dtype):
            a = np.zeros(shape, dtype)
            if a.nbytes:
                self.L.rb2_hip_memcpy(self.h, a.ctypes.data, dev, a.nbytes, 1)
            return a
        try:
            cap = 2 * n + 16
            d_edges = alloc(32 * cap)
            m, info = self.string_graph_dev(0, n, d_edges, cap, **kw)
            if m > cap:
                self.dev_free(ptrs.pop())
                cap = m
                d_edges = alloc(32 * cap)
                m, info = self.string_graph_dev(0, n, d_edges, cap, **kw)
            d_vtx, d_cinfo = alloc(32 * n), alloc(32)
            self.unitig_chains_dev(n, m, d_edges, d_vtx, d_cinfo)
            _, tinfo = self.unitig_text_dev(n, d_vtx, None, None, canonical, min_reads)
            cap_u, cap_txt = int(tinfo[0]), int(tinfo[1])
            d_urec, d_txt = alloc(40 * cap_u), alloc(cap_txt)
            if cap_u and cap_txt:
                stored, _ = self.unitig_text_dev(n, d_vtx, d_urec, d_txt, canonical, min_reads, cap_u, cap_txt)
                assert stored == cap_u, (stored, cap_u)
            self.sync()
            urec = fetch(d_urec, (cap_u, 5), np.int64) if cap_txt else np.zeros((0, 5), np.int64)
            txt = fetch(d_txt, cap_txt, np.uint8)
            vtx = fetch(d_vtx, (n, 4), np.int64)[:, :2]
            self.sync()
        finally:
            for d in ptrs:
                self.dev_free(d)
        order = np.lexsort((vtx[:, 1], vtx[:, 0]))
        first = np.searchsorted(vtx[order, 0], urec[:, 0])
        return [(txt[o:o + l].copy(), order[f:f + k].copy(), bool(fl & 1)) for (hd, k, o, l, fl), f in zip(urec.tolist(), first.tolist())], info

    def _n_strings(self):
        return int(self.counts()[:, 0].sum())

    def unpack_raw(self, first=0, n=None, reversed=False):
        if n is None:
            n = self._n_strings() - first
        off = np.zeros(max(n, 0) + 1, np.int64)
        size = int(self.L.rb2_hip_unpack(self.h, first, n, int(bool(reversed)), 0, None, off.ctypes.data))
        txt = np.empty(size, np.uint8)
        if size:
            got = int(self.L.rb2_hip_unpack(self.h, first, n, int(bool(reversed)), size, txt.ctypes.data, off.ctypes.data))
            assert got == size, (got, size)
        return txt, off

    def unpack(self, first=0, n=None):
        txt, off = self.unpack_raw(first, n, False)
        return [txt[off[i]:off[i + 1] - 1].copy() for i in range(len(off) - 1)]

    def unpack_dev(self, first, n, reversed, cap, txt_dev, off_dev):
        return int(self.L.rb2_hip_unpack_dev(self.h, first, n, int(bool(reversed)), cap, txt_dev, off_dev))

    def merge(self, other, batch_bytes=0):
        info = np.zeros(4, np.int64)
        self.L.rb2_hip_merge(self.h, other.h, batch_bytes, info.ctypes.data)
        return tuple(int(v) for v in info)

    def dev_alloc(self, nbytes):
        return self.L.rb2_hip_dev_alloc(self.h, nbytes)

    def dev_free(self, p):
        self.L.rb2_hip_dev_free(self.h, p)

    def synth_reads(self, dev_ptr, first, n_reads, read_len, seed=42, strand=0, genome_len=0, skew=0):
        self.L.rb2_hip_synth_reads_skew(self.h, dev_ptr, first, n_reads, read_len, seed, strand, genome_len, skew)

    def sync(self):
        self.L.rb2_hip_sync(self.h)

    def sparse_stats(self):
        a = np.zeros(4, np.int64)
        self.L.rb2_hip_sparse_stats(self.h, a.ctypes.data)
        return {"relayouts": int(a[0]), "void_rounds": int(a[1]), "sparse_rounds": int(a[2]), "sparse_now": bool(a[3])}

    def layout_stats(self):
        a = np.zeros(8, np.int64)
        self.L.rb2_hip_layout_stats(self.h, a.ctypes.data)
        return {"relayouts": int(a[0]), "void_rounds": int(a[1]), "sparse_rounds": int(a[2]), "sparse_now": bool(a[3]),
                "respreads": int(a[4]), "leaf_splits": int(a[5]), "grown_in_rounds": int(a[6]), "plain_handovers": int(a[7])}

    def rewind_stats(self):
        a = np.zeros(4, np.int64)
        self.L.rb2_hip_rewind_stats(self.h, a.ctypes.data)
        return {"rewinds": int(a[0]), "rounds_taken_back": int(a[1]), "deepest": int(a[2]), "even_depth": int(a[3])}

    def steady_stats(self):
        a = np.zeros(4, np.int64)
        self.L.rb2_hip_steady_stats(self.h, a.ctypes.data)
        return {"advance_single": int(a[0]), "prep_skipped": int(a[1]), "reported_at": int(a[2]), "used_from": int(a[3])}

    def lean_stats(self):
        a = np.zeros(2, np.int64)
        self.L.rb2_hip_lean_stats(self.h, a.ctypes.data)
        return {"rounds": int(a[0]), "stage": int(a[1])}

    def window_stats(self):
        a = np.zeros(6, np.int64)
        self.L.rb2_hip_window_stats(self.h, a.ctypes.data)
        return {"plain": int(a[0]), "compact0": int(a[1]), "compact1": int(a[2]), "compact2": int(a[3]), "compact_rounds": int(a[4]), "counted": bool(a[5])}

    def profile(self, on=True):
        self.L.rb2_hip_profile(self.h, int(on))

    def profile_get(self, reset=False):
        n = len(K_NAMES)
        la = np.zeros(n, np.int64)
        ms = np.zeros(n, np.float64)
        un = np.zeros(n, np.int64)
        self.L.rb2_hip_profile_get(self.h, la.ctypes.data, ms.ctypes.data, un.ctypes.data, 1 if reset else 0)
        return {K_NAMES[i]: {"launches": int(la[i]), "ms": float(ms[i]), "units": int(un[i])} for i in range(n)}

    @staticmethod
    def layout():
        L = load_hip_lib()
        a, b, c = C.c_int(), C.c_int(), C.c_int()
        L.rb2_hip_layout(C.byref(a), C.byref(b), C.byref(c))
        return {"leaf_syms": a.value, "tile_leaves": b.value, "string_tile": c.value}


TRANSPORTS = {"peer": 0, "rccl": 1}


class _Engine(HipBwt):

    def __init__(self, lib, h, so):
        self.L, self.h, self.so = lib, h, so

    def close(self):
        self.h = None


class MultiBwt:

    def __init__(self, sorting_order, devices, transport="peer", owners=None, rank=None, nranks=None, nccl_id=None):
        self.L = load_hip_lib()
        if self.L.rb2_hip_device_count() <= 0:
            raise RuntimeError("no HIP device visible: the gfx950 engine has no CPU fallback")
        own = (C.c_int * len(owners))(*owners) if owners is not None else None
        self.so = sorting_order
        if rank is None:
            devs = (C.c_int * len(devices))(*devices)
            self.h = self.L.rb2_hip_multi_create(len(devices), devs, sorting_order, TRANSPORTS[transport], own)
        else:
            idb = C.create_string_buffer(bytes(nccl_id), 128) if nccl_id is not None else None
            self.h = self.L.rb2_hip_multi_create_rank(devices[0], rank, nranks, idb, sorting_order, own)
        self.n = self.L.rb2_hip_multi_nlocal(self.h)
        self.world = self.L.rb2_hip_multi_nranks(self.h)

    @staticmethod
    def unique_id():
        b = C.create_string_buffer(128)
        load_hip_lib().rb2_hip_multi_unique_id(b)
        return b.raw

    @staticmethod
    def default_owners(nranks):
        a = (C.c_int * 31)()
        load_hip_lib().rb2_hip_default_owners(nranks, a)
        return list(a)

    def text_bytes(self):
        return [int(self.L.rb2_hip_multi_text_bytes(self.h, k)) for k in range(self.n)]

    def close(self):
        if getattr(self, "h", None):
            self.L.rb2_hip_multi_destroy(self.h)
            self.h = None

    def __del__(self):
        try:
            self.close()
        except Exception:
            pass

    def engine(self, k=0):
        return _Engine(self.L, self.L.rb2_hip_multi_engine(self.h, k), self.so)

    def insert_multi(self, buf):
        buf = np.ascontiguousarray(buf, dtype=np.uint8)
        self.L.rb2_hip_multi_insert_multi(self.h, len(buf), buf.ctypes.data)

    def insert_multi_dev(self, dev_ptrs, nbytes):
        if not isinstance(dev_ptrs, (list, tuple)):
            dev_ptrs = [dev_ptrs] * self.n
        arr = (C.c_void_p * self.n)(*dev_ptrs)
        self.L.rb2_hip_multi_insert_multi_dev(self.h, nbytes, arr)

    def counts(self):
        c = np.zeros(36, np.int64)
        self.L.rb2_hip_multi_get_counts(self.h, c.ctypes.data)
        return c.reshape(6, 6)

    def rope_rle(self, b):
        n = self.L.rb2_hip_multi_rope_bytes(self.h, b)
        out = np.zeros(max(n, 1), np.uint8)
        got = self.L.rb2_hip_multi_download_rope(self.h, b, out.ctypes.data)
        assert got == n
        return out[:n]

    def rope(self, b):
        return expand_runs(self.rope_rle(b))

    def load_ropes(self, rles):
        arrs = [np.ascontiguousarray(r, dtype=np.uint8) for r in rles]
        ptrs = (C.c_void_p * 6)(*[a.ctypes.data if len(a) else None for a in arrs])
        lens = (C.c_int64 * 6)(*[len(a) for a in arrs])
        self.L.rb2_hip_multi_load_ropes(self.h, ptrs, lens)

    def load_fmd(self, src):
        img = _fmd_image(src)
        return int(self.L.rb2_hip_multi_load_fmd(self.h, img.ctypes.data, len(img)))

    def reserve(self, batch_bytes=0, batch_strings=0, total_symbols=0):
        self.L.rb2_hip_multi_reserve(self.h, batch_bytes, batch_strings, total_symbols)

    def reset(self):
        self.L.rb2_hip_multi_reset(self.h)

    def rope_hashes(self):
        return [int(self.L.rb2_hip_multi_rope_hash(self.h, b)) for b in range(6)]

    def sync(self):
        self.L.rb2_hip_multi_sync(self.h)

    def rank1a(self, b, x):
        c = np.zeros(6, np.int64)
        self.L.rb2_hip_multi_rank1a(self.h, b, x, c.ctypes.data)
        return c

    def stats(self):
        a = np.zeros(6, np.int64)
        self.L.rb2_hip_multi_stats(self.h, a.ctypes.data)
        return {"host_syncs_in_rounds": int(a[0]), "rounds": int(a[1]), "batches": int(a[2]), "sparse_rounds": int(a[3]),
                "void_rounds": int(a[4]), "relayouts": int(a[5])}
```

Measured before the change: 24.32 Gsymbols/s.

## Fuse k_part work-order build into the k_tfix launch for lean steady rounds

For lean steady rounds with multi-launch tails, the tile-fix kernel and the leaf work-order (k_part) kernel are fused into one launch, k_tfix_part. The part blocks recompute each rope's new layout (n, leaf0, window offsets) themselves from the old rope sizes and segment counts through a shared layout helper, so they no longer wait for setup to write the new rope descriptors. This removes one kernel launch and its serialisation from the merge phase. The cost is duplicated layout arithmetic in every part block and tighter coupling between the counting and merge phases. It can be turned off with RB2_PART_RIDE.

```diff
diff --git a/include/rb2_hip.h b/include/rb2_hip.h
--- a/include/rb2_hip.h
+++ b/include/rb2_hip.h
@@ -164,6 +164,7 @@
 void rb2_hip_rewind_stats(rb2_hip_t *h, int64_t out[4]);
 void rb2_hip_steady_stats(rb2_hip_t *h, int64_t out[4]);
 void rb2_hip_lean_stats(rb2_hip_t *h, int64_t out[2]);
+void rb2_hip_part_ride_stats(rb2_hip_t *h, int64_t out[2]);
 void rb2_hip_window_stats(rb2_hip_t *h, int64_t out[6]);
 
 #define RB2_K_SYM      0
diff --git a/ropebwt2_amd/build.py b/ropebwt2_amd/build.py
--- a/ropebwt2_amd/build.py
+++ b/ropebwt2_amd/build.py
@@ -32,7 +32,7 @@
 def build_hip(force=False):
     os.makedirs(LIBDIR, exist_ok=True)
     out = lib_path("librb2hip.so")
-    srcs = [os.path.join(CSRC, f) for f in ("rb2_engine.hip", "rb2_kernels.h", "rb2_merge.h", "rb2_device.h", "rb2_multi.h", "rb2_query.h", "rb2_unitig.h", "rb2_query_host.h", "rb2_query_plan.h", "rb2_kmer_plan.h", "rb2_fmd_load.h", "rb2_delete.h", "rb2_delete_plan.h", "rb2_fmd_save.h", "rb2_fmd_plan.h", "rb2_unpack.h", "rb2_merge_plan.h", "rb2_graph.h", "rb2_graph_plan.h")] + [os.path.join(INC, "rb2_hip.h")]
+    srcs = [os.path.join(CSRC, f) for f in ("rb2_engine.hip", "rb2_kernels.h", "rb2_merge.h", "rb2_device.h", "rb2_multi.h", "rb2_query.h", "rb2_unitig.h", "rb2_query_host.h", "rb2_query_plan.h", "rb2_kmer_plan.h", "rb2_fmd_load.h", "rb2_delete.h", "rb2_delete_plan.h", "rb2_fmd_save.h", "rb2_fmd_plan.h", "rb2_unpack.h", "rb2_merge_plan.h", "rb2_part_layout.h", "rb2_graph.h", "rb2_graph_plan.h")] + [os.path.join(INC, "rb2_hip.h")]
     if not force and _newer(out, srcs):
         return out
     hipcc = os.environ.get("HIPCC", "/opt/rocm/bin/hipcc")
diff --git a/ropebwt2_amd/csrc/rb2_engine.hip b/ropebwt2_amd/csrc/rb2_engine.hip
--- a/ropebwt2_amd/csrc/rb2_engine.hip
+++ b/ropebwt2_amd/csrc/rb2_engine.hip
@@ -198,6 +198,8 @@
 	int64_t n_prep_skipped = 0, steady_seen = -1, steady_used = -1;
 	int lean = 1;
 	int64_t n_lean_rounds = 0;
+	int part_ride = 1;
+	int64_t n_parted_rounds = 0;
 	int64_t n_rewind = 0, n_rewound = 0, rewind_max = 0, n_rewind_even = 0;
 	unsigned long long *pair_d = nullptr, *pair_h = nullptr;
 	bool pair_valid = false;
@@ -336,6 +338,7 @@
 	bool known_steady = false;
 	uint64_t counted = (uint64_t)-1;
 	int lean = 0;
+	int parted = 0;
 	uint64_t setup_round = (uint64_t)-1;
 	bool setup_sparse = false; uint64_t setup_epoch = 0;
 };
@@ -474,7 +477,7 @@
 		hipLaunchKernelGGL(k_widen, dim3(cdiv(B.m, 256)), dim3(256), 0, st, (const uint32_t*)h->INS_E.p, a->p, B.m);
 	}
 	h->pos32 = false;
-	B.counted = (uint64_t)-1; B.lean = 0;
+	B.counted = (uint64_t)-1; B.lean = 0; B.parted = 0;
 	if (h->trace) fprintf(stderr, "[rb2_hip] round %llu: positions widened to 64 bits (largest piece known: %llu symbols, %llu rounds ago)\n", (unsigned long long)r, (unsigned long long)known, (unsigned long long)since);
 	return 0;
 }
@@ -489,6 +492,8 @@
 inline bool lazy_round(const rb2_hip_t *h, bool spec) { return spec && h->lazy_verdict && h->nranks == 1; }
 void require_verdicts_seen(const rb2_hip_t *h, uint64_t r, const char *what)
 { if (h->spec_rounds > 0) { rb2_fatal("[rb2_hip] internal: %s %llu queued behind %llu in-place rounds without their verdict\n", what, (unsigned long long)r, (unsigned long long)h->spec_rounds); } }
+inline unsigned merge_windows(const rb2_hip_t *h, const BatchState &B, uint64_t r) { return cdiv(B.n_tot + rank_share(h, std::min<uint64_t>(B.len, (r + 1) * B.m)), WIN) + NR; }
+inline const uint8_t *merge_old_xh(rb2_hip_t *h) { return h->pool_compact ? (const uint8_t*)h->pool[h->pside].view().xh : (const uint8_t*)nullptr; }
 void round_counts(rb2_hip_t *h, BatchState &B, uint64_t r, bool spec = false, bool allow_lean = true)
 {
 	hipStream_t st = h->st;
@@ -499,6 +504,7 @@
 	tl_slow(h, "start of round_counts");
 	B.lean = (allow_lean && !spec && h->nranks == 1 && !h->sparse && B.known_steady && h->steady_on) ? h->lean : 0;
 	const bool one_launch_tail = B.nst_ub < (unsigned)h->ts_max;
+	B.parted = (B.lean && h->part_ride && !one_launch_tail) ? 1 : 0;
 	if (!spec) require_verdicts_seen(h, r, "counting phase without spec of round");
 	SplitArgs sp; memset(&sp, 0, sizeof(sp));
 	if (spec) {
@@ -533,8 +539,14 @@
 	    hipLaunchKernelGGL(k_tscan3<false>, dim3(B.nsc), dim3(SCHUNK), 0, st, h->ctl, sd, trs, h->cpart.p, h->tsc.p);
 	  }
 	  const int do_setup = h->nranks == 1;
-	  hipLaunchKernelGGL(k_tfix, dim3(std::max<unsigned>(1u, cdiv(B.nst_ub, 256))), dim3(256), 0, st, h->ctl, sd, (int)(r & 1), trs, h->tsc.p, h->tfix.p, h->gcnt, do_setup, (int)h->sparse, (uint32_t)r, hmax_report(h), (int)spec, steady_report(h));
+	  if (!B.parted) hipLaunchKernelGGL(k_tfix, dim3(std::max<unsigned>(1u, cdiv(B.nst_ub, 256))), dim3(256), 0, st, h->ctl, sd, (int)(r & 1), trs, h->tsc.p, h->tfix.p, h->gcnt, do_setup, (int)h->sparse, (uint32_t)r, hmax_report(h), (int)spec, steady_report(h));
 	  if (do_setup) mark_setup(h, B, r); }
+	if (B.parted)
+	{ Scope sc(h, RB2_K_PART, units);
+	  const unsigned ntfix = std::max<unsigned>(1u, cdiv(B.nst_ub, 256));
+	  const TfixArgs ta = { h->tsc.p, h->tfix.p, h->gcnt, 1, 0, (uint32_t)r, hmax_report(h), 0, steady_report(h) };
+	  with_pos(h, B, [&](const auto &S) { using P = std::remove_pointer_t<decltype(S.L)>;
+	    hipLaunchKernelGGL((k_tfix_part<P>), dim3(ntfix + cdiv(merge_windows(h, B, r) + NR, 255)), dim3(256), 0, st, h->ctl, sd, (int)(r & 1), trs, ta, ntfix, (const P*)S.L, h->LD.p, merge_old_xh(h)); }); }
 	tl_slow(h, "tile scans");
 }
 
@@ -566,19 +578,22 @@
 	PoolView oldp = h->pool[h->pside].view(), newp = h->pool[h->pside ^ 1].view();
 	const uint64_t n_new_ub = B.n_tot + std::min<uint64_t>(B.len, (r + 1) * B.m);
 	const unsigned nlf = cdiv(n_new_ub, WIN) + NR;
-	const unsigned wg = cdiv(B.n_tot + rank_share(h, std::min<uint64_t>(B.len, (r + 1) * B.m)), WIN) + NR;
+	const unsigned wg = merge_windows(h, B, r);
 	if ((uint64_t)nlf * 64 >= (1ull << 32)) { rb2_fatal("[rb2_hip] the index is too large for one k_merge launch (%llu symbols: a launch is capped at 2^32 threads)\n", (unsigned long long)n_new_ub); }
 	if (!setup_done(h, B, r, false))
 	{ Scope sc(h, RB2_K_TSCAN, 0);
 	  hipLaunchKernelGGL(k_setup<false>, dim3(1), dim3(64), 0, st, h->ctl, sd, h->gcnt, (int)(r & 1), (uint32_t)r, hmax_report(h), (int)(h->push[0] != nullptr), steady_report(h)); }
 	const bool lean = B.lean != 0;
 	if (lean && (h->nranks != 1 || h->sparse || !B.known_steady)) { rb2_fatal("[rb2_hip] internal: round %llu was counted lean and is not merged as a steady dense round\n", (unsigned long long)r); }
+	if (B.parted && !lean) { rb2_fatal("[rb2_hip] internal: the work orders of round %llu were cut inside its counting phase and the round is not merged lean\n", (unsigned long long)r); }
 	if (lean) ++h->n_lean_rounds;
+	if (B.parted) ++h->n_parted_rounds;
 	with_pos(h, B, [&](const auto &S) { using P = std::remove_pointer_t<decltype(S.L)>;
 	launch_prep<false>(h, B, r, oldp, S);
 	tl_slow(h, "k_prep");
+	if (!B.parted)
 	{ Scope sc(h, RB2_K_PART, units);
-	  const uint8_t *old_xh = h->pool_compact ? (const uint8_t*)oldp.xh : (const uint8_t*)nullptr;
+	  const uint8_t *old_xh = merge_old_xh(h);
 	  if (lean) hipLaunchKernelGGL((k_part<false, P, true>), dim3(cdiv(wg + NR, 255)), dim3(256), 0, st, h->ctl, sd, (const P*)S.L, h->LD.p, old_xh);
 	  else RB2_LAUNCH_STRIDE(h, (k_part<true, P>), (k_part<false, P>), dim3(cdiv(wg + NR, 255)), dim3(256), 0, st, h->ctl, sd, S.INS_E, h->LD.p, old_xh); }
 	tl_slow(h, "k_part");
@@ -596,7 +611,7 @@
 	HIPCHK(hipGetLastError());
 	tl_slow(h, "ne snapshot");
 	h->side ^= 1; h->pside ^= 1; B.cur ^= 1;
-	B.lean = 0;
+	B.lean = 0; B.parted = 0;
 	h->pool_compact = compact_out;
 	if (compact_out) ++h->n_compact_rounds;
 }
@@ -701,7 +716,7 @@
 	HIPCHK(hipMemsetAsync(&h->ctl->overflow, 0, 4, h->st));
 	h->spec_rounds = 0; h->mb_h->void_round = 0;
 	h->mb_h->progress = (uint32_t)r_void;
-	B.counted = (uint64_t)-1; B.setup_round = (uint64_t)-1; B.lean = 0;
+	B.counted = (uint64_t)-1; B.setup_round = (uint64_t)-1; B.lean = 0; B.parted = 0;
 	return depth;
 }
 
@@ -907,7 +922,7 @@
 			++h->n_rewind; h->n_rewound += depth; h->rewind_max = std::max(h->rewind_max, depth); if (!(depth & 1)) ++h->n_rewind_even;
 			B.known_ae = B.known_ae0;
 			memset((void*)h->mb_h->ne, 0xff, sizeof(h->mb_h->ne));
-			B.known_steady = false; h->mb_h->steady = 0; B.lean = 0;
+			B.known_steady = false; h->mb_h->steady = 0; B.lean = 0; B.parted = 0;
 			r = r_void;
 			void_to_dense(h, B, r);
 			round_counts(h, B, r);
@@ -985,6 +1000,7 @@
 	if (getenv("RB2_STEADY")) h->steady_on = atoi(getenv("RB2_STEADY")) != 0;
 	if (getenv("RB2_STEADY_LEAN")) h->lean = std::min(1, std::max(0, atoi(getenv("RB2_STEADY_LEAN"))));
 	if (!h->steady_on) h->lean = 0;
+	if (getenv("RB2_PART_RIDE")) h->part_ride = atoi(getenv("RB2_PART_RIDE")) != 0;
 	if (getenv("RB2_STEADY_AHEAD")) h->steady_ahead = std::max(0, atoi(getenv("RB2_STEADY_AHEAD")));
 	{ Ctl *hc = (Ctl*)calloc(1, sizeof(Ctl)); for (int b = 0; b < NR; ++b) hc->own[b] = 1; HIPCHK(hipMemcpy(h->ctl, hc, sizeof(Ctl), hipMemcpyHostToDevice)); free(hc); }
 	HIPCHK(hipMemsetAsync(h->d_tmp, 0, 256, h->st));
@@ -1922,6 +1938,11 @@
 	out[0] = h->n_lean_rounds; out[1] = h->lean;
 }
 
+void rb2_hip_part_ride_stats(rb2_hip_t *h, int64_t out[2])
+{ finish_pending(h);
+	out[0] = h->n_parted_rounds; out[1] = h->part_ride;
+}
+
 void rb2_hip_window_stats(rb2_hip_t *h, int64_t out[6])
 { finish_pending(h);
 	unsigned long long w[4] = {0, 0, 0, 0};
diff --git a/ropebwt2_amd/csrc/rb2_kernels.h b/ropebwt2_amd/csrc/rb2_kernels.h
--- a/ropebwt2_amd/csrc/rb2_kernels.h
+++ b/ropebwt2_amd/csrc/rb2_kernels.h
@@ -1,7 +1,18 @@
 #pragma once
 #include "rb2_device.h"
+#include "rb2_part_layout.h"
 
 namespace rb2 {
+
+struct PartLane { PartPiece p; PartPlace q; uint64_t pinc, winc; };
+__device__ __forceinline__ PartLane part_layout_wave(bool ok, uint64_t old_n, uint64_t cnt)
+{
+	PartLane l;
+	l.p = part_piece<LEAF, SB, WPL>(ok ? old_n : 0ull, ok ? cnt : 0ull);
+	l.pinc = dpp_incl_add64(l.p.padded); l.winc = dpp_incl_add64(l.p.nwin);
+	l.q = part_place<SB>(l.p, l.pinc, l.winc);
+	return l;
+}
 
 
 __device__ __forceinline__ uint32_t zero_bytes(uint32_t x)
@@ -460,8 +471,9 @@
 
 
 template <bool SPARSE> __device__ __forceinline__ void setup_body(Ctl *ctl, int side, const uint64_t *gcnt, int par, uint32_t round, volatile unsigned long long *hmax, volatile unsigned long long *steady, bool keep_ne = false);
-__global__ __launch_bounds__(256) void k_tfix(Ctl *ctl, int side, int par, const TileRecs trec, const TileScan *tsc, TileFix *tf, uint64_t *gcnt, int do_setup, int sparse,
-		uint32_t round, volatile unsigned long long *hmax, int spec, volatile unsigned long long *steady)
+struct TfixArgs { const TileScan *tsc; TileFix *tf; uint64_t *gcnt; int do_setup, sparse; uint32_t round; volatile unsigned long long *hmax; int spec; volatile unsigned long long *steady; };
+__device__ __forceinline__ void tfix_body(Ctl *ctl, int side, int par, const TileRecs &trec, const TileScan *tsc, TileFix *tf, uint64_t *gcnt, int do_setup, int sparse,
+		uint32_t round, volatile unsigned long long *hmax, int spec, volatile unsigned long long *steady, const uint32_t bidx)
 {
 	__shared__ uint32_t s_t0[NR + 1];
 	__shared__ uint64_t s_g[NR * 6];
@@ -469,7 +481,7 @@
 	const SegDesc &sg = ctl->seg[side];
 	if (threadIdx.x <= NR) s_t0[threadIdx.x] = sg.tile0[threadIdx.x];
 	__syncthreads();
-	if (blockIdx.x == 0) {
+	if (bidx == 0) {
 		const int i = threadIdx.x;
 		if (i < NR * 6) { const int b = i / 6, a = i % 6; const uint64_t v = s_t0[NR] ? (uint64_t)(tsc[s_t0[b + 1]].pre[a] - tsc[s_t0[b]].pre[a]) : 0ull; gcnt[i] = v; s_g[i] = v; }
 		if (i == NR * 6) gcnt[NR * 6] = ctl->ne[par];
@@ -478,7 +490,7 @@
 			if (i < 64) { if (sparse) setup_body<true>(ctl, side, s_g, par, round, hmax, steady); else setup_body<false>(ctl, side, s_g, par, round, hmax, steady); }
 		}
 	}
-	const uint32_t tile = blockIdx.x * 256 + threadIdx.x;
+	const uint32_t tile = bidx * 256 + threadIdx.x;
 	if (tile >= s_t0[NR]) return;
 	int b = 0;
 	while (tile >= s_t0[b+1]) ++b;
@@ -501,6 +513,11 @@
 	f.segstart = sg.start[b]; f.segend = sg.start[b] + sg.cnt[b];
 	tf[tile] = f;
 }
+__global__ __launch_bounds__(256) void k_tfix(Ctl *ctl, int side, int par, const TileRecs trec, const TileScan *tsc, TileFix *tf, uint64_t *gcnt, int do_setup, int sparse,
+		uint32_t round, volatile unsigned long long *hmax, int spec, volatile unsigned long long *steady)
+{
+	tfix_body(ctl, side, par, trec, tsc, tf, gcnt, do_setup, sparse, round, hmax, spec, steady, blockIdx.x);
+}
 
 template <bool SPARSE> __device__ __forceinline__ void setup_body(Ctl *ctl, int side, const uint64_t *gcnt , int par, uint32_t round, volatile unsigned long long *hmax, volatile unsigned long long *steady, bool keep_ne)
 {
@@ -523,7 +540,8 @@
 	SegDesc &ng = ctl->seg[side ^ 1];
 	const RopeDesc o = ctl->rope[side][rr];
 	RopeDesc n;
-	n.n = ok ? o.n + sg.cnt[rr] : 0;
+	const PartLane pl = part_layout_wave(ok, o.n, sg.cnt[rr]);
+	n.n = pl.p.n;
 	if (hmax) {
 		unsigned long long mx = n.n;
 #pragma unroll
@@ -543,12 +561,9 @@
 		n.nleaves = o.nleaves; n.leaf0 = o.leaf0; n.sb0 = o.sb0;
 		if (ok) ctl->rope[side ^ 1][r] = n;
 	} else {
-		n.nleaves = (n.n + LEAF - 1) / LEAF;
-		const uint64_t padded = (n.nleaves + SB - 1) / SB * SB, nwin = (n.nleaves + WPL - 1) / WPL;
-		const uint64_t pinc = dpp_incl_add64(padded), winc = dpp_incl_add64(nwin);
-		n.leaf0 = pinc - padded; n.sb0 = n.leaf0 / SB;
-		if (ok) { ctl->rope[side ^ 1][r] = n; ctl->wf0[r] = winc - nwin; }
-		if (r == 63) { ctl->wf0[NR] = winc; ctl->wf0[NR + 1] = winc; ctl->nsb_total = pinc / SB; }
+		n.nleaves = pl.p.nleaves; n.leaf0 = pl.q.leaf0; n.sb0 = pl.q.sb0;
+		if (ok) { ctl->rope[side ^ 1][r] = n; ctl->wf0[r] = pl.q.wf0; }
+		if (r == 63) { ctl->wf0[NR] = pl.winc; ctl->wf0[NR + 1] = pl.winc; ctl->nsb_total = pl.pinc / SB; }
 	}
 	uint64_t c2 = 0;
 	if (ok && r != 0 && ctl->own[r]) {
@@ -926,14 +941,13 @@
 }
 
 
-template <bool STRIDE, typename P = uint64_t, bool LEAN = false> __global__ __launch_bounds__(256) void k_part(const Ctl *ctl, int side, const P *INS_E, LeafDesc *LD, const uint8_t *old_xh)
-{
-	__shared__ uint64_t s_wf0[NR + 1];
-	__shared__ uint32_t s_q[256];
-	if (threadIdx.x <= NR) s_wf0[threadIdx.x] = ctl->wf0[threadIdx.x];
-	__syncthreads();
-	for (uint64_t blk = blockIdx.x; blk * 255 < s_wf0[NR] + NR; blk += gridDim.x) {
-	if (STRIDE && blk != blockIdx.x) __syncthreads();
+struct PartLay { uint64_t wf0[NR + 1], leaf0[NR], n[NR]; };
+template <bool STRIDE, typename P, bool LEAN> __device__ __forceinline__ void part_body(const Ctl *ctl, int side, const P *INS_E, LeafDesc *LD, const uint8_t *old_xh,
+		const PartLay &lay, uint32_t *s_q , const uint64_t blk0, const uint64_t nblk)
+{
+	const uint64_t *s_wf0 = lay.wf0;
+	for (uint64_t blk = blk0; blk * 255 < s_wf0[NR] + NR; blk += nblk) {
+	if (STRIDE && blk != blk0) __syncthreads();
 	const uint64_t gid = blk * 255 + threadIdx.x;
 	const bool ok = gid < s_wf0[NR] + NR;
 	int b = 0; uint64_t j = 0; uint32_t q = 0;
@@ -953,13 +967,13 @@
 	s_q[threadIdx.x] = q;
 	__syncthreads();
 	if (!ok || threadIdx.x == 255 || j >= s_wf0[b+1] - s_wf0[b]) { if (!STRIDE) return; continue; }
-	const RopeDesc &orp = ctl->rope[side][b], &nrp = ctl->rope[side ^ 1][b];
+	const RopeDesc &orp = ctl->rope[side][b];
 	const uint32_t q1 = s_q[threadIdx.x + 1];
 	const uint64_t o0 = j * WIN, i0 = o0 - q;
 	LeafDesc d;
 	d.i0 = i0;
 	d.ins0 = ctl->seg[side].start[b] + q;
-	d.gl = nrp.leaf0 + j * WPL;
+	d.gl = lay.leaf0[b] + j * WPL;
 	d.oleaf0 = (uint32_t)orp.leaf0;
 	const uint64_t ow = i0 >> 12, onw = (orp.nleaves + WPL - 1) / WPL;
 	static_assert(WPL * LEAF == 4096, "a window is 4096 symbols");
@@ -967,10 +981,40 @@
 	const uint32_t h0 = ow < onw ? (xw ? (uint32_t)xw[ow] & 3u : 0u) : 1u;
 	const uint32_t h1 = ow + 1 < onw ? (xw ? (uint32_t)xw[ow + 1] & 3u : 0u) : 1u;
 	d.ni = (uint16_t)((uint32_t)(q1 - q) | h0 << 14);
-	d.nvalid = (uint16_t)((uint32_t)min((uint64_t)WIN, nrp.n - o0) | h1 << 14);
+	d.nvalid = (uint16_t)((uint32_t)min((uint64_t)WIN, lay.n[b] - o0) | h1 << 14);
 	LD[s_wf0[b] + j] = d;
 	if (!STRIDE) return;
 	}
+}
+
+template <bool STRIDE, typename P = uint64_t, bool LEAN = false> __global__ __launch_bounds__(256) void k_part(const Ctl *ctl, int side, const P *INS_E, LeafDesc *LD, const uint8_t *old_xh)
+{
+	__shared__ PartLay s_lay;
+	__shared__ uint32_t s_q[256];
+	if (threadIdx.x <= NR) s_lay.wf0[threadIdx.x] = ctl->wf0[threadIdx.x];
+	if (threadIdx.x < NR) { const RopeDesc &nrp = ctl->rope[side ^ 1][threadIdx.x]; s_lay.leaf0[threadIdx.x] = nrp.leaf0; s_lay.n[threadIdx.x] = nrp.n; }
+	__syncthreads();
+	part_body<STRIDE, P, LEAN>(ctl, side, INS_E, LD, old_xh, s_lay, s_q, blockIdx.x, gridDim.x);
+}
+
+template <typename P> __device__ __forceinline__ void part_ride_body(const Ctl *ctl, int side, const P *L, LeafDesc *LD, const uint8_t *old_xh, const uint32_t k)
+{
+	__shared__ PartLay s_lay;
+	__shared__ uint32_t s_q[256];
+	if (threadIdx.x < 64) {
+		const int r = (int)threadIdx.x; const bool ok = r < NR; const int rr = ok ? r : 0;
+		const PartLane pl = part_layout_wave(ok, ctl->rope[side][rr].n, ctl->seg[side].cnt[rr]);
+		if (ok) { s_lay.wf0[r] = pl.q.wf0; s_lay.leaf0[r] = pl.q.leaf0; s_lay.n[r] = pl.p.n; }
+		if (r == 63) s_lay.wf0[NR] = pl.winc;
+	}
+	__syncthreads();
+	part_body<false, P, true>(ctl, side, L, LD, old_xh, s_lay, s_q, k, 1);
+}
+
+template <typename P> __global__ __launch_bounds__(256) void k_tfix_part(Ctl *ctl, int side, int par, const TileRecs trec, const TfixArgs a, const uint32_t ntfix, const P *L, LeafDesc *LD, const uint8_t *old_xh)
+{
+	if (blockIdx.x < ntfix) tfix_body(ctl, side, par, trec, a.tsc, a.tf, a.gcnt, a.do_setup, a.sparse, a.round, a.hmax, a.spec, a.steady, blockIdx.x);
+	else part_ride_body<P>(ctl, side, L, LD, old_xh, blockIdx.x - ntfix);
 }
 
 
diff --git a/ropebwt2_amd/csrc/rb2_part_layout.h b/ropebwt2_amd/csrc/rb2_part_layout.h
--- /dev/null
+++ b/ropebwt2_amd/csrc/rb2_part_layout.h
@@ -0,0 +1,43 @@
+#pragma once
+#include <cstdint>
+
+#if defined(__HIPCC__) || defined(__CUDACC__)
+#define RB2_PL_HD __host__ __device__
+#else
+#define RB2_PL_HD
+#endif
+
+struct PartPiece { uint64_t n, nleaves, padded, nwin; };
+struct PartPlace { uint64_t leaf0, sb0, wf0; };
+
+template <int LEAF_, int SB_, int WPL_> RB2_PL_HD inline PartPiece part_piece(uint64_t old_n, uint64_t cnt)
+{
+	PartPiece p;
+	p.n = old_n + cnt;
+	p.nleaves = (p.n + LEAF_ - 1) / LEAF_;
+	p.padded = (p.nleaves + SB_ - 1) / SB_ * SB_;
+	p.nwin = (p.nleaves + WPL_ - 1) / WPL_;
+	return p;
+}
+
+template <int SB_> RB2_PL_HD inline PartPlace part_place(const PartPiece &p, uint64_t padded_incl, uint64_t nwin_incl)
+{
+	PartPlace q;
+	q.leaf0 = padded_incl - p.padded;
+	q.sb0 = q.leaf0 / SB_;
+	q.wf0 = nwin_incl - p.nwin;
+	return q;
+}
+
+template <int NR_, int LEAF_, int SB_, int WPL_> RB2_PL_HD inline uint64_t part_layout(const uint64_t *old_n, const uint64_t *cnt, uint64_t *n, uint64_t *nleaves, uint64_t *leaf0, uint64_t *wf0)
+{
+	uint64_t pinc = 0, winc = 0;
+	for (int b = 0; b < NR_; ++b) {
+		const PartPiece p = part_piece<LEAF_, SB_, WPL_>(old_n[b], cnt[b]);
+		pinc += p.padded; winc += p.nwin;
+		const PartPlace q = part_place<SB_>(p, pinc, winc);
+		n[b] = p.n; nleaves[b] = p.nleaves; leaf0[b] = q.leaf0; wf0[b] = q.wf0;
+	}
+	wf0[NR_] = winc;
+	return pinc / SB_;
+}
diff --git a/ropebwt2_amd/hipbwt.py b/ropebwt2_amd/hipbwt.py
--- a/ropebwt2_amd/hipbwt.py
+++ b/ropebwt2_amd/hipbwt.py
@@ -91,6 +91,7 @@
         "rb2_hip_rewind_stats": (None, [vp, vp]),
         "rb2_hip_steady_stats": (None, [vp, vp]),
         "rb2_hip_lean_stats": (None, [vp, vp]),
+        "rb2_hip_part_ride_stats": (None, [vp, vp]),
         "rb2_hip_window_stats": (None, [vp, vp]),
         "rb2_hip_host_register": (C.c_int, [vp, C.c_int64]),
         "rb2_hip_host_unregister": (C.c_int, [vp]),
@@ -151,7 +152,7 @@
     "rb2_hip_unpack", "rb2_hip_unpack_dev", "rb2_hip_merge",
     "rb2_hip_string_graph", "rb2_hip_string_graph_dev",
     "rb2_hip_num_subropes", "rb2_hip_memcpy", "rb2_hip_use_stream",
-    "rb2_hip_dev_free", "rb2_hip_synth_reads", "rb2_hip_synth_reads_cov", "rb2_hip_synth_reads_skew", "rb2_hip_sync", "rb2_hip_sparse_stats", "rb2_hip_layout_stats", "rb2_hip_rewind_stats", "rb2_hip_steady_stats", "rb2_hip_lean_stats", "rb2_hip_window_stats", "rb2_hip_host_register", "rb2_hip_host_unregister", "rb2_hip_profile",
+    "rb2_hip_dev_free", "rb2_hip_synth_reads", "rb2_hip_synth_reads_cov", "rb2_hip_synth_reads_skew", "rb2_hip_sync", "rb2_hip_sparse_stats", "rb2_hip_layout_stats", "rb2_hip_rewind_stats", "rb2_hip_steady_stats", "rb2_hip_lean_stats", "rb2_hip_part_ride_stats", "rb2_hip_window_stats", "rb2_hip_host_register", "rb2_hip_host_unregister", "rb2_hip_profile",
     "rb2_hip_profile_get", "rb2_hip_kernel_name", "rb2_hip_layout",
     "rb2_hip_multi_create", "rb2_hip_multi_unique_id", "rb2_hip_multi_create_rank", "rb2_hip_multi_destroy", "rb2_hip_default_owners",
     "rb2_hip_multi_nranks", "rb2_hip_multi_transport", "rb2_hip_multi_nlocal", "rb2_hip_multi_engine", "rb2_hip_multi_insert_multi", "rb2_hip_multi_insert_multi_dev",
@@ -785,6 +786,11 @@
         self.L.rb2_hip_lean_stats(self.h, a.ctypes.data)
         return {"rounds": int(a[0]), "stage": int(a[1])}
 
+    def part_ride_stats(self):
+        a = np.zeros(2, np.int64)
+        self.L.rb2_hip_part_ride_stats(self.h, a.ctypes.data)
+        return {"rounds": int(a[0]), "switch": int(a[1])}
+
     def window_stats(self):
         a = np.zeros(6, np.int64)
         self.L.rb2_hip_window_stats(self.h, a.ctypes.data)
```

Result: no change. 24.53 Gsymbols/s (median of 4 runs) (+0.9%).
